# nemo110110/modify-sift-gpu

Hardware: AMD Instinct MI355X
Metric: SIFT images/sec at 1080p (features/sec alongside), 1/2/4/8 MI355X (higher is better)
Workload: dtype f32

## Files before the change

include/sgpu.h:

```cpp
#ifndef SGPU_H
#define SGPU_H
#include <stddef.h>
#include <stdint.h>

#ifdef __cplusplus
extern "C" {
#endif

#define SGPU_OK 0
#define SGPU_EINVAL (-1)
#define SGPU_ENODEV (-2)
#define SGPU_ENOMEM (-3)
#define SGPU_ERANGE (-4)

typedef struct sgpu_options {
    float filter_width_factor;
    float descriptor_window_factor;
    float orientation_window_factor;
    float orientation_gaussian_factor;
    float dog_threshold;
    float edge_threshold;
    int subpixel;
    int max_orientation;
    int fixed_orientation;
    int octave_min;
    int octave_num;
    int dog_level_num;
    int lowe_origin;
    int normalized;
    int descriptors;
    int keep_extremum_sign;
    int circular_window;
    int verbose;
    int max_dimension;
    int preprocess_on_cpu;
    int feature_count_threshold;
    int truncate_method;
} sgpu_options;

void sgpu_default_options(sgpu_options* opt);

int sgpu_parse_args(sgpu_options* opt, int argc, const char* const* argv, int* device);

typedef struct sgpu_ctx sgpu_ctx;

int sgpu_ctx_create(int device, const sgpu_options* opt, sgpu_ctx** out);
int sgpu_ctx_destroy(sgpu_ctx* ctx);
int sgpu_ctx_set_options(sgpu_ctx* ctx, const sgpu_options* opt);
const char* sgpu_last_error(const sgpu_ctx* ctx);
int sgpu_device_count(void);

#define SGPU_INPUT_HOST   0
#define SGPU_INPUT_DEVICE 1
#define SGPU_INPUT_STAGED 2

int sgpu_stage_input(sgpu_ctx* ctx, const uint8_t* images, int n, int w, int h, int stride);

int sgpu_reserve(sgpu_ctx* ctx, int n, int w, int h, int stride);
int sgpu_last_pyramid_launches(const sgpu_ctx* ctx, int* filters);
long long sgpu_debug_alloc_count(void);

int sgpu_extract(sgpu_ctx* ctx, const uint8_t* images, int n, int w, int h, int stride,
                 int flags);

int sgpu_extract_stream(sgpu_ctx* ctx, const uint8_t* const* batches, int nbatches, int batch,
                        int w, int h, int stride, float* keys, float* desc, int64_t cap,
                        int32_t* counts);
void* sgpu_host_alloc(size_t bytes);
void sgpu_host_free(void* p);

int sgpu_extract_f32(sgpu_ctx* ctx, const float* images, int n, int w, int h, int stride,
                     int flags);

#define SGPU_RGB  1
#define SGPU_BGR  2
#define SGPU_RGBA 3
#define SGPU_BGRA 4
int sgpu_extract_color(sgpu_ctx* ctx, const uint8_t* images, int n, int w, int h, int stride,
                       int format, int flags);

int sgpu_feature_count(const sgpu_ctx* ctx, int image);
int64_t sgpu_feature_total(const sgpu_ctx* ctx);

int sgpu_copy_features(sgpu_ctx* ctx, int image, float* keys, float* descriptors);

int sgpu_device_features(sgpu_ctx* ctx, const float** keys, const float** descriptors,
                         const int64_t** image_offsets);

int sgpu_extract_keypoints(sgpu_ctx* ctx, int image, const float* keys, int num,
                           int has_orientation);

int sgpu_match(sgpu_ctx* ctx, const uint8_t* d1, int n1, const uint8_t* d2, int n2,
               float distmax, float ratiomax, int mutual_best_match, int max_match,
               int* out_pairs, int flags);

int sgpu_match_guided(sgpu_ctx* ctx, const uint8_t* d1, int n1, const uint8_t* d2, int n2,
                      const float* loc1, const float* loc2, const float* H, const float* F,
                      float distmax, float ratiomax, float hdistmax, float fdistmax,
                      int mutual_best_match, int max_match, int* out_pairs, int flags);

int sgpu_match_shard_begin(sgpu_ctx* ctx, const uint8_t* d1, int ns, int row_begin,
                           const uint8_t* d2, int n2, float distmax, float ratiomax,
                           int mutual_best_match, int* row_match, int* col_best, int flags);
int sgpu_match_shard_end(const int* col_best_all, int nshards, int n2, const int* row_match,
                         int ns, int row_begin, float distmax, float ratiomax,
                         int mutual_best_match, int max_match, int* out_pairs);
int sgpu_match_sharded(sgpu_ctx* ctx, const uint8_t* d1, int ns, int row_begin,
                       const uint8_t* d2, int n2, float distmax, float ratiomax,
                       int mutual_best_match, int max_match, int* out_pairs, int flags);

void sgpu_quantize_descriptors(const float* d, size_t count, uint8_t* out);
int sgpu_quantize_descriptors_gpu(sgpu_ctx* ctx, const float* d, size_t ndesc, uint8_t* out,
                                  int flags);
int sgpu_feature_descriptors_u8(sgpu_ctx* ctx, const uint8_t** desc_u8);
int sgpu_copy_features_u8(sgpu_ctx* ctx, int image, uint8_t* desc);

int sgpu_match_batch(sgpu_ctx* ctx, const uint8_t* desc, const int64_t* set_offsets, int nsets,
                     const int* set_pairs , int npairs,
                     float distmax, float ratiomax, int mutual_best_match, int max_match,
                     int* out_pairs , int64_t cap, int* out_counts ,
                     int flags);
int sgpu_match_images(sgpu_ctx* ctx, const int* image_pairs, int npairs, float distmax,
                      float ratiomax, int mutual_best_match, int max_match,
                      int* out_pairs, int64_t cap, int* out_counts);

int sgpu_match_batch_guided(sgpu_ctx* ctx, const uint8_t* desc, const float* loc,
                            const int64_t* set_offsets, int nsets,
                            const int* set_pairs , int npairs,
                            const float* H ,
                            const float* F ,
                            float distmax, float ratiomax, float hdistmax, float fdistmax,
                            int mutual_best_match, int max_match,
                            int* out_pairs , int64_t cap,
                            int* out_counts , int flags);
int sgpu_match_images_guided(sgpu_ctx* ctx, const int* image_pairs, int npairs,
                             const float* H, const float* F,
                             float distmax, float ratiomax, float hdistmax, float fdistmax,
                             int mutual_best_match, int max_match,
                             int* out_pairs, int64_t cap, int* out_counts);

#define SGPU_MODEL_HOMOGRAPHY  0
#define SGPU_MODEL_FUNDAMENTAL 1
int sgpu_estimate_batch(sgpu_ctx* ctx, const float* loc ,
                        const int64_t* set_offsets, int nsets,
                        const int* set_pairs , int npairs,
                        const int* matches ,
                        const int* match_counts ,
                        int model, float threshold, int iterations, uint32_t seed,
                        float* out_models , int* out_inliers ,
                        uint8_t* out_mask , int flags);
int sgpu_estimate_images(sgpu_ctx* ctx, const int* image_pairs, int npairs,
                         const int* matches, const int* match_counts,
                         int model, float threshold, int iterations, uint32_t seed,
                         float* out_models, int* out_inliers, uint8_t* out_mask);
int sgpu_estimate_batch_refined(sgpu_ctx* ctx, const float* loc, const int64_t* set_offsets,
                                int nsets, const int* set_pairs, int npairs, const int* matches,
                                const int* match_counts, int model, float threshold,
                                int iterations, uint32_t seed, int refine_rounds,
                                float* out_models, int* out_inliers, uint8_t* out_mask,
                                int* out_rounds , int flags);
int sgpu_estimate_images_refined(sgpu_ctx* ctx, const int* image_pairs, int npairs,
                                 const int* matches, const int* match_counts,
                                 int model, float threshold, int iterations, uint32_t seed,
                                 int refine_rounds, float* out_models, int* out_inliers,
                                 uint8_t* out_mask, int* out_rounds );

int sgpu_last_timing(const sgpu_ctx* ctx, float* times, int n);
int sgpu_set_host_output(sgpu_ctx* ctx, float* keys, float* descriptors, int capacity);
int sgpu_set_stage_timing(sgpu_ctx* ctx, int on);

#define SGPU_COMM_ID_BYTES 128
int sgpu_comm_unique_id(uint8_t* id, int bytes);
int sgpu_comm_init(sgpu_ctx* ctx, int nranks, int rank, const uint8_t* id, int bytes);
int sgpu_comm_allgather_i32(sgpu_ctx* ctx, const int32_t* send, int n, int32_t* recv);
int sgpu_comm_allreduce_f64(sgpu_ctx* ctx, double* v, int n, int op_max);

#define SGPU_DEBUG_PARTS2   1
#define SGPU_DEBUG_PARTS4   2
#define SGPU_DEBUG_TINY_CAP 4
#define SGPU_DEBUG_FUSED_MATCH 8
#define SGPU_DEBUG_EXACT_DESCRIPTOR 16
#define SGPU_DEBUG_GAUSS_BLOCK 32
#define SGPU_DEBUG_BAND_SHIFT 20
#define SGPU_DEBUG_KEYED_MATCH 64
#define SGPU_DEBUG_FULL_COLUMNS 128
#define SGPU_DEBUG_DESC_DUAL 256
#define SGPU_DEBUG_ORIENT_WAVE 512
#define SGPU_DEBUG_GAUSS_TILE_ALWAYS 1024
#define SGPU_DEBUG_MATCH_REGSTAGE 2048
#define SGPU_DEBUG_PYR_SERIAL 4096
#define SGPU_DEBUG_GAUSS_LONG_BANDS 8192
#define SGPU_DEBUG_DUO_ALWAYS 16384
#define SGPU_DEBUG_DUO_OFF 32768
#define SGPU_DEBUG_GAUSS_TILE_OFF 65536
#define SGPU_DEBUG_DESC_WIDE_OFF 131072
#define SGPU_DEBUG_DESC_WIDE_ALWAYS 262144
#define SGPU_DEBUG_EXTREMA_TILE_OFF 524288

int sgpu_debug_set_flags(sgpu_ctx* ctx, int flags);
#define SGPU_FEATURES_QUEUE 0
#define SGPU_FEATURES_STATIC_ORIENTATION 1
#define SGPU_FEATURES_STATIC_DESCRIPTOR 2
#define SGPU_FEATURES_STATIC 3
int sgpu_debug_set_feature_queue(sgpu_ctx* ctx, int mode);
#define SGPU_TRIO_OFF 0
#define SGPU_TRIO_ON 1
#define SGPU_TRIO_ALWAYS 2
#define SGPU_PAIRS_FRONT 0
#define SGPU_PAIRS_END 1
int sgpu_debug_set_schedule(sgpu_ctx* ctx, int trio, int pairs);
#define SGPU_DUO_STRIPS_RULE 0
#define SGPU_DUO_STRIPS_WAVE 1
#define SGPU_DUO_STRIPS_COOP 2
int sgpu_debug_set_duo_strips(sgpu_ctx* ctx, int mode);
int sgpu_debug_set_match_prune(sgpu_ctx* ctx, int on);
int sgpu_debug_match_plan_stats(const sgpu_ctx* ctx, long long out[4]);
#define SGPU_PLAN_ENTRY_INTS 7
#define SGPU_PLAN_LEVEL 0
#define SGPU_PLAN_TILE 1
#define SGPU_PLAN_TWO 2
#define SGPU_PLAN_TILE_TWO 3
#define SGPU_PLAN_TILE_DUO 4
#define SGPU_PLAN_TILE_DUO_ONE 5
#define SGPU_PLAN_DUO 6
#define SGPU_PLAN_TRIO 7
#define SGPU_PLAN_KINDS 8
int sgpu_debug_pyramid_plan(const sgpu_ctx* ctx, int* out, int cap);
int sgpu_debug_geometry(const sgpu_ctx* ctx, int* n_octaves, int* dims , int max);
int sgpu_debug_gaussian(sgpu_ctx* ctx, int image, int octave, int level, float* out);
int sgpu_debug_candidates(sgpu_ctx* ctx, int* ints, float* floats, int cap, int* n);

typedef struct sgpu_verify_params {
    float distmax, ratiomax;
    int   mutual_best_match;
    int   max_match;
    float h_threshold, f_threshold;
    float hdistmax, fdistmax;
    int   iterations;
    uint32_t seed;
    int   refine_rounds;
} sgpu_verify_params;
void sgpu_default_verify_params(sgpu_verify_params* p);
int sgpu_verify_batch(sgpu_ctx* ctx, const uint8_t* desc, const float* loc,
                      const int64_t* set_offsets, int nsets,
                      const int* set_pairs , int npairs,
                      const sgpu_verify_params* params,
                      float* out_H , int* out_inliers_H ,
                      float* out_F , int* out_inliers_F ,
                      int* out_putative ,
                      int* out_pairs , int64_t cap, int* out_counts ,
                      int flags);
int sgpu_verify_images(sgpu_ctx* ctx, const int* image_pairs, int npairs,
                       const sgpu_verify_params* params,
                       float* out_H, int* out_inliers_H, float* out_F, int* out_inliers_F,
                       int* out_putative, int* out_pairs, int64_t cap, int* out_counts);

int sgpu_select_top_scale_batch(sgpu_ctx* ctx, const float* scale, int scale_stride ,
                                const int64_t* set_offsets, int nsets, int top,
                                int* out_index ,
                                int64_t* out_offsets , int flags);
int sgpu_select_top_scale_images(sgpu_ctx* ctx, int top, int* out_index, int64_t* out_offsets);
int sgpu_prematch_batch(sgpu_ctx* ctx, const uint8_t* desc, const float* scale, int scale_stride,
                        const int64_t* set_offsets, int nsets,
                        const int* set_pairs , int npairs, int top,
                        float distmax, float ratiomax, int mutual_best_match,
                        int* out_counts ,
                        int* out_pairs , int64_t cap, int flags);
int sgpu_prematch_images(sgpu_ctx* ctx, const int* image_pairs, int npairs, int top,
                         float distmax, float ratiomax, int mutual_best_match,
                         int* out_counts, int* out_pairs, int64_t cap);

#ifdef __cplusplus
}
#endif
#endif
```

modify-sift-gpu_amd/csrc/sgpu_capi.cpp:

```cpp
#include <dlfcn.h>

#include <cstdio>
#include <cstdlib>
#include <cstring>

#include "sgpu_ctx.h"

using namespace sgh;

std::atomic<long long> sgh::g_allocs{0};

int sgh::part_streams(Part& pt, int which) {
    int prio_lo = 0, prio_hi = 0;
    (void)hipDeviceGetStreamPriorityRange(&prio_lo, &prio_hi);
    if ((which & PS_MAIN) && !pt.stream &&
        hipStreamCreateWithPriority(&pt.stream, hipStreamNonBlocking, prio_hi) != hipSuccess)
        return SGPU_ENODEV;
    if ((which & PS_LO) && !pt.stream_lo &&
        hipStreamCreateWithPriority(&pt.stream_lo, hipStreamNonBlocking, prio_lo) != hipSuccess)
        return SGPU_ENODEV;
    if ((which & PS_OCT) && !pt.stream_oct &&
        hipStreamCreateWithPriority(&pt.stream_oct, hipStreamNonBlocking, prio_hi) != hipSuccess)
        return SGPU_ENODEV;
    if (!pt.ev_ds) {
        for (hipEvent_t& e : pt.ev)
            if (hipEventCreate(&e) != hipSuccess) return SGPU_ENODEV;
        if (hipEventCreateWithFlags(&pt.ev_ds, hipEventDisableTiming) != hipSuccess ||
            hipEventCreateWithFlags(&pt.ev_oct, hipEventDisableTiming) != hipSuccess)
            return SGPU_ENODEV;
    }
    return SGPU_OK;
}

static void apply_env_hooks(sgpu_ctx* ctx) {
    if (const char* ev = getenv("SGPU_EXACT_DESCRIPTOR"))
        if (ev[0] == '1') ctx->debug_flags |= SGPU_DEBUG_EXACT_DESCRIPTOR;
    if (const char* ev = getenv("SGPU_GAUSS")) {
        if (!strcmp(ev, "block")) ctx->debug_flags |= SGPU_DEBUG_GAUSS_BLOCK;
    }
    if (const char* ev = getenv("SGPU_DUO")) {
        if (!strcmp(ev, "off")) ctx->debug_flags |= SGPU_DEBUG_DUO_OFF;
        if (!strcmp(ev, "always")) ctx->debug_flags |= SGPU_DEBUG_DUO_ALWAYS;
        if (!strcmp(ev, "on")) ctx->duo_on = true;
    }
    if (const char* ev = getenv("SGPU_DUO_WIDE")) {
        if (ev[0] == '1') ctx->duo_wide = true;
    }
    if (const char* ev = getenv("SGPU_DUO_U8")) {
        if (ev[0] == '1') ctx->duo_u8 = true;
    }
    if (const char* ev = getenv("SGPU_DUO_PLAN")) {
        if (!strcmp(ev, "end")) ctx->duo_plan = SGPU_PAIRS_END;
        if (!strcmp(ev, "front")) ctx->duo_plan = SGPU_PAIRS_FRONT;
    }
    if (const char* ev = getenv("SGPU_TRIO")) {
        if (!strcmp(ev, "off")) ctx->trio_mode = SGPU_TRIO_OFF;
        if (!strcmp(ev, "always")) ctx->trio_mode = SGPU_TRIO_ALWAYS;
        if (!strcmp(ev, "on")) ctx->trio_mode = SGPU_TRIO_ON;
    }
    if (const char* ev = getenv("SGPU_GAUSS_BANDS"))
        if (!strcmp(ev, "long")) ctx->debug_flags |= SGPU_DEBUG_GAUSS_LONG_BANDS;
    if (const char* ev = getenv("SGPU_PYR")) {
        if (!strcmp(ev, "serial")) ctx->debug_flags |= SGPU_DEBUG_PYR_SERIAL;
    }
    if (const char* ev = getenv("SGPU_STREAMS")) ctx->multi_stream = !strcmp(ev, "multi");
    if (const char* ev = getenv("SGPU_MATCH"))
        if (!strcmp(ev, "reg")) ctx->debug_flags |= SGPU_DEBUG_MATCH_REGSTAGE;
    if (const char* ev = getenv("SGPU_DESC")) {
        if (!strcmp(ev, "dual")) ctx->debug_flags |= SGPU_DEBUG_DESC_DUAL;
        if (!strcmp(ev, "narrow")) ctx->debug_flags |= SGPU_DEBUG_DESC_WIDE_OFF;
        if (!strcmp(ev, "wide")) ctx->debug_flags |= SGPU_DEBUG_DESC_WIDE_ALWAYS;
    }
    if (const char* ev = getenv("SGPU_GAUSS_TILE")) {
        if (!strcmp(ev, "off")) ctx->debug_flags |= SGPU_DEBUG_GAUSS_TILE_OFF;
        if (!strcmp(ev, "always")) ctx->debug_flags |= SGPU_DEBUG_GAUSS_TILE_ALWAYS;
    }
    if (const char* ev = getenv("SGPU_WIDE_DESC_MAX"))
        if (atoll(ev) >= 0) ctx->wide_desc_max = (size_t)atoll(ev);
    if (const char* ev = getenv("SGPU_WAVE_ORIENT_MAX"))
        if (atoll(ev) >= 0) ctx->wave_orient_max = (size_t)atoll(ev);
    if (const char* ev = getenv("SGPU_EXTREMA")) {
        if (!strcmp(ev, "wave")) ctx->debug_flags |= SGPU_DEBUG_EXTREMA_TILE_OFF;
    }
    if (const char* ev = getenv("SGPU_FEATURE_QUEUE")) {
        if (!strcmp(ev, "on") || !strcmp(ev, "ori") || !strcmp(ev, "desc") || !strcmp(ev, "off")) {
            ctx->queue_ori = !strcmp(ev, "on") || !strcmp(ev, "ori");
            ctx->queue_desc = !strcmp(ev, "on") || !strcmp(ev, "desc");
        }
    }
    if (const char* ev = getenv("SGPU_FEATURE_QUEUE_GRID"))
        if (atoi(ev) >= 1) {
            ctx->fq.ori_grid = std::min(ctx->fq.ori_grid, atoi(ev));
            ctx->fq.desc_grid = std::min(ctx->fq.desc_grid, atoi(ev));
        }
    if (const char* ev = getenv("SGPU_TILE_DUO"))
        ctx->tile_duo = !strcmp(ev, "on");
    if (const char* ev = getenv("SGPU_MATCH_PRUNE"))
        ctx->match_prune = strcmp(ev, "off") != 0;
    if (const char* ev = getenv("SGPU_GAUSS_TILE_MB"))
        if (atoi(ev) >= 0) ctx->tile_mb = atoi(ev);
}

extern "C" {

void sgpu_default_options(sgpu_options* o) {
    o->filter_width_factor = 4.0f;
    o->descriptor_window_factor = 3.0f;
    o->orientation_window_factor = 2.0f;
    o->orientation_gaussian_factor = 1.5f;
    o->dog_threshold = 0.0f;
    o->edge_threshold = 0.0f;
    o->subpixel = 1;
    o->max_orientation = 2;
    o->fixed_orientation = 0;
    o->octave_min = 0;
    o->octave_num = -1;
    o->dog_level_num = 3;
    o->lowe_origin = 0;
    o->normalized = 1;
    o->descriptors = 1;
    o->keep_extremum_sign = 0;
    o->circular_window = 0;
    o->verbose = 0;
    o->max_dimension = 13200;
    o->preprocess_on_cpu = 1;
    o->feature_count_threshold = -1;
    o->truncate_method = 0;
}

int sgpu_parse_args(sgpu_options* o, int argc, const char* const* argv, int* device) {
    if (!o) return SGPU_EINVAL;
    auto key = [](const char* s) {
        std::string k;
        for (int i = 0; i < 4 && s[i]; i++) k += (char)((s[i] >= 'A' && s[i] <= 'Z') ? s[i] + 32 : s[i]);
        return k;
    };
    for (int i = 0; i < argc; i++) {
        const char* arg = argv[i];
        if (!arg || arg[0] != '-' || !arg[1]) continue;
        const std::string k = key(arg + 1);
        const char* param = (i + 1 < argc) ? argv[i + 1] : nullptr;
        float fv = 0.f;
        int iv = 0;
        if (k == "cuda") {
            int dev = -1;
            if (param && sscanf(param, "%d", &dev) == 1 && dev >= 0) {
                if (device) *device = dev;
                i++;
            }
        } else if (k == "sd") o->descriptors = 0;
        else if (k == "unn") o->normalized = 0;
        else if (k == "ndes") o->normalized = 1;
        else if (k == "m" || k == "mo") {
            int mo = 2;
            if (param) sscanf(param, "%d", &mo);
            o->max_orientation = std::min(std::max(1, mo), 4);
        } else if (k == "m2p") o->max_orientation = 2;
        else if (k == "s") {
            int sp = 1;
            if (param) sscanf(param, "%d", &sp);
            o->subpixel = std::min(std::max(0, sp), 5);
        } else if (k == "ofix") o->fixed_orientation = (strcmp(arg + 1, "ofix") == 0);
        else if (k == "lowe") o->lowe_origin = 1;
        else if (k == "sign") o->keep_extremum_sign = 1;
        else if (k == "prep") o->preprocess_on_cpu = 1;
        else if (k == "nopr") o->preprocess_on_cpu = 0;
        else if (!param) continue;
        else if (k == "tc" || k == "tc1" || k == "tc2" || k == "tc3") {
            o->truncate_method = k == "tc2" ? 1 : k == "tc3" ? 2 : 0;
            if (sscanf(param, "%d", &iv) == 1 && iv > 0) { o->feature_count_threshold = iv; i++; }
        } else if (k == "maxd") {
            if (sscanf(param, "%d", &iv) == 1 && iv > 0) { o->max_dimension = iv; i++; }
        }
        else if (k == "f") { if (sscanf(param, "%f", &fv) == 1 && fv > 0) { o->filter_width_factor = fv; i++; } }
        else if (k == "w") { if (sscanf(param, "%f", &fv) == 1 && fv > 0) { o->orientation_window_factor = fv; i++; } }
        else if (k == "dw") { if (sscanf(param, "%f", &fv) == 1 && fv > 0) { o->descriptor_window_factor = fv; i++; } }
        else if (k == "fo") { iv = -3; if (sscanf(param, "%d", &iv) == 1 && iv >= -2) { o->octave_min = iv; i++; } }
        else if (k == "no") {
            iv = -1;
            if (sscanf(param, "%d", &iv) == 1) {
                iv = std::max(-1, iv);
                if (iv == -1 || iv >= 1) { o->octave_num = iv; i++; }
            }
        } else if (k == "t") { if (sscanf(param, "%f", &fv) == 1 && fv > 0 && fv < 0.5f) { o->dog_threshold = fv; i++; } }
        else if (k == "e") { if (sscanf(param, "%f", &fv) == 1 && fv > 0) { o->edge_threshold = fv; i++; } }
        else if (k == "d") { if (sscanf(param, "%d", &iv) == 1 && iv >= 1 && iv <= 6) { o->dog_level_num = iv; i++; } }
        else if (k == "v") { if (sscanf(param, "%d", &iv) == 1 && iv >= 0 && iv <= 4) o->verbose = iv; }
    }
    return SGPU_OK;
}

int sgpu_device_count(void) {
    int n = 0;
    if (hipGetDeviceCount(&n) != hipSuccess) return 0;
    return n;
}

int sgpu_ctx_set_options(sgpu_ctx* ctx, const sgpu_options* opt) {
    if (!ctx) return SGPU_EINVAL;
    sgpu_options o;
    if (opt) o = *opt; else sgpu_default_options(&o);
    if (o.octave_min < -3) o.octave_min = -3;
    if (o.dog_level_num < 1 || o.dog_level_num > 6) return ctx->fail(SGPU_EINVAL, "dog_level_num must be 1..6");
    if (o.max_dimension < 8) return ctx->fail(SGPU_EINVAL, "max_dimension must be >= 8");
    ctx->opt = o;
    ctx->f_ready = false;
    sgp::Options po;
    po.filter_width_factor = o.filter_width_factor;
    po.dog_level_num = o.dog_level_num;
    po.dog_threshold = o.dog_threshold;
    po.edge_threshold = o.edge_threshold;
    po.octave_min = o.octave_min;
    ctx->sched = sgp::make_schedule(po);
    return SGPU_OK;
}

int sgpu_ctx_create(int device, const sgpu_options* opt, sgpu_ctx** out) {
    if (!out) return SGPU_EINVAL;
    *out = nullptr;
    int n = 0;
    if (hipGetDeviceCount(&n) != hipSuccess || n <= 0) return SGPU_ENODEV;
    if (device < 0 || device >= n) return SGPU_EINVAL;
    sgpu_ctx* ctx = new sgpu_ctx();
    ctx->device = device;
    if (hipSetDevice(device) != hipSuccess ||
        hipStreamCreateWithFlags(&ctx->stream, hipStreamNonBlocking) != hipSuccess) {
        delete ctx;
        return SGPU_ENODEV;
    }
    for (int i = 0; i <= T_N; i++) (void)hipEventCreate(&ctx->ev[i]);
    {
        Part* p = ctx->part;
        bool ok = part_streams(p[0], PS_MAIN) == SGPU_OK && part_streams(p[0], PS_OCT) == SGPU_OK &&
                  hipStreamCreateWithFlags(&ctx->h2d, hipStreamNonBlocking) == hipSuccess &&
                  hipStreamCreateWithFlags(&ctx->d2h, hipStreamNonBlocking) == hipSuccess &&
                  part_streams(p[0], PS_LO) == SGPU_OK && part_streams(p[1], PS_OCT) == SGPU_OK &&
                  part_streams(p[2], PS_MAIN) == SGPU_OK && part_streams(p[2], PS_LO) == SGPU_OK &&
                  part_streams(p[1], PS_MAIN) == SGPU_OK && part_streams(p[1], PS_LO) == SGPU_OK;
        ok = ok && sgk::feature_queue_grids(&ctx->fq) == hipSuccess;
        for (int i = 0; ok && i < 2; i++)
            ok = hipEventCreateWithFlags(&ctx->up_ev[i], hipEventDisableTiming) == hipSuccess &&
                 hipEventCreateWithFlags(&ctx->down_ev[i], hipEventDisableTiming) == hipSuccess;
        if (!ok) {
            sgpu_ctx_destroy(ctx);
            return SGPU_ENODEV;
        }
    }
    apply_env_hooks(ctx);
    ctx->env_flags = ctx->debug_flags;
    int rc = sgpu_ctx_set_options(ctx, opt);
    if (rc != SGPU_OK) {
        sgpu_ctx_destroy(ctx);
        return rc;
    }
    *out = ctx;
    return SGPU_OK;
}

int sgpu_ctx_destroy(sgpu_ctx* ctx) {
    if (!ctx) return SGPU_EINVAL;
    (void)hipSetDevice(ctx->device);
    if (ctx->stream) (void)hipStreamSynchronize(ctx->stream);
    for (Part& pt : ctx->part) {
        if (pt.stream) (void)hipStreamSynchronize(pt.stream);
        if (pt.stream_lo) (void)hipStreamSynchronize(pt.stream_lo);
        if (pt.stream_oct) (void)hipStreamSynchronize(pt.stream_oct);
        pt.release();
    }
    comm_release(ctx);
    for (hipStream_t st : {ctx->h2d, ctx->d2h})
        if (st) (void)hipStreamSynchronize(st);
    for (int i = 0; i < 2; i++) {
        if (ctx->up_ev[i]) (void)hipEventDestroy(ctx->up_ev[i]);
        if (ctx->down_ev[i]) (void)hipEventDestroy(ctx->down_ev[i]);
    }
    if (ctx->h2d) (void)hipStreamDestroy(ctx->h2d);
    if (ctx->d2h) (void)hipStreamDestroy(ctx->d2h);
    DevBuf* bufs[] = {&ctx->input, &ctx->input2, &ctx->duo_trash, &ctx->all_keys, &ctx->all_desc, &ctx->gray, &ctx->pre, &ctx->m_d1, &ctx->m_d2, &ctx->m_s1, &ctx->m_s2,
                      &ctx->m_part, &ctx->m_terms, &ctx->m_match, &ctx->m_dist, &ctx->m_mask, &ctx->m_loc,
                      &ctx->m_colpart, &ctx->m_cols, &ctx->m_prune, &ctx->m_s1c,
                      &ctx->b_desc, &ctx->b_s8, &ctx->b_sums, &ctx->b_plan, &ctx->b_part, &ctx->b_dec,
                      &ctx->b_cnt, &ctx->b_out, &ctx->b_loc, &ctx->q_in, &ctx->q_out, &ctx->f_u8, &ctx->f_s8,
                      &ctx->f_sums, &ctx->c_buf, &ctx->e_loc, &ctx->e_plan, &ctx->e_pts, &ctx->e_slots,
                      &ctx->e_out, &ctx->e_mask, &ctx->v_buf, &ctx->p_scale, &ctx->p_index, &ctx->p_u8};
    for (DevBuf* b : bufs) b->release();
    for (int i = 0; i <= T_N; i++)
        if (ctx->ev[i]) (void)hipEventDestroy(ctx->ev[i]);
    if (ctx->stream) (void)hipStreamDestroy(ctx->stream);
    delete ctx;
    return SGPU_OK;
}

const char* sgpu_last_error(const sgpu_ctx* ctx) { return ctx ? ctx->err.c_str() : "null context"; }

long long sgpu_debug_alloc_count(void) { return g_allocs.load(); }

int sgpu_set_stage_timing(sgpu_ctx* ctx, int on) {
    if (!ctx) return SGPU_EINVAL;
    ctx->stage_timing = on != 0;
    return SGPU_OK;
}

int sgpu_last_pyramid_launches(const sgpu_ctx* ctx, int* filters) {
    if (!ctx || ctx->batch <= 0) return SGPU_EINVAL;
    if (filters) *filters = ctx->part[0].gauss_filters;
    return ctx->part[0].gauss_launches;
}

int sgpu_last_timing(const sgpu_ctx* ctx, float* times, int n) {
    if (!ctx || !times) return SGPU_EINVAL;
    for (int i = 0; i < n && i < T_N; i++) times[i] = ctx->timing[i];
    return SGPU_OK;
}

int sgpu_debug_set_flags(sgpu_ctx* ctx, int flags) {
    if (!ctx) return SGPU_EINVAL;
    ctx->debug_flags = flags | ctx->env_flags;
    return SGPU_OK;
}

int sgpu_debug_set_match_prune(sgpu_ctx* ctx, int on) {
    if (!ctx) return SGPU_EINVAL;
    ctx->match_prune = on != 0;
    return SGPU_OK;
}

int sgpu_debug_match_plan_stats(const sgpu_ctx* ctx, long long out[4]) {
    if (!ctx || !out || !ctx->b_planned) return SGPU_EINVAL;
    const sgplan::Plan& plan = ctx->b_hplan;
    long long tiles = 0, chunks = 0;
    for (const sgplan::Item& it : plan.items)
        tiles = std::max<long long>(tiles, (it.c_end - it.c_begin + sgplan::kTileCols - 1) / sgplan::kTileCols);
    for (const sgplan::Side& sd : plan.sides) chunks = std::max<long long>(chunks, sd.chunks);
    out[0] = (long long)plan.items.size();
    out[1] = (long long)plan.sides.size();
    out[2] = tiles;
    out[3] = chunks;
    return SGPU_OK;
}

static_assert(SGPU_PLAN_KINDS == sgpyr::kKinds && SGPU_PLAN_TRIO == sgpyr::kTrio &&
              SGPU_PLAN_TILE_DUO_ONE == sgpyr::kTileDuoOne, "sgpu.h and sift_pyramid_plan.h agree");
int sgpu_debug_pyramid_plan(const sgpu_ctx* ctx, int* out, int cap) {
    if (!ctx || ctx->batch <= 0 || cap < 0 || (cap > 0 && !out)) return SGPU_EINVAL;
    const Part& pt = ctx->part[0];
    const int n = (int)pt.plan.launches.size();
    for (int e = 0; e < n && (e + 1) * SGPU_PLAN_ENTRY_INTS <= cap; e++) {
        const sgpyr::Launch& l = pt.plan.launches[e];
        int* p = out + e * SGPU_PLAN_ENTRY_INTS;
        p[0] = l.kind;
        for (int j = 0; j < 3; j++) {
            p[1 + 2 * j] = l.op[j] < 0 ? -1 : pt.levels[l.op[j]].o;
            p[2 + 2 * j] = l.op[j] < 0 ? -1 : pt.levels[l.op[j]].k;
        }
    }
    return n;
}

static_assert(SGPU_DUO_STRIPS_RULE == sgk::kDuoStripsRule && SGPU_DUO_STRIPS_WAVE == sgk::kDuoStripsWave &&
              SGPU_DUO_STRIPS_COOP == sgk::kDuoStripsCoop, "sgpu.h and sift_kernels.h agree");
int sgpu_debug_set_duo_strips(sgpu_ctx* ctx, int mode) {
    if (!ctx || mode < SGPU_DUO_STRIPS_RULE || mode > SGPU_DUO_STRIPS_COOP) return SGPU_EINVAL;
    ctx->duo_strips = mode;
    return SGPU_OK;
}

int sgpu_debug_set_feature_queue(sgpu_ctx* ctx, int mode) {
    if (!ctx || mode < SGPU_FEATURES_QUEUE || mode > SGPU_FEATURES_STATIC) return SGPU_EINVAL;
    ctx->queue_ori = !(mode & SGPU_FEATURES_STATIC_ORIENTATION);
    ctx->queue_desc = !(mode & SGPU_FEATURES_STATIC_DESCRIPTOR);
    return SGPU_OK;
}

int sgpu_debug_set_schedule(sgpu_ctx* ctx, int trio, int pairs) {
    if (!ctx || trio < SGPU_TRIO_OFF || trio > SGPU_TRIO_ALWAYS || pairs < SGPU_PAIRS_FRONT ||
        pairs > SGPU_PAIRS_END)
        return SGPU_EINVAL;
    ctx->trio_mode = trio;
    ctx->duo_plan = pairs;
    return SGPU_OK;
}

int sgpu_debug_geometry(const sgpu_ctx* ctx, int* n_octaves, int* dims, int max) {
    if (!ctx || !n_octaves) return SGPU_EINVAL;
    *n_octaves = (int)ctx->oct.size();
    for (int o = 0; o < (int)ctx->oct.size() && o < max; o++) {
        dims[3 * o] = ctx->oct[o].w;
        dims[3 * o + 1] = ctx->oct[o].h;
        dims[3 * o + 2] = ctx->oct[o].wa;
    }
    return SGPU_OK;
}

int sgpu_debug_gaussian(sgpu_ctx* ctx, int image, int octave, int level, float* out) {
    if (!ctx || image < 0 || image >= ctx->batch || octave < 0 ||
        octave >= (int)ctx->oct.size() || level < 0 || level >= ctx->sched.level_num)
        return SGPU_EINVAL;
    HIPCHK(ctx, hipSetDevice(ctx->device));
    const Part& pt = ctx->part[ctx->part_of(image)];
    const sgk::OctaveDesc& od = pt.fp.oct[octave];
    const long long npx = (long long)od.wa * od.h;
    const float* src = pt.pyr.as<float>() + od.gauss_off + level * od.level_stride +
                       (image - pt.img0) * npx;
    HIPCHK(ctx, hipMemcpy(out, src, npx * sizeof(float), hipMemcpyDeviceToHost));
    return SGPU_OK;
}

static sgk::DebugCandidatesFn debug_candidates_hook() {
    static sgk::DebugCandidatesFn fn = [] {
        Dl_info info{};
        if (!dladdr(reinterpret_cast<void*>(&sgpu_debug_candidates), &info) || !info.dli_fname)
            return (sgk::DebugCandidatesFn) nullptr;
        std::string path(info.dli_fname);
        const size_t slash = path.rfind('/');
        path = (slash == std::string::npos ? std::string(".") : path.substr(0, slash)) +
               "/libsiftgpu_debug.so";
        void* h = dlopen(path.c_str(), RTLD_NOW | RTLD_LOCAL);
        return h ? reinterpret_cast<sgk::DebugCandidatesFn>(dlsym(h, "sgpu_testhook_candidates"))
                 : (sgk::DebugCandidatesFn) nullptr;
    }();
    return fn;
}

int sgpu_debug_candidates(sgpu_ctx* ctx, int* ints, float* floats, int cap, int* n) {
    if (!ctx || !n) return SGPU_EINVAL;
    uint32_t total = 0;
    for (int p = 0; p < ctx->nparts; p++) total += ctx->part[p].n_cand;
    *n = (int)total;
    if (!ints || !floats || cap < (int)total) return total ? SGPU_ERANGE : SGPU_OK;
    if (total == 0) return SGPU_OK;
    const sgk::DebugCandidatesFn hook = debug_candidates_hook();
    if (!hook) return ctx->fail(SGPU_EINVAL, "test-hook library lib/libsiftgpu_debug.so not found");
    HIPCHK(ctx, hipSetDevice(ctx->device));
    DevBuf a, b;
    ALLOCCHK(ctx, a.ensure(total * sizeof(int4)));
    ALLOCCHK(ctx, b.ensure(total * sizeof(float4)));
    uint32_t at = 0;
    for (int p = 0; p < ctx->nparts; p++) {
        const Part& pt = ctx->part[p];
        if (!pt.n_cand) continue;
        HIPCHK(ctx, hook(pt.pyr.as<float>(), pt.mask.as<uint32_t>(), pt.row_base.as<uint32_t>(),
                         pt.total_rows, pt.row_base.as<uint32_t>() + pt.total_rows,
                         (int)pt.n_cand, &pt.fp, a.as<int4>() + at, b.as<float4>() + at,
                         ctx->stream));
        at += pt.n_cand;
    }
    HIPCHK(ctx, hipMemcpyAsync(ints, a.p, total * sizeof(int4), hipMemcpyDeviceToHost, ctx->stream));
    HIPCHK(ctx, hipMemcpyAsync(floats, b.p, total * sizeof(float4), hipMemcpyDeviceToHost, ctx->stream));
    HIPCHK(ctx, hipStreamSynchronize(ctx->stream));
    at = 0;
    for (int p = 0; p < ctx->nparts; p++) {
        const Part& pt = ctx->part[p];
        for (uint32_t i = 0; i < pt.n_cand; i++) ints[4 * (at + i) + 3] += pt.img0;
        at += pt.n_cand;
    }
    a.release();
    b.release();
    return SGPU_OK;
}

}
```

modify-sift-gpu_amd/csrc/sgpu_ctx.h:

```cpp
#pragma once
#include <hip/hip_runtime.h>

#include <algorithm>
#include <atomic>
#include <cstdint>
#include <string>
#include <vector>

#include "../../include/sgpu.h"
#include "sift_geom.h"
#include "sift_kernels.h"
#include "sift_match_plan.h"
#include "sift_params.h"
#include "sift_pyramid_plan.h"
#include "sift_select.h"

typedef struct ncclComm* ncclComm_t;

namespace sgh {

#ifndef SGK_WIDE_DESC_MAX
#define SGK_WIDE_DESC_MAX 8192
#endif

extern std::atomic<long long> g_allocs;

struct DevBuf {
    void* p = nullptr;
    size_t bytes = 0;
    hipError_t ensure(size_t n) {
        if (n <= bytes) return hipSuccess;
        if (p) (void)hipFree(p);
        p = nullptr;
        bytes = 0;
        n = std::max<size_t>(n, 256);
        g_allocs++;
        hipError_t e = hipMalloc(&p, n);
        if (e == hipSuccess) bytes = n;
        return e;
    }
    void release() {
        if (p) (void)hipFree(p);
        p = nullptr;
        bytes = 0;
    }
    template <class T> T* as() const { return reinterpret_cast<T*>(p); }
};

enum { T_UPLOAD, T_PYRAMID, T_DETECT, T_ORIENT, T_EXPAND, T_DESC, T_DOWNLOAD, T_TOTAL, T_MATCH,
       T_LIST, T_COPY_KEYS, T_COPY_DESC, T_ESTIMATE, T_VERIFY, T_PREMATCH, T_N };

struct Part {
    hipStream_t stream = nullptr;
    hipStream_t stream_lo = nullptr;
    bool one_stream = false;
    hipStream_t stream_oct = nullptr;
    hipEvent_t ev_ds = nullptr;
    hipEvent_t ev_oct = nullptr;
    size_t cand_hint = 0, feat_hint = 0;
    int gauss_launches = 0, gauss_filters = 0;
    std::vector<sgk::LevelOp> ops;
    std::vector<sgpyr::LevelDesc> levels;
    sgpyr::Plan plan;
    bool events = true;
    bool copied_out = false;
    hipEvent_t ev[10] = {};
    int img0 = 0, n = 0;
    sgk::FeatureParams fp{};
    int total_rows = 0;
    long long mask_words = 0;
    size_t cand_cap = 0;
    uint32_t n_cand = 0;
    std::vector<int64_t> img_off;
    int64_t* h_read = nullptr;
    size_t h_read_n = 0;
    DevBuf pyr, mask, row_count, row_base, scan_tmp, cand, info, ocount, eoff, feat, feat_info,
        keys, desc, img_off_dev;
    float timing[T_N] = {};

    void release() {
        DevBuf* bufs[] = {&pyr, &mask, &row_count, &row_base, &scan_tmp, &cand, &info, &ocount,
                          &eoff, &feat, &feat_info, &keys, &desc, &img_off_dev};
        for (DevBuf* b : bufs) b->release();
        if (h_read) (void)hipHostFree(h_read);
        h_read = nullptr;
        for (hipEvent_t& e : ev)
            if (e) (void)hipEventDestroy(e);
        if (stream) (void)hipStreamDestroy(stream);
        if (stream_lo) (void)hipStreamDestroy(stream_lo);
        if (ev_ds) (void)hipEventDestroy(ev_ds);
        if (ev_oct) (void)hipEventDestroy(ev_oct);
        ev_ds = ev_oct = nullptr;
        if (stream_oct) (void)hipStreamDestroy(stream_oct);
        stream = stream_lo = stream_oct = nullptr;
    }
};

constexpr int kMaxParts = 4;
#ifndef SGPU_WAVE_ORIENT_MAX
#define SGPU_WAVE_ORIENT_MAX 16384
#endif
constexpr size_t kWaveOrientationMax = SGPU_WAVE_ORIENT_MAX;

}

struct sgpu_ctx {
    int device = 0;
    hipStream_t stream = nullptr;
    sgpu_options opt{};
    sgp::Schedule sched{};
    sgp::InputPlan plan{};
    int debug_flags = 0;
    bool multi_stream = false;
    bool duo_on = false;
    bool duo_wide = false;
    bool duo_u8 = false;
    int trio_mode = SGPU_TRIO_OFF;
    int duo_plan = SGK_DUO_PLAN;
    int duo_strips = SGPU_DUO_STRIPS_RULE;
    size_t wide_desc_max = SGK_WIDE_DESC_MAX;
    size_t wave_orient_max = sgh::kWaveOrientationMax;
    bool unit_input = true;
    bool tile_duo = false;
    int tile_mb = SGK_TILE_MB;
    int env_flags = 0;
    sgk::FeatureQueue fq{};
    bool queue_ori = true, queue_desc = true;
    struct HostOut {
        float* keys = nullptr;
        float* desc = nullptr;
        int cap = 0;
        bool armed = false, active = false, done = false;
    } host_out;
    bool stage_timing = true;
    bool streaming = false;
    std::string err;
    int batch = 0, w = 0, h = 0, nparts = 0;
    std::vector<sgp::Octave> oct;
    size_t staged_bytes = 0;
    std::vector<int64_t> img_off;
    sgh::Part part[sgh::kMaxParts];
    sgh::DevBuf input, all_keys, all_desc, gray, pre;
    sgh::DevBuf input2;
    sgh::DevBuf duo_trash;
    hipStream_t h2d = nullptr, d2h = nullptr;
    hipEvent_t up_ev[2] = {}, down_ev[2] = {};
    bool gathered = false;
    hipEvent_t ev[sgh::T_N + 1] = {};
    float timing[sgh::T_N] = {};
    sgh::DevBuf m_d1, m_d2, m_s1, m_s2, m_part, m_terms, m_match, m_dist, m_mask, m_loc, m_colpart, m_cols;
    sgh::DevBuf m_prune, m_s1c;
    bool match_prune = true;
    std::vector<int> h_match;
    bool dist_ready = false;
    sgh::DevBuf b_desc, b_s8, b_sums, b_plan, b_part, b_dec, b_cnt, b_out;
    sgh::DevBuf b_loc;
    sgplan::Plan b_hplan;
    bool b_planned = false;
    std::vector<unsigned char> b_tables;
    sgh::DevBuf e_loc, e_plan, e_pts, e_slots, e_out, e_mask;
    sgeo::Plan e_hplan;
    std::vector<unsigned char> e_tables, e_result;
    sgh::DevBuf v_buf;
    std::vector<unsigned char> v_result;
    sgh::DevBuf p_scale, p_index, p_u8;
    sgplan::Plan p_hplan;
    std::vector<int64_t> p_sub;
    std::vector<int> p_pairs;
    sgh::DevBuf q_in, q_out, f_u8, f_s8, f_sums;
    bool f_ready = false;
    ncclComm_t comm = nullptr;
    int comm_ranks = 0, comm_rank = 0;
    sgh::DevBuf c_buf;

    int fail(int code, const char* what, hipError_t e = hipSuccess) {
        err = what;
        if (e != hipSuccess) {
            err += ": ";
            err += hipGetErrorString(e);
        }
        return code;
    }
    int part_of(int i) const {
        for (int p = 0; p < nparts; p++)
            if (i < part[p].img0 + part[p].n) return p;
        return nparts - 1;
    }
};

#define HIPCHK(ctx, call)                                                \
    do {                                                                 \
        hipError_t _e = (call);                                          \
        if (_e != hipSuccess) return (ctx)->fail(SGPU_ENODEV, #call, _e); \
    } while (0)
#define ALLOCCHK(ctx, call)                                              \
    do {                                                                 \
        hipError_t _e = (call);                                          \
        if (_e != hipSuccess) return (ctx)->fail(SGPU_ENOMEM, #call, _e); \
    } while (0)

namespace sgh {
enum { PS_MAIN = 1, PS_LO = 2, PS_OCT = 4, PS_ALL = 7 };
int part_streams(Part& pt, int which = PS_ALL);
float match_dist(int v);
int ensure_dist_table(sgpu_ctx* ctx);
int feature_u8(sgpu_ctx* ctx);
void comm_release(sgpu_ctx* ctx);

struct SetSource {
    bool images = false, device = false;
    const uint8_t* desc = nullptr;
    const float* loc = nullptr;
    const float* scale = nullptr;
    int scale_stride = 1;
};
struct DeviceSets {
    const uint8_t* u8 = nullptr;
    const uint8_t* s8 = nullptr;
    const int* sums = nullptr;
    const float* loc = nullptr;
    int loc_stride = 2;
    const float* scale = nullptr;
    int scale_stride = 1;
    bool timing_started = false;
};
enum { SET_DESC = 1, SET_LOC = 2, SET_SCALE = 4 };
int resolve_sets(sgpu_ctx* ctx, const SetSource& src, int64_t rows, int need, DeviceSets& sets);
int check_batch(sgpu_ctx* ctx, const char* what);
int probe_offsets(const int64_t* off, int nsets);
inline size_t round8(size_t n) { return (n + 7) & ~(size_t)7; }
int ensure_pair_buffers(sgpu_ctx* ctx, const sgplan::Plan& plan, size_t table_bytes,
                        int64_t out_rows, int cnt_pairs, int64_t s8_rows);
int derive_s8(sgpu_ctx* ctx, DeviceSets& sets, int64_t rows);
struct MatchPass {
    const uint8_t* s8;
    const int* sums;
    const sgplan::Plan& plan;
    sgplan::TableView tab;
    float distmax, ratiomax;
    int max_match;
    int64_t out_rows;
    int* d_counts;
    long long* d_offs;
    int* d_out;
    const float* loc = nullptr;
    int loc_stride = 2;
    const sgk::GuidedParams* d_geom = nullptr;
};
int queue_match_pass(sgpu_ctx* ctx, const MatchPass& m);
int download_fitting(sgpu_ctx* ctx, const int* counts, int npairs, const int* d_out, int* out_pairs,
                     int64_t cap, bool want_matches = true);
}
```

modify-sift-gpu_amd/csrc/sgpu_debug.hip:

```cpp
#include <cstdint>

#include "sift_kernels.h"
#include "sift_math.h"

using namespace sgm;

#include "sift_keys.h"

namespace sgk {
namespace {

__global__ __launch_bounds__(64) void k_debug_candidates(
    const float* __restrict__ pyr, const uint32_t* __restrict__ mask,
    const uint32_t* __restrict__ row_base, int total_rows, const uint32_t* __restrict__ n_cand_dev,
    const FeatureParams fp, int4* __restrict__ ints, float4* __restrict__ floats) {
    const uint32_t f = blockIdx.x * 64 + threadIdx.x;
    if (f >= *n_cand_dev) return;
    const KeyLoc L = locate(f, row_base, total_rows, mask, fp);
    const KeyOut kv = key_at(pyr, fp, L);
    ints[f] = make_int4(L.col, L.row, L.o * fp.d + L.j, L.b);
    floats[f] = make_float4(kv.dx, kv.dy, kv.ds, kv.result);
}

}
}

extern "C" __attribute__((visibility("default"))) hipError_t sgpu_testhook_candidates(
    const float* pyr, const uint32_t* mask, const uint32_t* row_base, int total_rows,
    const uint32_t* n_cand_dev, int n_cand_cap, const sgk::FeatureParams* fp, int4* ints,
    float4* floats, hipStream_t stream) {
    if (n_cand_cap <= 0) return hipSuccess;
    hipLaunchKernelGGL(sgk::k_debug_candidates, dim3((n_cand_cap + 63) / 64), dim3(64), 0, stream,
                       pyr, mask, row_base, total_rows, n_cand_dev, *fp, ints, floats);
    return hipGetLastError();
}
```

modify-sift-gpu_amd/csrc/sgpu_extract.cpp:

```cpp
#include <cmath>
#include <cstring>

#include "sgpu_ctx.h"

using namespace sgh;

extern "C" {

static int layout_part(sgpu_ctx* ctx, Part& pt) {
    const sgpu_options& O = ctx->opt;
    const sgp::Schedule& S = ctx->sched;
    const int d = S.dog_level_num, nlev = S.level_num;
    const int noct = (int)ctx->oct.size();
    const int n = pt.n;

    sgk::FeatureParams& fp = pt.fp;
    fp = sgk::FeatureParams{};
    fp.batch = n;
    fp.n_octaves = noct;
    fp.d = d;
    long long goff = 0, moff = 0;
    int rows = 0;
    for (int o = 0; o < noct; o++) {
        const sgp::Octave& oc = ctx->oct[o];
        sgk::OctaveDesc& od = fp.oct[o];
        od.w = oc.w;
        od.h = oc.h;
        od.wa = oc.wa;
        od.nwords = (oc.wa + 31) / 32;
        od.gauss_off = goff;
        od.level_stride = (long long)n * oc.wa * oc.h;
        goff += od.level_stride * nlev;
        od.mask_off = moff;
        od.mask_level_stride = (long long)n * oc.h * od.nwords;
        moff += od.mask_level_stride * d;
        fp.row_off[o] = rows;
        rows += d * oc.h;
    }
    fp.rows_per_image = rows;
    pt.total_rows = rows * n;
    pt.mask_words = moff;
    for (int j = 0; j < d; j++) fp.level_sigma[j] = sgp::level_sigma(S, j + S.level_min + 1);
    fp.sigma_step = powf(2.0f, 1.0f / d);
    fp.t0 = (O.subpixel ? 0.8f : 1.0f) * S.dog_threshold;
    fp.t = S.dog_threshold;
    fp.edge = (S.edge_threshold + 1) * (S.edge_threshold + 1) / S.edge_threshold;
    fp.gaussian_factor = O.orientation_gaussian_factor;
    fp.sample_factor = O.orientation_gaussian_factor * O.orientation_window_factor;
    fp.window_factor = O.descriptor_window_factor;
    fp.subpixel = O.subpixel ? 1 : 0;
    fp.num_orientation = O.fixed_orientation ? 0 : std::min(O.max_orientation, 2);
    fp.keep_sign = O.keep_extremum_sign;
    fp.circular = O.circular_window;
    fp.normalize = O.normalized;
    fp.unit_input = ctx->unit_input ? 1 : 0;
    fp.origin_offset = O.lowe_origin ? 0.0f : 0.5f;
    fp.octave_min = ctx->plan.octave_min + ctx->plan.ds;

    const size_t sum_px = (size_t)goff / (size_t)std::max(1, nlev) / (size_t)n;
    pt.cand_cap = (ctx->debug_flags & SGPU_DEBUG_TINY_CAP)
                      ? std::max<size_t>(pt.cand_cap, 64)
                      : std::max(pt.cand_cap, std::max<size_t>(1024, sum_px / 256 * n));
    const size_t nc = pt.cand_cap, ne_cap = 2 * nc;
    ALLOCCHK(ctx, pt.pyr.ensure((size_t)goff * sizeof(float) + 256));
    ALLOCCHK(ctx, pt.mask.ensure((size_t)moff * sizeof(uint32_t)));
    ALLOCCHK(ctx, pt.row_count.ensure((size_t)pt.total_rows * sizeof(uint32_t)));
    ALLOCCHK(ctx, pt.row_base.ensure(((size_t)pt.total_rows + 1) * sizeof(uint32_t)));
    ALLOCCHK(ctx, pt.img_off_dev.ensure((size_t)(n + 2) * sizeof(int64_t)));
    ALLOCCHK(ctx, pt.cand.ensure(nc * sizeof(float4)));
    ALLOCCHK(ctx, pt.info.ensure(nc * sizeof(int2)));
    ALLOCCHK(ctx, pt.ocount.ensure((sgk::feature_queue_base(nc) + sgk::kFeatureQueueWords) * sizeof(uint32_t)));
    ALLOCCHK(ctx, pt.eoff.ensure((nc + 1) * sizeof(uint32_t)));
    ALLOCCHK(ctx, pt.feat.ensure(ne_cap * sizeof(float4)));
    ALLOCCHK(ctx, pt.feat_info.ensure(ne_cap * sizeof(int2)));
    ALLOCCHK(ctx, pt.keys.ensure(ne_cap * sizeof(float4)));
    if (O.descriptors) ALLOCCHK(ctx, pt.desc.ensure(ne_cap * 128 * sizeof(float)));
    ALLOCCHK(ctx, pt.scan_tmp.ensure((sgk::scan_tmp_words(std::max<size_t>(nc, pt.total_rows)) + 16) * 4));
    if (pt.h_read_n < (size_t)n + 2) {
        if (pt.h_read) (void)hipHostFree(pt.h_read);
        pt.h_read = nullptr;
        g_allocs++;
        ALLOCCHK(ctx, hipHostMalloc((void**)&pt.h_read, ((size_t)n + 2) * sizeof(int64_t)));
        pt.h_read_n = (size_t)n + 2;
    }
    return SGPU_OK;
}

static int build_level_ops(sgpu_ctx* ctx, Part& pt, const uint8_t* src8, const float* srcf,
                           int stride, hipStream_t st) {
    const sgpu_options& O = ctx->opt;
    const sgp::Schedule& S = ctx->sched;
    const sgk::FeatureParams& fp = pt.fp;
    const int nlev = S.level_num, noct = (int)ctx->oct.size(), n = pt.n, h = ctx->h;
    const size_t img_elems = (size_t)stride * h;
    float* pyr = pt.pyr.as<float>();
    sgk::Taps ltaps[sgk::kMaxLevels], taps0;
    int lfw[sgk::kMaxLevels] = {0};
    for (int k = 1; k < nlev; k++)
        lfw[k] = sgp::make_filter(S.sigma[k - 1], O.filter_width_factor, ltaps[k].k);
    const int fw0 = sgp::make_filter(S.initial_smooth, O.filter_width_factor, taps0.k);
    const int kds = S.level_ds - S.level_min;
    pt.ops.clear();
    pt.levels.clear();
    pt.ops.reserve((size_t)noct * nlev);
    pt.levels.reserve((size_t)noct * nlev);
    for (int o = 0; o < noct; o++) {
        const sgk::OctaveDesc& od = fp.oct[o];
        const long long npx = (long long)od.wa * od.h;
        float* lvl0 = pyr + od.gauss_off;
        float* ds = nullptr;
        int dsw = 0, dsh = 0;
        long long ds_stride = 0;
        if (o + 1 < noct) {
            const sgk::OctaveDesc& nd = fp.oct[o + 1];
            ds = pyr + nd.gauss_off;
            dsw = nd.wa;
            dsh = nd.h;
            ds_stride = (long long)nd.wa * nd.h;
        }
        const float* in_f = srcf;
        const uint8_t* in_8 = src8;
        int in_stride = stride;
        long long in_img = (long long)img_elems;
        if (o == 0 && ctx->plan.octave_min != 0) {
            float* tmp = lvl0 + od.level_stride;
            HIPCHK(ctx, sgk::launch_first_octave_input(srcf, src8, stride, (long long)img_elems,
                                                       ctx->w & ~3, h, ctx->plan.octave_min, tmp,
                                                       od.wa, od.h, npx, n, st));
            in_f = tmp;
            in_8 = nullptr;
            in_stride = od.wa;
            in_img = npx;
        }
        for (int k = (o == 0 ? 0 : 1); k < nlev; k++) {
            pt.ops.emplace_back();
            sgk::LevelOp& op = pt.ops.back();
            op.fw = k == 0 ? fw0 : lfw[k];
            const float* tk = k == 0 ? taps0.k : ltaps[k].k;
            for (int i = 0; i < op.fw; i++) op.taps.k[i] = tk[i];
            const bool dk = ds && kds == k;
            op.src = k == 0 ? in_f : lvl0 + (k - 1) * od.level_stride;
            op.src_u8 = k == 0 ? in_8 : nullptr;
            op.src_stride = k == 0 ? in_stride : od.wa;
            op.src_img_stride = k == 0 ? in_img : npx;
            op.dst = lvl0 + k * od.level_stride;
            op.dst_img_stride = npx;
            op.w = od.wa;
            op.h = od.h;
            op.batch = n;
            op.ds_dst = dk ? ds : nullptr;
            op.ds_w = dk ? dsw : 0;
            op.ds_h = dk ? dsh : 0;
            op.ds_img_stride = dk ? ds_stride : 0;
            if (o == 0 && k == 0 && pt.one_stream) {
                op.zero.p[0] = pt.row_count.as<uint32_t>();
                op.zero.n[0] = (size_t)pt.total_rows;
                op.zero.p[1] = pt.mask.as<uint32_t>();
                op.zero.n[1] = (size_t)pt.mask_words;
                op.zero.p[2] = pt.ocount.as<uint32_t>();
                op.zero.n[2] = sgk::feature_queue_base(pt.cand_cap) + sgk::kFeatureQueueWords;
            }
            pt.levels.push_back(sgpyr::LevelDesc{o, k, op.fw, op.w, op.h, op.batch, dk,
                                                 op.src_u8 != nullptr,
                                                 (op.zero.n[0] | op.zero.n[1] | op.zero.n[2]) != 0});
        }
    }
    pt.gauss_filters = (int)pt.ops.size();
    return SGPU_OK;
}

struct OpSupport {
    const sgk::LevelOp* op;
    bool tile(int i) const { return sgk::gauss_tile_supported(op[i]); }
    bool tile_duo(int i, int j) const { return sgk::gauss_tile_duo_supported(op[i], op[j]); }
    bool duo(int i, int j) const { return sgk::gauss_duo_supported(op[i], op[j]); }
    bool trio(int i, int j, int l) const { return sgk::gauss_trio_supported(op[i], op[j], op[l]); }
};

static sgpyr::Rules pyramid_rules(const sgpu_ctx* ctx, const Part& pt) {
    const int f = ctx->debug_flags;
    sgpyr::Rules R;
    R.kds = ctx->sched.level_ds - ctx->sched.level_min;
    R.side_stream = !pt.one_stream;
    R.serial = (f & SGPU_DEBUG_PYR_SERIAL) != 0;
    R.wave_rows = (f & SGPU_DEBUG_GAUSS_BLOCK) ? -1 : ((f >> SGPU_DEBUG_BAND_SHIFT) & 0x7ff);
    R.long_bands = (f & SGPU_DEBUG_GAUSS_LONG_BANDS) != 0;
    R.tiles_off = (f & SGPU_DEBUG_GAUSS_TILE_OFF) != 0;
    R.tiles_always = (f & SGPU_DEBUG_GAUSS_TILE_ALWAYS) != 0;
    R.tile_mb = ctx->tile_mb;
    R.tile_duo = ctx->tile_duo;
    R.duo_off = (f & SGPU_DEBUG_DUO_OFF) != 0;
    R.duo_always = (f & SGPU_DEBUG_DUO_ALWAYS) != 0;
    R.duo_on = ctx->duo_on;
    R.duo_wide = ctx->duo_wide;
    R.duo_u8 = ctx->duo_u8;
    R.trio_mode = ctx->trio_mode;
    R.duo_plan = ctx->duo_plan;
    return R;
}
static_assert(SGPU_TRIO_OFF == sgpyr::kTrioOff && SGPU_TRIO_ON == sgpyr::kTrioOn &&
              SGPU_TRIO_ALWAYS == sgpyr::kTrioAlways && SGPU_PAIRS_FRONT == sgpyr::kPairsFront &&
              SGPU_PAIRS_END == sgpyr::kPairsEnd, "sgpu.h and sift_pyramid_plan.h agree");

static int ensure_gauss_trash(sgpu_ctx* ctx) {
    ALLOCCHK(ctx, ctx->duo_trash.ensure(std::max(sgk::kGaussDuoTrashBytes, sgk::kGaussTrioTrashBytes)));
    return SGPU_OK;
}

static int enqueue_part(sgpu_ctx* ctx, Part& pt, const void* src_in, bool is_f32, int stride,
                        hipEvent_t wait, hipEvent_t wait_lo = nullptr) {
    hipStream_t st = pt.stream;
    const sgpu_options& O = ctx->opt;
    const int n = pt.n, h = ctx->h;
    const int rc_layout = layout_part(ctx, pt);
    if (rc_layout != SGPU_OK) return rc_layout;
    const sgk::FeatureParams& fp = pt.fp;
    const long long moff = pt.mask_words;
    const size_t nc = pt.cand_cap, ne_cap = 2 * nc;

    if (wait) HIPCHK(ctx, hipStreamWaitEvent(st, wait, 0));
    pt.events = ctx->stage_timing || !pt.one_stream || ctx->nparts > 1 || ctx->streaming;
    auto rec = [&](int i, hipStream_t s_) -> hipError_t {
        return pt.events ? hipEventRecord(pt.ev[i], s_) : hipSuccess;
    };
    HIPCHK(ctx, rec(0, st));
    const size_t img_elems = (size_t)stride * h;
    const uint8_t* src8 = is_f32 ? nullptr : (const uint8_t*)src_in + (size_t)pt.img0 * img_elems;
    const float* srcf = is_f32 ? (const float*)src_in + (size_t)pt.img0 * img_elems : nullptr;

    float* pyr = pt.pyr.as<float>();
    const int rc_ops = build_level_ops(ctx, pt, src8, srcf, stride, st);
    if (rc_ops != SGPU_OK) return rc_ops;
    const sgpyr::Rules R = pyramid_rules(ctx, pt);
    sgpyr::plan_pyramid(pt.levels.data(), (int)pt.levels.size(), R, OpSupport{pt.ops.data()}, pt.plan);
    const int rc_trash = pt.plan.trash ? ensure_gauss_trash(ctx) : SGPU_OK;
    if (rc_trash != SGPU_OK) return rc_trash;
    const bool side = pt.plan.side;
    float* const trash = ctx->duo_trash.as<float>();
    pt.gauss_launches = 0;
    for (const sgpyr::Launch& l : pt.plan.launches) {
        const hipStream_t s_ = l.side ? pt.stream_oct : st;
        const sgk::LevelOp& a = pt.ops[l.op[0]];
        const sgk::LevelOp& b = pt.ops[std::max(l.op[1], 0)];
        const sgk::LevelOp& c = pt.ops[std::max(l.op[2], 0)];
        int nl = 1;
        if (l.wait_ds) HIPCHK(ctx, hipStreamWaitEvent(s_, pt.ev_ds, 0));
        switch (l.kind) {
            case sgpyr::kLevel: HIPCHK(ctx, sgk::launch_gauss_op(a, s_, R.wave_rows, R.long_bands)); break;
            case sgpyr::kTile: HIPCHK(ctx, sgk::launch_gauss_tile(a, s_)); break;
            case sgpyr::kTwo: HIPCHK(ctx, sgk::launch_gauss_two(a, b, s_, R.wave_rows, R.long_bands, &nl)); break;
            case sgpyr::kTileTwo: HIPCHK(ctx, sgk::launch_gauss_tile_two(a, b, s_, &nl)); break;
            case sgpyr::kTileDuo: HIPCHK(ctx, sgk::launch_gauss_tile_duo(a, b, s_)); break;
            case sgpyr::kTileDuoOne: HIPCHK(ctx, sgk::launch_gauss_tile_duo_one(a, b, c, s_, &nl)); break;
            case sgpyr::kDuo:
                HIPCHK(ctx, sgk::launch_gauss_duo(a, b, s_, R.wave_rows, trash, ctx->duo_strips));
                break;
            case sgpyr::kTrio: HIPCHK(ctx, sgk::launch_gauss_trio(a, b, c, s_, R.wave_rows, trash)); break;
            default: return ctx->fail(SGPU_EINVAL, "unknown pyramid launch kind");
        }
        pt.gauss_launches += nl;
        if (l.rec_ds) HIPCHK(ctx, hipEventRecord(pt.ev_ds, st));
    }
    if (side) {
        HIPCHK(ctx, hipEventRecord(pt.ev_oct, pt.stream_oct));
        HIPCHK(ctx, hipStreamWaitEvent(st, pt.ev_oct, 0));
    }
    HIPCHK(ctx, rec(1, st));

    if (!pt.one_stream)
        HIPCHK(ctx, sgk::launch_zero(pt.row_count.as<uint32_t>(), (size_t)pt.total_rows,
                                     pt.mask.as<uint32_t>(), (size_t)moff, nullptr, 0, st));
    const bool ext_tiles = !(ctx->debug_flags & SGPU_DEBUG_EXTREMA_TILE_OFF) &&
                           ((ctx->debug_flags & SGPU_DEBUG_GAUSS_TILE_ALWAYS) ||
                            4ll * fp.oct[0].wa * fp.oct[0].h * n <= ((long long)ctx->tile_mb << 20));
    HIPCHK(ctx, sgk::launch_extrema(pyr, pt.mask.as<uint32_t>(), pt.row_count.as<uint32_t>(),
                                    fp, st, ext_tiles));
    if (O.feature_count_threshold > 0)
        HIPCHK(ctx, sgk::launch_limit_rows(pt.row_count.as<uint32_t>(), fp,
                                           O.feature_count_threshold, O.truncate_method, st));
    HIPCHK(ctx, rec(7, st));
    HIPCHK(ctx, sgk::launch_scan(pt.row_count.as<uint32_t>(), pt.row_base.as<uint32_t>(),
                                 pt.total_rows, pt.scan_tmp.as<uint32_t>(), st));
    HIPCHK(ctx, rec(2, st));

    if (!pt.one_stream) {
        st = pt.stream_lo;
        HIPCHK(ctx, hipStreamWaitEvent(st, pt.ev[2], 0));
    }
    if (wait_lo) HIPCHK(ctx, hipStreamWaitEvent(st, wait_lo, 0));
    const uint32_t* n_cand_dev = pt.row_base.as<uint32_t>() + pt.total_rows;
    if (!pt.one_stream)
        HIPCHK(ctx, sgk::launch_zero(pt.ocount.as<uint32_t>(), sgk::feature_queue_base(nc) + sgk::kFeatureQueueWords,
                                     nullptr, 0, nullptr, 0, st));
    sgk::FeatureQueue fq = ctx->fq;
    fq.next = pt.ocount.as<uint32_t>() + sgk::feature_queue_base(nc);
    const int cand_grid = (int)std::min(nc, pt.cand_hint ? pt.cand_hint : nc);
    const bool ori_wave = (ctx->debug_flags & SGPU_DEBUG_ORIENT_WAVE) ||
                          (pt.cand_hint > 0 && pt.cand_hint <= ctx->wave_orient_max);
    const int feat_grid = (int)std::min(ne_cap, pt.feat_hint ? pt.feat_hint : ne_cap);
    const bool desc_wide = !(ctx->debug_flags & SGPU_DEBUG_DESC_WIDE_OFF) &&
                           ((ctx->debug_flags & SGPU_DEBUG_DESC_WIDE_ALWAYS) ||
                            (pt.feat_hint > 0 && pt.feat_hint <= ctx->wide_desc_max));
    HIPCHK(ctx, sgk::launch_orientation(pyr, pt.mask.as<uint32_t>(), pt.row_base.as<uint32_t>(),
                                        pt.total_rows, n_cand_dev, (int)nc, cand_grid, fp,
                                        pt.cand.as<float4>(), pt.info.as<int2>(),
                                        pt.ocount.as<uint32_t>(), st, ori_wave,
                                        ctx->queue_ori ? &fq : nullptr));
    if (O.feature_count_threshold > 0 && fp.num_orientation >= 2)
        HIPCHK(ctx, sgk::launch_limit_oriented(pt.ocount.as<uint32_t>(), pt.row_base.as<uint32_t>(),
                                               fp, O.feature_count_threshold, O.truncate_method,
                                               (uint32_t)nc, st));
    HIPCHK(ctx, rec(3, st));
    const uint32_t* n_feat_dev = pt.eoff.as<uint32_t>() + nc;
    sgk::ImageOffsetsArgs io;
    io.row_base = pt.row_base.as<uint32_t>();
    io.batch = n;
    io.rows_per_image = fp.rows_per_image;
    io.total_rows = pt.total_rows;
    io.off = pt.img_off_dev.as<int64_t>();
    HIPCHK(ctx, sgk::launch_scan(pt.ocount.as<uint32_t>(), pt.eoff.as<uint32_t>(), nc,
                                 pt.scan_tmp.as<uint32_t>(), st));
    HIPCHK(ctx, sgk::launch_expand(pt.cand.as<float4>(), pt.info.as<int2>(),
                                   pt.eoff.as<uint32_t>(), n_cand_dev, (int)nc, fp,
                                   pt.feat.as<float4>(), pt.feat_info.as<int2>(),
                                   pt.keys.as<float4>(), st, &io));
    HIPCHK(ctx, rec(4, st));
    pt.copied_out = ctx->host_out.active && pt.one_stream && n == 1 && ctx->nparts == 1;
    const bool exact_desc = ctx->debug_flags & SGPU_DEBUG_EXACT_DESCRIPTOR;
    const bool dual_desc = ctx->debug_flags & SGPU_DEBUG_DESC_DUAL;
    const bool host_in_desc = pt.copied_out && O.descriptors && desc_wide && !exact_desc && !dual_desc;
    sgk::HostCopy hcopy;
    if (host_in_desc) {
        hcopy.keys = pt.keys.as<float4>();
        hcopy.rec = pt.img_off_dev.as<int64_t>();
        hcopy.rec_n = n + 2;
        hcopy.cap = (uint32_t)ctx->host_out.cap;
        hcopy.hkeys = reinterpret_cast<float4*>(ctx->host_out.keys);
        hcopy.hdesc = ctx->host_out.desc;
        hcopy.hrec = pt.h_read;
    }
    if (O.descriptors) {
        sgk::DescriptorForm form;
        form.exact = exact_desc;
        form.dual = dual_desc;
        form.wide = desc_wide;
        form.host = host_in_desc ? &hcopy : nullptr;
        form.queue = ctx->queue_desc ? &fq : nullptr;
        HIPCHK(ctx, sgk::launch_descriptor(pyr, pt.feat.as<float4>(), pt.feat_info.as<int2>(),
                                           n_feat_dev, feat_grid, fp, pt.desc.as<float>(), form, st));
    }
    HIPCHK(ctx, rec(5, st));
    if (pt.copied_out && !host_in_desc)
        HIPCHK(ctx, sgk::launch_copy_out(pt.keys.as<float4>(), O.descriptors ? pt.desc.as<float>() : nullptr,
                                         n_feat_dev, ctx->host_out.cap, pt.img_off_dev.as<int64_t>(),
                                         n + 2, ctx->host_out.keys,
                                         O.descriptors ? ctx->host_out.desc : nullptr, pt.h_read, st));
    return SGPU_OK;
}

static int enqueue_readback(sgpu_ctx* ctx, Part& pt) {
    hipStream_t st = pt.one_stream ? pt.stream : pt.stream_lo;
    if (!pt.copied_out)
        HIPCHK(ctx, hipMemcpyAsync(pt.h_read, pt.img_off_dev.p, (size_t)(pt.n + 2) * sizeof(int64_t),
                                   hipMemcpyDeviceToHost, st));
    if (pt.events) HIPCHK(ctx, hipEventRecord(pt.ev[6], st));
    return SGPU_OK;
}

static int plan_batch(sgpu_ctx* ctx, int n, int w, int h) {
    const sgpu_options& O = ctx->opt;
    const sgp::InputPlan plan = sgp::plan_input(w, h, O.octave_min, O.max_dimension, O.preprocess_on_cpu);
    if (plan.w < 8 || plan.h < 8) return ctx->fail(SGPU_EINVAL, "image too small for the first octave");
    {
        sgp::Options po;
        po.filter_width_factor = O.filter_width_factor;
        po.dog_level_num = O.dog_level_num;
        po.dog_threshold = O.dog_threshold;
        po.edge_threshold = O.edge_threshold;
        po.octave_min = plan.octave_min + plan.ds;
        ctx->sched = sgp::make_schedule(po);
    }
    ctx->plan = plan;
    ctx->oct = sgp::make_octaves(plan.w, plan.h, O.octave_num, plan.octave_min);
    const int noct = (int)ctx->oct.size();
    if (noct > sgk::kMaxOctaves) return ctx->fail(SGPU_EINVAL, "too many octaves");
    for (const auto& oc : ctx->oct)
        if (oc.w < 4 || oc.h < 4) return ctx->fail(SGPU_EINVAL, "image too small for the octave count");
    ctx->batch = n;
    ctx->w = plan.ds ? plan.w : w;
    ctx->h = plan.h;
    ctx->gathered = false;
    ctx->f_ready = false;
    return SGPU_OK;
}

static int abandon_batch(sgpu_ctx* ctx, int rc) {
    ctx->host_out.done = false;
    for (hipStream_t st : {ctx->stream, ctx->h2d, ctx->d2h})
        if (st) (void)hipStreamSynchronize(st);
    for (Part& pt : ctx->part) {
        if (pt.stream) (void)hipStreamSynchronize(pt.stream);
        if (pt.stream_lo) (void)hipStreamSynchronize(pt.stream_lo);
        if (pt.stream_oct) (void)hipStreamSynchronize(pt.stream_oct);
        pt.img_off.clear();
    }
    ctx->batch = 0;
    ctx->img_off.clear();
    ctx->gathered = false;
    ctx->f_ready = false;
    return rc;
}

static int check_extract_args(sgpu_ctx* ctx, const void* images, bool is_f32, int n, int w, int h,
                              int stride, int flags, int color) {
    const bool staged = (flags & SGPU_INPUT_STAGED) != 0;
    const int channels = color == SGPU_RGB || color == SGPU_BGR ? 3 : color ? 4 : 1;
    if ((!images && !staged) || n <= 0 || w < 8 || h < 8 || stride < w * channels)
        return ctx->fail(SGPU_EINVAL, "bad image arguments");
    if (color && (staged || is_f32 || color > SGPU_BGRA))
        return ctx->fail(SGPU_EINVAL, "bad color input");
    if (staged && (is_f32 || ctx->staged_bytes < (size_t)n * h * stride))
        return ctx->fail(SGPU_EINVAL, "staged input does not match the batch");
    return SGPU_OK;
}

static int extract_body(sgpu_ctx* ctx, const void* images, bool is_f32, int n, int w, int h,
                        int stride, int flags, int color) {
    ctx->unit_input = !is_f32;
    const bool staged = (flags & SGPU_INPUT_STAGED) != 0;
    const int channels = color == SGPU_RGB || color == SGPU_BGR ? 3 : color ? 4 : 1;
    HIPCHK(ctx, hipSetDevice(ctx->device));
    int rc0 = plan_batch(ctx, n, w, h);
    if (rc0 != SGPU_OK) return rc0;
    const sgp::InputPlan plan = ctx->plan;

    int np = 1;
    if ((ctx->debug_flags & SGPU_DEBUG_PARTS2) && n >= 2) np = 2;
    if ((ctx->debug_flags & SGPU_DEBUG_PARTS4) && n >= 4) np = 4;
    ctx->nparts = np;
    for (int p = 0; p < np; p++)
        if (part_streams(ctx->part[p]) != SGPU_OK)
            return ctx->fail(SGPU_ENODEV, "stream creation failed");
    for (int p = 0, i0 = 0; p < np; p++) {
        const int cnt = n / np + (p < n % np ? 1 : 0);
        ctx->part[p].img0 = i0;
        ctx->part[p].n = cnt;
        ctx->part[p].one_stream = false;
        i0 += cnt;
    }
    const bool one = np == 1 && !ctx->multi_stream;
    ctx->part[0].one_stream = one;
    const hipStream_t up = one ? ctx->part[0].stream : ctx->stream;

    const size_t in_bytes = (size_t)n * h * stride * (is_f32 ? sizeof(float) : 1);
    const bool up_events = !one || ((color || plan.ds > 0 ||
                                     !(flags & (SGPU_INPUT_DEVICE | SGPU_INPUT_STAGED))) &&
                                    ctx->stage_timing);
    if (up_events) HIPCHK(ctx, hipEventRecord(ctx->ev[0], up));
    const void* src_in = staged ? ctx->input.p : images;
    if (!(flags & (SGPU_INPUT_DEVICE | SGPU_INPUT_STAGED))) {
        ctx->staged_bytes = 0;
        ALLOCCHK(ctx, ctx->input.ensure(in_bytes));
        HIPCHK(ctx, hipMemcpyAsync(ctx->input.p, images, in_bytes, hipMemcpyHostToDevice, up));
        src_in = ctx->input.p;
    }
    if (color) {
        const int tw = w & ~3;
        ALLOCCHK(ctx, ctx->gray.ensure((size_t)n * h * tw * sizeof(float)));
        HIPCHK(ctx, sgk::launch_color_to_gray((const uint8_t*)src_in, n, w, h, stride, channels,
                                              color == SGPU_BGR || color == SGPU_BGRA,
                                              ctx->gray.as<float>(), up));
        src_in = ctx->gray.p;
        is_f32 = true;
        stride = tw;
    }
    if (plan.ds > 0) {
        const size_t px = (size_t)plan.w * plan.h;
        ALLOCCHK(ctx, ctx->pre.ensure((size_t)n * px * sizeof(float)));
        HIPCHK(ctx, sgk::launch_first_octave_input(is_f32 ? (const float*)src_in : nullptr,
                                                   is_f32 ? nullptr : (const uint8_t*)src_in,
                                                   stride, (long long)stride * h, w & ~3, h, plan.ds,
                                                   ctx->pre.as<float>(), plan.w, plan.h,
                                                   (long long)px, n, up));
        src_in = ctx->pre.p;
        is_f32 = true;
        stride = plan.w;
    }
    if (up_events) HIPCHK(ctx, hipEventRecord(ctx->ev[1], up));

    for (int p = 0; p < np; p++) {
        hipEvent_t wait = p == 0 ? (one ? nullptr : ctx->ev[1]) : ctx->part[p - 1].ev[2];
        int rc = enqueue_part(ctx, ctx->part[p], src_in, is_f32, stride, wait);
        if (rc != SGPU_OK) return rc;
    }
    for (int p = 0; p < np; p++) {
        int rc = enqueue_readback(ctx, ctx->part[p]);
        if (rc != SGPU_OK) return rc;
    }
    for (int p = 0; p < np; p++) {
        HIPCHK(ctx, hipStreamSynchronize(ctx->part[p].stream));
        HIPCHK(ctx, hipStreamSynchronize(ctx->part[p].stream_lo));
    }

    for (int p = 0; p < np; p++) {
        Part& pt = ctx->part[p];
        uint32_t nc = (uint32_t)pt.h_read[0];
        if (nc > pt.cand_cap) {
            pt.cand_cap = (size_t)nc + nc / 4 + 1024;
            int rc = enqueue_part(ctx, pt, src_in, is_f32, stride, nullptr);
            if (rc == SGPU_OK) rc = enqueue_readback(ctx, pt);
            if (rc != SGPU_OK) return rc;
            HIPCHK(ctx, hipStreamSynchronize(pt.one_stream ? pt.stream : pt.stream_lo));
            nc = (uint32_t)pt.h_read[0];
            if (nc > pt.cand_cap) return ctx->fail(SGPU_ERANGE, "keypoint capacity overflow");
        }
        pt.n_cand = nc;
        pt.img_off.assign(pt.h_read + 1, pt.h_read + 2 + pt.n);
        pt.cand_hint = (size_t)nc + nc / 16 + 64;
        pt.feat_hint = (size_t)pt.img_off[pt.n] + pt.img_off[pt.n] / 16 + 64;
    }
    ctx->img_off.assign(n + 1, 0);
    int64_t base = 0;
    for (int p = 0; p < np; p++) {
        const Part& pt = ctx->part[p];
        for (int i = 0; i <= pt.n; i++) ctx->img_off[pt.img0 + i] = base + pt.img_off[i];
        base += pt.img_off[pt.n];
    }

    Part& p0 = ctx->part[0];
    ctx->timing[T_UPLOAD] = 0.0f;
    if (!p0.events) {
        for (int i = T_UPLOAD; i <= T_DOWNLOAD; i++) ctx->timing[i] = 0.0f;
        ctx->timing[T_TOTAL] = ctx->timing[T_LIST] = 0.0f;
        return SGPU_OK;
    }
    if (up_events) (void)hipEventElapsedTime(&ctx->timing[T_UPLOAD], ctx->ev[0], ctx->ev[1]);
    (void)hipEventElapsedTime(&ctx->timing[T_PYRAMID], p0.ev[0], p0.ev[1]);
    (void)hipEventElapsedTime(&ctx->timing[T_DETECT], p0.ev[1], p0.ev[2]);
    (void)hipEventElapsedTime(&ctx->timing[T_LIST], p0.ev[7], p0.ev[2]);
    (void)hipEventElapsedTime(&ctx->timing[T_ORIENT], p0.ev[2], p0.ev[3]);
    (void)hipEventElapsedTime(&ctx->timing[T_EXPAND], p0.ev[3], p0.ev[4]);
    (void)hipEventElapsedTime(&ctx->timing[T_DESC], p0.ev[4], p0.ev[5]);
    (void)hipEventElapsedTime(&ctx->timing[T_DOWNLOAD], p0.ev[5], p0.ev[6]);
    (void)hipEventElapsedTime(&ctx->timing[T_TOTAL], up_events ? ctx->ev[0] : p0.ev[0], ctx->part[np - 1].ev[6]);
    return SGPU_OK;
}

static int extract_impl(sgpu_ctx* ctx, const void* images, bool is_f32, int n, int w, int h,
                        int stride, int flags, int color = 0) {
    if (!ctx) return SGPU_EINVAL;
    const bool armed = ctx->host_out.armed;
    ctx->host_out.armed = false;
    ctx->host_out.done = false;
    const int rc_args = check_extract_args(ctx, images, is_f32, n, w, h, stride, flags, color);
    if (rc_args != SGPU_OK) return rc_args;
    ctx->host_out.active = armed && n == 1;
    const int rc = extract_body(ctx, images, is_f32, n, w, h, stride, flags, color);
    ctx->host_out.done = rc == SGPU_OK && ctx->host_out.active && ctx->nparts == 1 &&
                         ctx->part[0].copied_out;
    ctx->host_out.active = false;
    ctx->part[0].copied_out = ctx->part[1].copied_out = false;
    return rc == SGPU_OK ? rc : abandon_batch(ctx, rc);
}

static int extract_stream_body(sgpu_ctx* ctx, const uint8_t* const* batches, int nbatches,
                               int batch, int w, int h, int stride, float* keys, float* desc,
                               int64_t cap, int32_t* counts) {
    if (!batches || nbatches <= 0 || batch <= 0 || w < 8 || h < 8 || stride < w || !counts ||
        cap < 0)
        return ctx->fail(SGPU_EINVAL, "bad stream arguments");
    for (int k = 0; k < nbatches; k++)
        if (!batches[k]) return ctx->fail(SGPU_EINVAL, "null batch pointer");
    if (desc && !ctx->opt.descriptors) return ctx->fail(SGPU_EINVAL, "descriptors disabled (-sd)");
    HIPCHK(ctx, hipSetDevice(ctx->device));
    int rc = plan_batch(ctx, batch, w, h);
    if (rc != SGPU_OK) return rc;
    int64_t out_base = 0;
    int result = SGPU_OK;
    auto emit_counts = [&](int k, const std::vector<int64_t>& off, int n) {
// ... 426 lines not shown
```

modify-sift-gpu_amd/csrc/sift_detect.hip:

```cpp
#include <algorithm>

#include "sift_device.h"
#include "sift_keys.h"

#ifndef SGK_EXT2_WAVES
#define SGK_EXT2_WAVES 1
#endif
#ifndef SGK_EXT_XCD
#define SGK_EXT_XCD 2
#endif
#ifndef SGK_EXT_XCDG
#define SGK_EXT_XCDG 4
#endif
#ifndef SGK_EXT_CPL
#define SGK_EXT_CPL 2
#endif
#ifndef SGK_EXT_WAVES
#define SGK_EXT_WAVES 32768
#endif
#ifndef SGK_EXT_MINROWS
#define SGK_EXT_MINROWS 16
#endif
#ifndef SGK_EXT_SEG_MIN
#define SGK_EXT_SEG_MIN 32
#endif

namespace sgk {
namespace {


struct ExtremaWaveGrid {
    int wave0[kMaxOctaves + 1];
    int seg_rows[kMaxOctaves];
    int nseg[kMaxOctaves];
};

template <int ND, int CPL>
__global__ __launch_bounds__(256, SGK_EXT2_WAVES) void k_extrema_wave2(const float* __restrict__ pyr,
                                                       uint32_t* __restrict__ mask,
                                                       uint32_t* __restrict__ row_count,
                                                       const FeatureParams fp,
                                                       const ExtremaWaveGrid eg) {
    static_assert(CPL == 1 || CPL == 2, "one or two columns per lane");
    constexpr int TW = 64 * CPL - 2;
    constexpr int RW = 64 * CPL + 2 * CPL + 2;
    constexpr int NJ = ND - 2;
    __shared__ __attribute__((aligned(8))) float s_ring[4][ND][4][RW];
    __shared__ uint16_t s_list[4][NJ * 64 * CPL];
    const int lane = threadIdx.x & 63, wave = threadIdx.x >> 6;
    const int gw = (SGK_EXT_XCD == 1 ? xcd_block(blockIdx.x, gridDim.x)
                    : SGK_EXT_XCD == 2 ? xcd_group<SGK_EXT_XCDG>(blockIdx.x, gridDim.x)
                                       : (int)blockIdx.x) * 4 + wave;
    if (gw >= eg.wave0[fp.n_octaves]) return;
    int o = 0;
    while (o + 1 < fp.n_octaves && gw >= eg.wave0[o + 1]) o++;
    o = __builtin_amdgcn_readfirstlane(o);
    const OctaveDesc& od = fp.oct[o];
    const long long mask_off = od.mask_off, mask_lstride = od.mask_level_stride;
    const int nwords = od.nwords;
    const long long rc_base = fp.row_off[o];
    const int W = od.wa, H = od.h;
    const int strips_x = (W + TW - 1) / TW;
    const int id = gw - eg.wave0[o];
    const int sx = id % strips_x, rest = id / strips_x;
    const int sg = rest % eg.nseg[o], b = rest / eg.nseg[o];
    const int x0 = sx * TW + (CPL - 1);
    const int ys = sg * eg.seg_rows[o], ye = min(H, ys + eg.seg_rows[o]);
    const long long lstride = od.level_stride;
    const float* g0 = pyr + od.gauss_off + (long long)b * W * H;
    float(*ring)[4][RW] = s_ring[wave];
    uint16_t* list = s_list[wave];

    const int xl = x0 - 1 + CPL * lane;
    const int gx = CPL == 1 ? clampi(xl, 0, W - 1) : min(xl, W - 2);
    bool out_col[CPL];
#pragma unroll
    for (int k = 0; k < CPL; k++) {
        const int i = CPL * lane + k, x = xl + k;
        out_col[k] = i >= 1 && i <= TW && x > 0 && x < W - 1;
    }
    struct Row { float m[ND + 1][CPL]; };
    Row rA, rB;
    auto fetch = [&](Row& r, int y) {
        const float* q = g0 + (long long)clampi(y, 0, H - 1) * W + gx;
#pragma unroll
        for (int m = 0; m <= ND; m++) {
            if constexpr (CPL == 1) {
                r.m[m][0] = q[m * lstride];
            } else {
                const float2 v = *reinterpret_cast<const float2*>(q + m * lstride);
                r.m[m][0] = v.x;
                r.m[m][1] = v.y;
            }
        }
    };
    float dog[ND][CPL];
    auto put = [&](const Row& r, int y) {
        float* rr = &ring[0][y & 3][CPL * lane + CPL];
#pragma unroll
        for (int m = 0; m < ND; m++) {
#pragma unroll
            for (int k = 0; k < CPL; k++) dog[m][k] = r.m[m + 1][k] - r.m[m][k];
            if constexpr (CPL == 1)
                rr[m * 4 * RW] = dog[m][0];
            else
                *reinterpret_cast<float2*>(&rr[m * 4 * RW]) = make_float2(dog[m][0], dog[m][1]);
        }
        asm volatile("" ::: "memory");
    };
    float hx0[ND][CPL], hn0[ND][CPL], hx1[ND][CPL], hn1[ND][CPL], cvx[ND][CPL];
    auto rowmm = [&](float (*mx)[CPL], float (*mn)[CPL], float (*cv)[CPL]) {
#pragma unroll
        for (int m = 0; m < ND; m++) {
            float v[CPL + 2];
#pragma unroll
            for (int k = 0; k < CPL; k++) v[k + 1] = dog[m][k];
            v[0] = __int_as_float(__builtin_amdgcn_update_dpp(
                0, __float_as_int(dog[m][CPL - 1]), 0x138, 0xf, 0xf, false));
            v[CPL + 1] = __int_as_float(__builtin_amdgcn_update_dpp(
                0, __float_as_int(dog[m][0]), 0x130, 0xf, 0xf, false));
#pragma unroll
            for (int k = 0; k < CPL; k++) {
                mx[m][k] = fmax_(fmax_(v[k], v[k + 1]), v[k + 2]);
                mn[m][k] = fmin_(fmin_(v[k], v[k + 1]), v[k + 2]);
                if (cv) cv[m][k] = v[k + 1];
            }
        }
    };
    auto body = [&](int y) {
        float hx2[ND][CPL], hn2[ND][CPL], cnx[ND][CPL];
        rowmm(hx2, hn2, cnx);
        const bool row_ok = y < ye && y > 0 && y < H - 1;
        int ncand = 0;
#pragma unroll
        for (int j = 0; j < NJ; j++) {
#pragma unroll
            for (int k = 0; k < CPL; k++) {
                const float v = cvx[j + 1][k];
                float mx = hx0[j][k], mn = hn0[j][k];
#pragma unroll
                for (int m = j; m < j + 3; m++) {
                    mx = fmax_(mx, fmax_(fmax_(hx0[m][k], hx1[m][k]), hx2[m][k]));
                    mn = fmin_(mn, fmin_(fmin_(hn0[m][k], hn1[m][k]), hn2[m][k]));
                }
                const bool cand = row_ok && out_col[k] && !(fabs_(v) <= fp.t0) && !(v < mx && v > mn);
                const unsigned long long bal = __ballot(cand);
                if (cand) {
                    const int pos = ncand + __builtin_amdgcn_mbcnt_hi(
                                                (uint32_t)(bal >> 32),
                                                __builtin_amdgcn_mbcnt_lo((uint32_t)bal, 0u));
                    list[pos] = (uint16_t)((j << 7) | (CPL * lane + k));
                }
                ncand += __popcll(bal);
            }
        }
        asm volatile("" ::: "memory");
        for (int c0 = 0; c0 < ncand; c0 += 64) {
            if (c0 + lane < ncand) {
                const int code = list[c0 + lane];
                const int j = code >> 7, cl = code & 127;
                auto get = [&](int m, int r, int c) {
                    return ring[j + m][(y + r - 1) & 3][cl + c - 1 + CPL];
                };
                if (key_test(get, fp.t0, fp.t, fp.edge, fp.subpixel).result != 0.f) {
                    const int xx = x0 - 1 + cl;
                    uint32_t* mrow = mask + mask_off + j * mask_lstride +
                                     ((long long)b * H + y) * nwords;
                    atomicOr(&mrow[xx >> 5], 1u << (xx & 31));
                    atomicAdd(&row_count[(long long)b * fp.rows_per_image + rc_base + j * H + y],
                              1u);
                }
            }
        }
#pragma unroll
        for (int m = 0; m < ND; m++)
#pragma unroll
            for (int k = 0; k < CPL; k++) {
                hx0[m][k] = hx1[m][k]; hn0[m][k] = hn1[m][k];
                hx1[m][k] = hx2[m][k]; hn1[m][k] = hn2[m][k];
                cvx[m][k] = cnx[m][k];
            }
        asm volatile("" ::: "memory");
    };
    fetch(rA, ys - 1);
    put(rA, ys - 1);
    rowmm(hx0, hn0, nullptr);
    fetch(rA, ys);
    put(rA, ys);
    rowmm(hx1, hn1, cvx);
    fetch(rA, min(ys + 1, ye));
    fetch(rB, min(ys + 2, ye));
    for (int y = ys; y < ye; y += 2) {
        put(rA, y + 1);
        body(y);
        fetch(rA, min(y + 3, ye));
        put(rB, y + 2);
        body(y + 1);
        fetch(rB, min(y + 4, ye));
    }
}

struct ExtremaTileGrid {
    int tile0[kMaxOctaves + 1];
    int tx[kMaxOctaves];
    int ty[kMaxOctaves];
};
constexpr int kEtW = 64, kEtH = 16, kEtLW = 72;

template <int ND>
__global__ __launch_bounds__(256) void k_extrema_tile(const float* __restrict__ pyr,
                                                      uint32_t* __restrict__ mask,
                                                      uint32_t* __restrict__ row_count,
                                                      const FeatureParams fp,
                                                      const ExtremaTileGrid eg) {
    constexpr int NJ = ND - 2, R = kEtH + 2, NQ = kEtLW / 4, NIT = R * NQ;
    constexpr int LITEMS = (NIT + 255) / 256;
    __shared__ __attribute__((aligned(16))) float s_d[ND][R][kEtLW];
    const int tid = threadIdx.x, lane = tid & 63;
    const int wave = __builtin_amdgcn_readfirstlane(tid >> 6);
    const int bid = blockIdx.x;
    int o = 0;
    while (o + 1 < fp.n_octaves && bid >= eg.tile0[o + 1]) o++;
    o = __builtin_amdgcn_readfirstlane(o);
    const OctaveDesc& od = fp.oct[o];
    const int W = od.wa, H = od.h;
    const int id = bid - eg.tile0[o];
    const int sx = id % eg.tx[o], rest = id / eg.tx[o];
    const int sy = rest % eg.ty[o], b = rest / eg.ty[o];
    const int x0 = sx * kEtW, y0 = sy * kEtH;
    const long long lstride = od.level_stride;
    const float* g0 = pyr + od.gauss_off + (long long)b * W * H;
    float4 gq[LITEMS][ND + 1];
#pragma unroll
    for (int i = 0; i < LITEMS; i++) {
        const int it = min(tid + 256 * i, NIT - 1);
        const int rr = it / NQ, q = it - rr * NQ;
        const int y = clampi(y0 - 1 + rr, 0, H - 1);
        const int xq = clampi(x0 - 4 + 4 * q, 0, W - 4);
        const float* p = g0 + (long long)y * W + xq;
#pragma unroll
        for (int m = 0; m <= ND; m++) gq[i][m] = *reinterpret_cast<const float4*>(p + m * lstride);
    }
#pragma unroll
    for (int i = 0; i < LITEMS; i++) {
        const int it = tid + 256 * i;
        if (NIT % 256 != 0 && it >= NIT) break;
        const int rr = it / NQ, q = it - rr * NQ;
#pragma unroll
        for (int m = 0; m < ND; m++) {
            const float4 a = gq[i][m], c = gq[i][m + 1];
            *reinterpret_cast<float4*>(&s_d[m][rr][4 * q]) =
                make_float4(c.x - a.x, c.y - a.y, c.z - a.z, c.w - a.w);
        }
    }
    __syncthreads();
    const int x = x0 + lane;
    const bool col_ok = x > 0 && x < W - 1;
    const int lc = lane + 4;
    float hx[ND][6], hn[ND][6];
#pragma unroll
    for (int m = 0; m < ND; m++)
#pragma unroll
        for (int r = 0; r < 6; r++) {
            const float* row = &s_d[m][4 * wave + r][lc];
            const float a = row[-1], c = row[0], e = row[1];
            hx[m][r] = fmax_(fmax_(a, c), e);
            hn[m][r] = fmin_(fmin_(a, c), e);
        }
    uint32_t pend = 0;
#pragma unroll
    for (int i = 0; i < 4; i++) {
        const int y = y0 + 4 * wave + i;
        const bool row_ok = y > 0 && y < H - 1;
#pragma unroll
        for (int j = 0; j < NJ; j++) {
            const float v = s_d[j + 1][4 * wave + 1 + i][lc];
            float mx = hx[j][i], mn = hn[j][i];
#pragma unroll
            for (int m = j; m < j + 3; m++) {
                mx = fmax_(mx, fmax_(fmax_(hx[m][i], hx[m][i + 1]), hx[m][i + 2]));
                mn = fmin_(mn, fmin_(fmin_(hn[m][i], hn[m][i + 1]), hn[m][i + 2]));
            }
            if (row_ok && col_ok && !(fabs_(v) <= fp.t0) && !(v < mx && v > mn)) pend |= 1u << (i * NJ + j);
        }
    }
    while (__ballot(pend != 0)) {
        if (pend) {
            const int bit = __ffs(pend) - 1;
            pend &= pend - 1;
            const int i = bit / NJ, j = bit - i * NJ;
            const int lr = 4 * wave + 1 + i;
            auto get = [&](int m, int r, int c) { return s_d[j + m][lr + r - 1][lc + c - 1]; };
            if (key_test(get, fp.t0, fp.t, fp.edge, fp.subpixel).result != 0.f) {
                const int y = y0 + 4 * wave + i;
                uint32_t* mrow = mask + od.mask_off + j * od.mask_level_stride +
                                 ((long long)b * H + y) * od.nwords;
                atomicOr(&mrow[x >> 5], 1u << (x & 31));
                atomicAdd(&row_count[(long long)b * fp.rows_per_image + fp.row_off[o] + j * H + y], 1u);
            }
        }
    }
}

__device__ __forceinline__ uint32_t wave_incl_scan(uint32_t v) {
    const int lane = threadIdx.x & 63;
#pragma unroll
    for (int d = 1; d < 64; d <<= 1) {
        uint32_t t = __shfl_up(v, d, 64);
        if (lane >= d) v += t;
    }
    return v;
}

__global__ __launch_bounds__(256) void k_scan_block(const uint32_t* __restrict__ in,
                                                    uint32_t* __restrict__ out, size_t n,
                                                    uint32_t* __restrict__ block_sums) {
    __shared__ uint32_t s_w[4];
    const size_t base = (size_t)blockIdx.x * 1024 + threadIdx.x * 4;
    uint32_t v[4];
#pragma unroll
    for (int i = 0; i < 4; i++) v[i] = (base + i < n) ? in[base + i] : 0u;
    uint32_t tsum = v[0] + v[1] + v[2] + v[3];
    uint32_t incl = wave_incl_scan(tsum);
    const int lane = threadIdx.x & 63, wave = threadIdx.x >> 6;
    if (lane == 63) s_w[wave] = incl;
    __syncthreads();
    uint32_t wofs = 0, total = 0;
    for (int w = 0; w < 4; w++) {
        if (w < wave) wofs += s_w[w];
        total += s_w[w];
    }
    uint32_t run = wofs + incl - tsum;
#pragma unroll
    for (int i = 0; i < 4; i++) {
        if (base + i < n) out[base + i] = run;
        run += v[i];
    }
    if (threadIdx.x == 0) {
        if (block_sums) block_sums[blockIdx.x] = total;
        else out[n] = total;
    }
}

__global__ __launch_bounds__(1024) void k_scan_single(const uint32_t* __restrict__ in,
                                                      uint32_t* __restrict__ out, size_t n) {
    __shared__ uint32_t s_w[16];
    const int lane = threadIdx.x & 63, wave = threadIdx.x >> 6;
    const size_t c = (n + 1023) / 1024;
    const size_t base = (size_t)threadIdx.x * c;
    uint32_t v[32];
    uint32_t tsum = 0;
#pragma unroll
    for (int i = 0; i < 32; i++) {
        v[i] = ((size_t)i < c && base + i < n) ? in[base + i] : 0u;
        tsum += v[i];
    }
    const uint32_t incl = wave_incl_scan(tsum);
    if (lane == 63) s_w[wave] = incl;
    __syncthreads();
    uint32_t wofs = 0, total = 0;
#pragma unroll
    for (int w = 0; w < 16; w++) {
        const uint32_t sw = s_w[w];
        wofs += w < wave ? sw : 0u;
        total += sw;
    }
    uint32_t run = wofs + incl - tsum;
#pragma unroll
    for (int i = 0; i < 32; i++) {
        if ((size_t)i < c && base + i < n) out[base + i] = run;
        run += v[i];
    }
    if (threadIdx.x == 0) out[n] = total;
}

__global__ __launch_bounds__(256) void k_scan_add(uint32_t* __restrict__ out, size_t n,
                                                  const uint32_t* __restrict__ block_ofs) {
    const size_t base = (size_t)blockIdx.x * 1024 + threadIdx.x * 4;
    const uint32_t add = block_ofs[blockIdx.x];
#pragma unroll
    for (int i = 0; i < 4; i++)
        if (base + i < n) out[base + i] += add;
    if (blockIdx.x == 0 && threadIdx.x == 0) out[n] = block_ofs[gridDim.x];
}

constexpr int kMaxLimitLevels = kMaxOctaves * 8;

__device__ void limit_levels(int* cnt, int nl, int T, int method, bool list_stage) {
    if (list_stage && method != 0) {
        int total = 0;
        for (int q = 0; q < nl; q++) {
            const int l = method == 1 ? nl - 1 - q : q;
            if (total > T) cnt[l] = 0;
            else total += cnt[l];
        }
    }
    int num = 0;
    for (int l = 0; l < nl; l++) num += cnt[l];
    if (method == 2) {
        int i = 0, kept = 0;
        for (; kept < T && i < nl; ++i) kept += cnt[i];
        for (; i < nl; ++i) cnt[i] = 0;
    } else {
        for (int i = 0; i < nl && num - cnt[i] > T; ++i) {
            num -= cnt[i];
            cnt[i] = 0;
        }
    }
}

__device__ __forceinline__ int level_of_row(const FeatureParams& fp, int r) {
    int o = 0;
    while (o + 1 < fp.n_octaves && fp.row_off[o + 1] <= r) o++;
    return o * fp.d + (r - fp.row_off[o]) / fp.oct[o].h;
}

__global__ __launch_bounds__(256) void k_limit_rows(uint32_t* __restrict__ row_count,
                                                    const FeatureParams fp, int T, int method) {
    __shared__ int s_cnt[kMaxLimitLevels];
    const int nl = fp.n_octaves * fp.d;
    uint32_t* rc = row_count + (size_t)blockIdx.x * fp.rows_per_image;
    for (int l = threadIdx.x; l < nl; l += 256) s_cnt[l] = 0;
    __syncthreads();
    for (int r = threadIdx.x; r < fp.rows_per_image; r += 256) {
        const uint32_t v = rc[r];
        if (v) atomicAdd(&s_cnt[level_of_row(fp, r)], (int)v);
    }
    __syncthreads();
    if (threadIdx.x == 0) limit_levels(s_cnt, nl, T, method, true);
    __syncthreads();
    for (int r = threadIdx.x; r < fp.rows_per_image; r += 256)
        if (s_cnt[level_of_row(fp, r)] == 0) rc[r] = 0;
}

__global__ __launch_bounds__(256) void k_limit_oriented(uint32_t* __restrict__ ocount,
                                                        const uint32_t* __restrict__ row_base,
                                                        const FeatureParams fp, int T, int method,
                                                        uint32_t cap) {
    __shared__ int s_cnt[kMaxLimitLevels];
    const int nl = fp.n_octaves * fp.d;
    const size_t r0 = (size_t)blockIdx.x * fp.rows_per_image;
    auto range = [&](int l, uint32_t& lo, uint32_t& hi) {
        const int o = l / fp.d, j = l - o * fp.d;
        const size_t first = r0 + fp.row_off[o] + (size_t)j * fp.oct[o].h;
        lo = min(row_base[first], cap);
        hi = min(row_base[first + fp.oct[o].h], cap);
    };
    for (int l = threadIdx.x; l < nl; l += 256) s_cnt[l] = 0;
    __syncthreads();
    for (int l = 0; l < nl; l++) {
        uint32_t lo, hi;
        range(l, lo, hi);
        int sum = 0;
        for (uint32_t f = lo + threadIdx.x; f < hi; f += 256) sum += (int)ocount[f];
        if (sum) atomicAdd(&s_cnt[l], sum);
    }
    __syncthreads();
    if (threadIdx.x == 0) limit_levels(s_cnt, nl, T, method, false);
    __syncthreads();
    for (int l = 0; l < nl; l++) {
        if (s_cnt[l] != 0) continue;
        uint32_t lo, hi;
        range(l, lo, hi);
        for (uint32_t f = lo + threadIdx.x; f < hi; f += 256) ocount[f] = 0;
    }
}

}

hipError_t launch_extrema(const float* pyr, uint32_t* mask, uint32_t* row_count,
                          const FeatureParams& fp, hipStream_t stream, bool tiles) {
    bool tile_ok = tiles && ((uintptr_t)pyr % 16) == 0;
    for (int o = 0; o < fp.n_octaves; o++)
        tile_ok = tile_ok && fp.oct[o].wa % 4 == 0 && fp.oct[o].wa >= 4 && fp.oct[o].gauss_off % 4 == 0 &&
                  fp.oct[o].level_stride % 4 == 0;
    if (tile_ok) {
        ExtremaTileGrid tg{};
        long long nb = 0;
        for (int o = 0; o < fp.n_octaves; o++) {
            tg.tile0[o] = (int)nb;
            tg.tx[o] = (fp.oct[o].wa + kEtW - 1) / kEtW;
            tg.ty[o] = (fp.oct[o].h + kEtH - 1) / kEtH;
            nb += (long long)tg.tx[o] * tg.ty[o] * fp.batch;
        }
        tg.tile0[fp.n_octaves] = (int)nb;
        if (nb <= 0 || nb >= (1ll << 31)) return hipErrorInvalidValue;
        switch (fp.d + 2) {
#define SGK_EXTT(ND) \
    case ND: hipLaunchKernelGGL((k_extrema_tile<ND>), dim3((unsigned)nb), dim3(256), 0, stream, pyr, mask, \
                                row_count, fp, tg); return hipGetLastError();
            SGK_EXTT(3) SGK_EXTT(4) SGK_EXTT(5) SGK_EXTT(6) SGK_EXTT(7) SGK_EXTT(8)
#undef SGK_EXTT
            default: return hipErrorInvalidValue;
        }
    }
    bool pairs = SGK_EXT_CPL == 2 && ((uintptr_t)pyr % 8) == 0;
    for (int o = 0; o < fp.n_octaves; o++)
        pairs = pairs && fp.oct[o].wa % 2 == 0 && fp.oct[o].gauss_off % 2 == 0 &&
                fp.oct[o].level_stride % 2 == 0 && ((long long)fp.oct[o].wa * fp.oct[o].h) % 2 == 0;
    const int sw = pairs ? 126 : 62;
    ExtremaWaveGrid eg{};
    int nw = 0;
    for (int o = 0; o < fp.n_octaves; o++) {
        const OctaveDesc& od = fp.oct[o];
        const int strips_x = (od.wa + sw - 1) / sw;
        const long long per_col = (long long)strips_x * fp.batch;
        const int minrows = fp.batch == 1 ? 8 : SGK_EXT_MINROWS;
        int nseg = (int)std::min<long long>(std::max<long long>(1, (SGK_EXT_WAVES + per_col - 1) / per_col),
                                            std::max(1, od.h / minrows));
        if (o > 0 && per_col * (od.h / SGK_EXT_SEG_MIN) >= 8192)
            nseg = std::min(nseg, std::max(1, od.h / SGK_EXT_SEG_MIN));
        const int rows = (od.h + nseg - 1) / nseg;
        nseg = (od.h + rows - 1) / rows;
        eg.wave0[o] = nw;
        eg.seg_rows[o] = rows;
        eg.nseg[o] = nseg;
        nw += strips_x * nseg * fp.batch;
    }
    eg.wave0[fp.n_octaves] = nw;
    const unsigned nb = (unsigned)((nw + 3) / 4);
    switch ((fp.d + 2) * 2 + (pairs ? 1 : 0)) {
#define SGK_EXTW(ND)                                                                             \
    case 2 * ND: hipLaunchKernelGGL((k_extrema_wave2<ND, 1>), dim3(nb), dim3(256), 0, stream, pyr, \
                                    mask, row_count, fp, eg); break;                             \
    case 2 * ND + 1: hipLaunchKernelGGL((k_extrema_wave2<ND, 2>), dim3(nb), dim3(256), 0, stream,  \
                                        pyr, mask, row_count, fp, eg); break;
        SGK_EXTW(3) SGK_EXTW(4) SGK_EXTW(5) SGK_EXTW(6) SGK_EXTW(7) SGK_EXTW(8)
        default: return hipErrorInvalidValue;
#undef SGK_EXTW
    }
    return hipGetLastError();
}

static size_t scan_blocks(size_t n) { return (n + 1023) / 1024; }

size_t scan_tmp_words(size_t n) {
    size_t words = 0;
    while (n > 1024) {
        size_t nb = scan_blocks(n);
        words += nb + nb + 1;
        n = nb;
    }
    return words + 16;
}

__global__ __launch_bounds__(256) void k_zero(uint32_t* __restrict__ a, size_t na,
                                              uint32_t* __restrict__ b, size_t nb,
                                              uint32_t* __restrict__ c, size_t nc) {
    const size_t step = (size_t)gridDim.x * 256;
    for (size_t q = (size_t)blockIdx.x * 256 + threadIdx.x; q * 4 < na; q += step) zero_words(a, na, q);
    for (size_t q = (size_t)blockIdx.x * 256 + threadIdx.x; q * 4 < nb; q += step) zero_words(b, nb, q);
    for (size_t q = (size_t)blockIdx.x * 256 + threadIdx.x; q * 4 < nc; q += step) zero_words(c, nc, q);
}

hipError_t launch_zero(uint32_t* a, size_t na, uint32_t* b, size_t nb, uint32_t* c, size_t nc,
                       hipStream_t stream) {
    for (const uint32_t* p : {(const uint32_t*)a, (const uint32_t*)b, (const uint32_t*)c})
        if ((uintptr_t)p % 16) return hipErrorInvalidValue;
    if (!a) na = 0;
    if (!b) nb = 0;
    if (!c) nc = 0;
    const size_t quads = (std::max(na, std::max(nb, nc)) + 3) / 4;
    if (quads == 0) return hipSuccess;
    const unsigned grid = (unsigned)std::min<size_t>((quads + 255) / 256, 4096);
    hipLaunchKernelGGL(k_zero, dim3(grid), dim3(256), 0, stream, a, na, b, nb, c, nc);
    return hipGetLastError();
}

hipError_t launch_scan(const uint32_t* in, uint32_t* out, size_t n, uint32_t* tmp,
                       hipStream_t stream) {
    if (n <= 1024) {
        hipLaunchKernelGGL(k_scan_block, dim3(1), dim3(256), 0, stream, in, out, n,
                           (uint32_t*)nullptr);
        return hipGetLastError();
    }
    if (n <= 32768) {
        hipLaunchKernelGGL(k_scan_single, dim3(1), dim3(1024), 0, stream, in, out, n);
        return hipGetLastError();
    }
    const size_t nb = scan_blocks(n);
    uint32_t* sums = tmp;
    uint32_t* sums_scan = tmp + nb;
    hipLaunchKernelGGL(k_scan_block, dim3((unsigned)nb), dim3(256), 0, stream, in, out, n, sums);
    hipError_t e = launch_scan(sums, sums_scan, nb, tmp + nb + nb + 1, stream);
    if (e != hipSuccess) return e;
    hipLaunchKernelGGL(k_scan_add, dim3((unsigned)nb), dim3(256), 0, stream, out, n, sums_scan);
    return hipGetLastError();
}

hipError_t launch_limit_rows(uint32_t* row_count, const FeatureParams& fp, int threshold,
                             int method, hipStream_t stream) {
    if (fp.n_octaves * fp.d > kMaxLimitLevels) return hipErrorInvalidValue;
    hipLaunchKernelGGL(k_limit_rows, dim3(fp.batch), dim3(256), 0, stream, row_count, fp,
                       threshold, method);
    return hipGetLastError();
}

hipError_t launch_limit_oriented(uint32_t* ocount, const uint32_t* row_base,
                                 const FeatureParams& fp, int threshold, int method,
                                 uint32_t cand_cap, hipStream_t stream) {
    if (fp.n_octaves * fp.d > kMaxLimitLevels) return hipErrorInvalidValue;
    hipLaunchKernelGGL(k_limit_oriented, dim3(fp.batch), dim3(256), 0, stream, ocount, row_base,
                       fp, threshold, method, cand_cap);
    return hipGetLastError();
}

}
```

modify-sift-gpu_amd/csrc/sift_kernels.h:

```cpp
#pragma once
#include <hip/hip_runtime.h>
#include <stdint.h>

namespace sgk {

constexpr int kMaxLevels = 16;
constexpr int kMaxOctaves = 16;

struct Taps { float k[33]; };

struct OctaveDesc {
    int w, h, wa;
    int nwords;
    long long gauss_off;
    long long level_stride;
    long long mask_off;
    long long mask_level_stride;
};

struct FeatureParams {
    int batch, n_octaves, d;
    int rows_per_image;
    int row_off[kMaxOctaves];
    float level_sigma[kMaxLevels];
    float sigma_step;
    float t0, t, edge;
    float gaussian_factor, sample_factor;
    float window_factor;
    int subpixel, num_orientation, keep_sign, circular, normalize;
    float origin_offset;
    int octave_min;
    int unit_input;
    OctaveDesc oct[kMaxOctaves];
};

struct ZeroJob {
    uint32_t* p[3] = {nullptr, nullptr, nullptr};
    size_t n[3] = {0, 0, 0};
};

hipError_t launch_gauss(const float* src, const uint8_t* src_u8, int src_stride,
                        long long src_img_stride, float* dst, long long dst_img_stride,
                        int w, int h, int fw, const Taps& taps, int batch,
                        float* ds_dst, int ds_w, int ds_h, long long ds_img_stride,
                        hipStream_t stream, int wave_rows = -1, bool long_bands = false,
                        const ZeroJob& zero = ZeroJob{});

struct LevelOp {
    const float* src;
    const uint8_t* src_u8;
    int src_stride;
    long long src_img_stride;
    float* dst;
    long long dst_img_stride;
    int w, h, fw;
    Taps taps;
    int batch;
    float* ds_dst;
    int ds_w, ds_h;
    long long ds_img_stride;
    ZeroJob zero;
};
hipError_t launch_gauss_op(const LevelOp& op, hipStream_t stream, int wave_rows,
                           bool long_bands = false);
hipError_t launch_gauss_two(const LevelOp& a, const LevelOp& b, hipStream_t stream, int wave_rows,
                            bool long_bands = false, int* launches = nullptr);

constexpr size_t kGaussDuoTrashBytes = 1024 * 3072;
constexpr int kDuoStripsRule = 0, kDuoStripsWave = 1, kDuoStripsCoop = 2;
bool gauss_duo_supported(const LevelOp& a, const LevelOp& b);
hipError_t launch_gauss_duo(const LevelOp& a, const LevelOp& b, hipStream_t stream, int rows_hint,
                            float* trash, int strips = kDuoStripsRule);

constexpr size_t kGaussTrioTrashBytes = 1024 * 4096;
bool gauss_trio_supported(const LevelOp& a, const LevelOp& b, const LevelOp& c);
hipError_t launch_gauss_trio(const LevelOp& a, const LevelOp& b, const LevelOp& c,
                             hipStream_t stream, int rows_hint, float* trash);

bool gauss_tile_supported(const LevelOp& op);
hipError_t launch_gauss_tile(const LevelOp& op, hipStream_t stream);
hipError_t launch_gauss_tile_two(const LevelOp& a, const LevelOp& b, hipStream_t stream,
                                 int* launches = nullptr);
bool gauss_tile_duo_supported(const LevelOp& a, const LevelOp& b);
hipError_t launch_gauss_tile_duo(const LevelOp& a, const LevelOp& b, hipStream_t stream);
hipError_t launch_gauss_tile_duo_one(const LevelOp& a, const LevelOp& b, const LevelOp& c,
                                     hipStream_t stream, int* launches = nullptr);

hipError_t launch_first_octave_input(const float* src, const uint8_t* src_u8, int stride,
                                     long long src_img_stride, int tw, int h, int fo, float* dst,
                                     int dw, int dh, long long dst_img_stride, int batch,
                                     hipStream_t stream);

hipError_t launch_color_to_gray(const uint8_t* src, int n, int w, int h, int stride,
                                int channels, bool bgr, float* dst, hipStream_t stream);

hipError_t launch_extrema(const float* pyr, uint32_t* mask, uint32_t* row_count,
                          const FeatureParams& fp, hipStream_t stream, bool tiles = false);

size_t scan_tmp_words(size_t n);
hipError_t launch_zero(uint32_t* a, size_t na, uint32_t* b, size_t nb, uint32_t* c, size_t nc,
                       hipStream_t stream);
hipError_t launch_scan(const uint32_t* in, uint32_t* out, size_t n, uint32_t* tmp,
                       hipStream_t stream);

constexpr int kQueueCounters = 8;
constexpr int kQueueStride = 32;
constexpr size_t kFeatureQueueWords = 2 * kQueueCounters * kQueueStride;
constexpr size_t feature_queue_base(size_t n_cand_cap) {
    return (n_cand_cap + kQueueStride - 1) / kQueueStride * kQueueStride;
}
struct FeatureQueue {
    uint32_t* next = nullptr;
    int ori_grid = 0;
    int desc_grid = 0;
    int desc_waves = 1;
};
hipError_t feature_queue_grids(FeatureQueue* q);

hipError_t launch_orientation(const float* pyr, const uint32_t* mask, const uint32_t* row_base,
                              int total_rows, const uint32_t* n_cand_dev, int n_cand_cap,
                              int grid_hint, const FeatureParams& fp, float4* out4, int2* info,
                              uint32_t* ocount, hipStream_t stream,
                              bool wave_per_candidate = false,
                              const FeatureQueue* queue = nullptr);

struct ImageOffsetsArgs {
    const uint32_t* row_base = nullptr;
    int batch = 0, rows_per_image = 0, total_rows = 0;
    int64_t* off = nullptr;
};
hipError_t launch_expand(const float4* cand, const int2* info, const uint32_t* eoff,
                         const uint32_t* n_cand_dev, int n_cand_cap, const FeatureParams& fp,
                         float4* feat, int2* feat_info, float4* keys, hipStream_t stream,
                         const ImageOffsetsArgs* io = nullptr);

hipError_t launch_copy_out(const float4* keys, const float* desc, const uint32_t* n_dev, int cap,
                           const int64_t* rec, int rec_n, float* hkeys, float* hdesc,
                           int64_t* hrec, hipStream_t stream);

struct HostCopy {
    const float4* keys = nullptr;
    const int64_t* rec = nullptr;
    int rec_n = 0;
    uint32_t cap = 0;
    float4* hkeys = nullptr;
    float* hdesc = nullptr;
    int64_t* hrec = nullptr;
};
struct DescriptorForm {
    const int* out_index = nullptr;
    bool rect = false;
    bool exact = false;
    bool dual = false;
    bool wide = false;
    const HostCopy* host = nullptr;
    const FeatureQueue* queue = nullptr;
};
hipError_t launch_descriptor(const float* pyr, const float4* feat, const int2* feat_info,
                             const uint32_t* n_feat_dev, int n_feat_cap, const FeatureParams& fp,
                             float* desc, const DescriptorForm& form, hipStream_t stream);

hipError_t launch_orient_keys(const float* pyr, float4* feat, const int2* feat_info,
                              const int* index, int n, const FeatureParams& fp, float4* keys_out,
                              hipStream_t stream);

hipError_t launch_limit_rows(uint32_t* row_count, const FeatureParams& fp, int threshold,
                             int method, hipStream_t stream);
hipError_t launch_limit_oriented(uint32_t* ocount, const uint32_t* row_base,
                                 const FeatureParams& fp, int threshold, int method,
                                 uint32_t cand_cap, hipStream_t stream);


typedef hipError_t (*DebugCandidatesFn)(const float* pyr, const uint32_t* mask,
                                        const uint32_t* row_base, int total_rows,
                                        const uint32_t* n_cand_dev, int n_cand_cap,
                                        const FeatureParams* fp, int4* ints, float4* floats,
                                        hipStream_t stream);

constexpr int kDistTable = 262145;
struct Top2 { int max, idx, second; };
hipError_t launch_to_s8(const uint8_t* src, int n, uint8_t* dst, hipStream_t stream);
struct PrepSet {
    const uint8_t* src;
    int n;
    uint8_t* dst;
    int* sums = nullptr;
    int scale = 128;
    int bias = 0;
    int* zero = nullptr;
    int nzero = 0;
    int* ctp = nullptr;
    int* ctfill = nullptr;
};
hipError_t launch_prep_set(const PrepSet& p, hipStream_t stream);
int match_ct_pad();
int match_chunks(int nA, int nB, bool dma = false);
struct MatchRows {
    const uint8_t* A;
    int nA;
    const uint8_t* B;
    int nB;
    int chunks;
    Top2* part;
    bool row_side = true;
    const uint8_t* mask = nullptr;
    const int* row_term = nullptr;
    Top2* colpart = nullptr;
    bool raw = false;
    const int* amap = nullptr;
    const int* an = nullptr;
    const int* ctp = nullptr;
    const int* bn = nullptr;
};
hipError_t launch_match_rows(const MatchRows& r, hipStream_t stream);
size_t match_part_bound(int nA, int nB, bool dma = false);
int match_panels(int nA);
hipError_t launch_match_cols(const Top2* colpart, int n, int panels, const int* col_term,
                             const float* dist, float distmax, float ratiomax, int* out,
                             Top2* best, hipStream_t stream);
struct GuidedParams { float H[9]; float F[9]; float hdistmax, fdistmax; };
size_t guided_mask_bytes(int nA, int nB);
hipError_t launch_guided_mask(const float* loc1, int n1, const float* loc2, int n2,
                              const GuidedParams& gp, uint8_t* rec1, uint8_t* rec2,
                              hipStream_t stream);
struct ColumnList {
    int* flag = nullptr;
    int* list = nullptr;
    int* count = nullptr;
    const int* map = nullptr;
    int dma = 0;
    int* rmax = nullptr;
    int* ntau = nullptr;
    const int* bmap = nullptr;
    const int* bn = nullptr;
};
hipError_t launch_prune_set(const int* rmax, const int* ntau, int n, const uint8_t* s8,
                            const int* ct, uint8_t* s8c, int* ctc, int* mapc, int* countc,
                            hipStream_t stream);
struct MatchFinish {
    const Top2* part;
    int n;
    int chunks;
    const int* row_term;
    const float* dist;
    float distmax;
    float ratiomax;
    int* out;
    bool row_side = true;
    Top2* best = nullptr;
    const uint8_t* raw_A = nullptr;
    const uint8_t* raw_B = nullptr;
    int nB = 0;
    ColumnList cl{};
};
hipError_t launch_match_finish(const MatchFinish& f, hipStream_t stream);

}

namespace sgplan {
struct Item;
struct Side;
struct FinishPanel;
struct PairRec;
}
namespace sgeo {
struct PairRec;
struct Item;
}

namespace sgk {
hipError_t launch_quantize_desc(const float* d, size_t n, uint8_t* u8, uint8_t* s8, int* sums,
                                hipStream_t stream);
hipError_t launch_match_pairs(const uint8_t* s8, const sgplan::Item* items, int nitems, Top2* part,
                              hipStream_t stream);
hipError_t launch_match_pairs_guided(const uint8_t* s8, const sgplan::Item* items, int nitems,
                                     Top2* part, const float* loc, int loc_stride,
                                     const GuidedParams* geom, hipStream_t stream);
hipError_t launch_match_pairs_finish(const Top2* part, const sgplan::Side* sides,
                                     const sgplan::FinishPanel* fpanels, int nfpanels,
                                     const int* sums, const float* dist, float distmax,
                                     float ratiomax, int* dec, hipStream_t stream);
hipError_t launch_match_pairs_compact(const int* dec, const sgplan::PairRec* pairs, int npairs,
                                      int max_match, long long cap, int* counts, long long* offs,
                                      int* out, hipStream_t stream);

hipError_t launch_estimate_gather(const float* loc, int loc_stride, const sgeo::PairRec* pairs,
                                  int npairs, const int* matches, long long total, float4* pts,
                                  hipStream_t stream);
hipError_t launch_estimate_pairs(const float4* pts, const sgeo::PairRec* pairs,
                                 const sgeo::Item* items, int nitems, int model, float threshold,
                                 int iterations, uint32_t seed, unsigned long long* slots,
                                 hipStream_t stream);
hipError_t launch_estimate_finish(const float4* pts, const sgeo::PairRec* pairs, int npairs,
                                  int model, float threshold, uint32_t seed,
                                  const unsigned long long* slots, float* models, int* inliers,
                                  uint8_t* mask, int* err, hipStream_t stream);
hipError_t launch_estimate_refine(const float4* pts, const sgeo::PairRec* pairs, int npairs,
                                  int model, float threshold, int rounds, float* models,
                                  int* inliers, uint8_t* mask, int* rounds_done, hipStream_t stream);

hipError_t launch_verify_pair_recs(const long long* offs, const int* counts, int npairs,
                                   sgeo::PairRec* recs, hipStream_t stream);
hipError_t launch_verify_gather(const float* loc, int loc_stride, const sgeo::PairRec* pairs,
                                int npairs, const int* matches, const long long* total,
                                long long bound, float4* pts, hipStream_t stream);
hipError_t launch_verify_estimate_pairs(const float4* pts, const sgeo::PairRec* pairs,
                                        const sgeo::Item* items, int nitems, int model,
                                        float threshold, int iterations, uint32_t seed,
                                        unsigned long long* slots, hipStream_t stream);
hipError_t launch_verify_guided_params(const float* H, const float* F, float hdistmax,
                                       float fdistmax, int npairs, GuidedParams* geom,
                                       hipStream_t stream);

hipError_t launch_select_top_scale(const float* scale, int stride, const long long* set_off,
                                   const int* sub_off, int nsets, int top, int* index,
                                   hipStream_t stream);
hipError_t launch_gather_rows(const uint8_t* src, const int* src_terms, const long long* set_off,
                              const int* sub_off, const int* index, int nsets, uint8_t* dst,
                              int* dst_terms, hipStream_t stream);
hipError_t launch_remap_matches(const int* counts, const long long* offs, const int* pair_sub,
                                const int* index, int npairs, long long cap, int* out,
                                hipStream_t stream);
}
```

modify-sift-gpu_amd/csrc/sift_keys.h:

```cpp
#pragma once

namespace sgk {
namespace {

struct KeyOut { float result, dx, dy, ds; };

template <class Get>
__device__ __forceinline__ KeyOut key_test(Get get, float t0, float t, float edge, int subpixel) {
    KeyOut o{0.f, 0.f, 0.f, 0.f};
    const float v = get(1, 1, 1);
    if (fabs_(v) <= t0) return o;
    const float l = get(1, 1, 0), r = get(1, 1, 2);
    float nmax = fmax_(l, r), nmin = fmin_(l, r);
    if (v <= nmax && v >= nmin) return o;
    const int seq_m[8] = {1, 1, 0, 0, 0, 2, 2, 2};
    const int seq_r[8] = {0, 2, 0, 1, 2, 0, 1, 2};
#pragma unroll
    for (int s = 0; s < 8; s++) {
        if (s == 2) {
            const float vx2 = v * 2.0f;
            const float fxx = l + r - vx2;
            const float fyy = get(1, 0, 1) + get(1, 2, 1) - vx2;
            const float fxy = 0.25f * (get(1, 2, 2) + get(1, 0, 0) - get(1, 2, 0) - get(1, 0, 2));
            const float temp1 = fma_(fxx, fyy, -(fxy * fxy));
            const float temp2 = (fxx + fyy) * (fxx + fyy);
            if (temp1 <= 0 || temp2 > edge * temp1) return o;
        }
        const float a = get(seq_m[s], seq_r[s], 0), bb = get(seq_m[s], seq_r[s], 1),
                    cc = get(seq_m[s], seq_r[s], 2);
        if (v > nmax) {
            nmax = fmax_(fmax_(fmax_(nmax, a), bb), cc);
            if (v < nmax) return o;
        } else {
            nmin = fmin_(fmin_(fmin_(nmin, a), bb), cc);
            if (v > nmin) return o;
        }
    }
    bool ok = true;
    float dx = 0.f, dy = 0.f, ds = 0.f;
    if (subpixel) {
        const float vx2 = v * 2.0f;
        const float fxx = l + r - vx2;
        const float fyy = get(1, 0, 1) + get(1, 2, 1) - vx2;
        const float fxy = 0.25f * (get(1, 2, 2) + get(1, 0, 0) - get(1, 2, 0) - get(1, 0, 2));
        const float fx = 0.5f * (r - l);
        const float fy = 0.5f * (get(1, 2, 1) - get(1, 0, 1));
        const float pc = get(0, 1, 1), nc = get(2, 1, 1);
        const float fs = 0.5f * (nc - pc);
        const float fss = (nc + pc - vx2);
        const float fxs = 0.25f * (get(2, 1, 2) + get(0, 1, 0) - get(2, 1, 0) - get(0, 1, 2));
        const float fys = 0.25f * (get(2, 2, 1) + get(0, 0, 1) - get(2, 0, 1) - get(0, 2, 1));
        float4 A0 = fxx > 0 ? make_float4(fxx, fxy, fxs, -fx) : make_float4(-fxx, -fxy, -fxs, fx);
        float4 A1 = fxy > 0 ? make_float4(fxy, fyy, fys, -fy) : make_float4(-fxy, -fyy, -fys, fy);
        float4 A2 = fxs > 0 ? make_float4(fxs, fys, fss, -fs) : make_float4(-fxs, -fys, -fss, fs);
        const float maxa = fmax_(fmax_(A0.x, A1.x), A2.x);
        if ((double)maxa >= 1e-10) {
            if (maxa == A1.x) { float4 T = A1; A1 = A0; A0 = T; }
            else if (maxa == A2.x) { float4 T = A2; A2 = A0; A0 = T; }
            A0.y /= A0.x; A0.z /= A0.x; A0.w /= A0.x;
            A1.y = fma_(-A1.x, A0.y, A1.y); A1.z = fma_(-A1.x, A0.z, A1.z); A1.w = fma_(-A1.x, A0.w, A1.w);
            A2.y = fma_(-A2.x, A0.y, A2.y); A2.z = fma_(-A2.x, A0.z, A2.z); A2.w = fma_(-A2.x, A0.w, A2.w);
            if (fabs_(A2.y) > fabs_(A1.y)) { float4 T = A2; A2 = A1; A1 = T; }
            if ((double)fabs_(A1.y) >= 1e-10) {
                A1.z /= A1.y; A1.w /= A1.y;
                A2.z = fma_(-A2.y, A1.z, A2.z); A2.w = fma_(-A2.y, A1.w, A2.w);
                if ((double)fabs_(A2.z) >= 1e-10) {
                    ds = A2.w / A2.z;
                    dy = fma_(-ds, A1.z, A1.w);
                    dx = fma_(-dy, A0.y, fma_(-ds, A0.z, A0.w));
                    const float dot = fma_(ds, fs, fma_(dx, fx, dy * fy));
                    ok = fabs_(fma_(0.5f, dot, v)) > t && fabs_(ds) < 1.0f &&
                         fabs_(dx) < 1.0f && fabs_(dy) < 1.0f;
                }
            }
        }
    }
    if (ok) o.result = v > nmax ? 1.0f : -1.0f;
    o.dx = dx; o.dy = dy; o.ds = ds;
    return o;
}

struct KeyLoc { int b, o, j, row, col; };

__device__ __forceinline__ KeyLoc row_loc(int lo, const FeatureParams& fp) {
    KeyLoc L;
    L.b = lo / fp.rows_per_image;
    int rem = lo - L.b * fp.rows_per_image;
    int o = 0;
    while (o + 1 < fp.n_octaves && fp.row_off[o + 1] <= rem) o++;
    L.o = o;
    rem -= fp.row_off[o];
    const OctaveDesc& od = fp.oct[o];
    L.j = rem / od.h;
    L.row = rem - L.j * od.h;
    L.col = 0;
    return L;
}

__device__ __forceinline__ KeyLoc locate(uint32_t f, const uint32_t* __restrict__ row_base,
                                         int total_rows, const uint32_t* __restrict__ mask,
                                         const FeatureParams& fp) {
    int lo = 0, hi = total_rows;
    while (hi - lo > 1) {
        int mid = (lo + hi) >> 1;
        if (row_base[mid] <= f) lo = mid; else hi = mid;
    }
    KeyLoc L = row_loc(lo, fp);
    uint32_t k = f - row_base[lo];
    const OctaveDesc& od = fp.oct[L.o];
    const uint32_t* mrow = mask + od.mask_off + L.j * od.mask_level_stride +
                           ((long long)L.b * od.h + L.row) * od.nwords;
    int col = 0;
    for (int w = 0; w < od.nwords; w++) {
        uint32_t m = mrow[w];
        uint32_t c = __popc(m);
        if (k < c) {
            for (uint32_t q = 0; q < k; q++) m &= m - 1;
            col = w * 32 + (__ffs(m) - 1);
            break;
        }
        k -= c;
    }
    L.col = col;
    return L;
}

__device__ __forceinline__ KeyOut key_at(const float* __restrict__ pyr, const FeatureParams& fp,
                                         const KeyLoc& L) {
    const OctaveDesc& od = fp.oct[L.o];
    const long long npx = (long long)od.wa * od.h;
    const float* g = pyr + od.gauss_off + (long long)L.b * npx + (long long)L.row * od.wa + L.col;
    auto get = [&](int m, int r, int c) {
        const long long p = (long long)(r - 1) * od.wa + (c - 1);
        const float* gm = g + (long long)(L.j + m) * od.level_stride;
        return gm[od.level_stride + p] - gm[p];
    };
    return key_test(get, fp.t0, fp.t, fp.edge, fp.subpixel);
}

}
}
```

modify-sift-gpu_amd/python/sgpu.py:

```python
from __future__ import annotations

import contextlib
import ctypes
import os
import subprocess

import numpy as np

from sgpu_types import SgpuOptions, SgpuVerifyParams, default_options

PKG = os.path.dirname(os.path.dirname(os.path.abspath(__file__)))
LIB_PATH = os.environ.get("SGPU_LIB_PATH") or os.path.join(PKG, "lib", "libsiftgpu.so")

SGPU_OK, SGPU_EINVAL, SGPU_ENODEV, SGPU_ENOMEM, SGPU_ERANGE = 0, -1, -2, -3, -4
SGPU_INPUT_HOST, SGPU_INPUT_DEVICE, SGPU_INPUT_STAGED = 0, 1, 2

C_API = [
    "sgpu_default_options", "sgpu_parse_args", "sgpu_ctx_create", "sgpu_ctx_destroy",
    "sgpu_ctx_set_options", "sgpu_last_error", "sgpu_device_count", "sgpu_extract",
    "sgpu_extract_f32", "sgpu_stage_input", "sgpu_feature_count", "sgpu_feature_total", "sgpu_copy_features",
    "sgpu_device_features", "sgpu_match", "sgpu_quantize_descriptors", "sgpu_last_timing",
    "sgpu_debug_geometry", "sgpu_debug_gaussian", "sgpu_debug_candidates",
    "sgpu_debug_set_flags", "sgpu_comm_unique_id", "sgpu_comm_init", "sgpu_comm_allgather_i32",
    "sgpu_comm_allreduce_f64", "sgpu_extract_keypoints", "sgpu_match_guided", "sgpu_extract_color",
    "sgpu_match_shard_begin", "sgpu_match_shard_end", "sgpu_match_sharded",
    "sgpu_extract_stream", "sgpu_host_alloc", "sgpu_host_free", "sgpu_reserve",
    "sgpu_debug_alloc_count", "sgpu_last_pyramid_launches", "sgpu_set_stage_timing",
    "sgpu_set_host_output", "sgpu_debug_set_schedule", "sgpu_debug_set_match_prune",
    "sgpu_quantize_descriptors_gpu", "sgpu_feature_descriptors_u8", "sgpu_copy_features_u8",
    "sgpu_match_batch", "sgpu_match_images", "sgpu_debug_match_plan_stats",
    "sgpu_debug_set_duo_strips", "sgpu_debug_pyramid_plan", "sgpu_debug_set_feature_queue",
    "sgpu_match_batch_guided", "sgpu_match_images_guided",
    "sgpu_estimate_batch", "sgpu_estimate_images",
    "sgpu_estimate_batch_refined", "sgpu_estimate_images_refined",
    "sgpu_default_verify_params", "sgpu_verify_batch", "sgpu_verify_images",
    "sgpu_select_top_scale_batch", "sgpu_select_top_scale_images",
    "sgpu_prematch_batch", "sgpu_prematch_images",
]

PLAN_KINDS = ("level", "tile", "two", "tile_two", "tile_duo", "tile_duo_one", "duo", "trio")

_LIB = None


def build():
    subprocess.check_call(["make", "-C", PKG, "-j8"])


def lib():
    global _LIB
    if _LIB is None:
        if not os.path.exists(LIB_PATH):
            raise RuntimeError(f"{LIB_PATH} missing: build it with `make -C {PKG}`")
        L = ctypes.CDLL(LIB_PATH)
        P, c = ctypes.POINTER, ctypes
        vp = c.c_void_p
        L.sgpu_default_options.argtypes = [P(SgpuOptions)]
        L.sgpu_parse_args.argtypes = [P(SgpuOptions), c.c_int, P(c.c_char_p), P(c.c_int)]
        L.sgpu_ctx_create.argtypes = [c.c_int, P(SgpuOptions), P(vp)]
        L.sgpu_ctx_destroy.argtypes = [vp]
        L.sgpu_ctx_set_options.argtypes = [vp, P(SgpuOptions)]
        L.sgpu_last_error.argtypes = [vp]
        L.sgpu_last_error.restype = c.c_char_p
        L.sgpu_extract.argtypes = [vp, vp, c.c_int, c.c_int, c.c_int, c.c_int, c.c_int]
        L.sgpu_stage_input.argtypes = [vp, vp, c.c_int, c.c_int, c.c_int, c.c_int]
        L.sgpu_reserve.argtypes = [vp, c.c_int, c.c_int, c.c_int, c.c_int]
        L.sgpu_debug_alloc_count.argtypes = []
        L.sgpu_debug_alloc_count.restype = c.c_longlong
        L.sgpu_last_pyramid_launches.argtypes = [vp, P(c.c_int)]
        L.sgpu_set_stage_timing.argtypes = [vp, c.c_int]
        L.sgpu_set_host_output.argtypes = [vp, vp, vp, c.c_int]
        L.sgpu_extract_f32.argtypes = [vp, vp, c.c_int, c.c_int, c.c_int, c.c_int, c.c_int]
        L.sgpu_feature_count.argtypes = [vp, c.c_int]
        L.sgpu_feature_total.argtypes = [vp]
        L.sgpu_feature_total.restype = c.c_int64
        L.sgpu_copy_features.argtypes = [vp, c.c_int, vp, vp]
        L.sgpu_device_features.argtypes = [vp, P(vp), P(vp), P(vp)]
        L.sgpu_match.argtypes = [vp, vp, c.c_int, vp, c.c_int, c.c_float, c.c_float, c.c_int,
                                 c.c_int, vp, c.c_int]
        L.sgpu_match_guided.argtypes = [vp, vp, c.c_int, vp, c.c_int, vp, vp, vp, vp, c.c_float,
                                        c.c_float, c.c_float, c.c_float, c.c_int, c.c_int, vp,
                                        c.c_int]
        L.sgpu_extract_color.argtypes = [vp, vp, c.c_int, c.c_int, c.c_int, c.c_int, c.c_int, c.c_int]
        L.sgpu_quantize_descriptors.argtypes = [vp, c.c_size_t, vp]
        L.sgpu_last_timing.argtypes = [vp, vp, c.c_int]
        L.sgpu_debug_set_flags.argtypes = [vp, c.c_int]
        L.sgpu_debug_set_schedule.argtypes = [vp, c.c_int, c.c_int]
        L.sgpu_debug_set_match_prune.argtypes = [vp, c.c_int]
        L.sgpu_debug_set_duo_strips.argtypes = [vp, c.c_int]
        L.sgpu_debug_set_feature_queue.argtypes = [vp, c.c_int]
        L.sgpu_debug_geometry.argtypes = [vp, P(c.c_int), vp, c.c_int]
        L.sgpu_debug_gaussian.argtypes = [vp, c.c_int, c.c_int, c.c_int, vp]
        L.sgpu_debug_candidates.argtypes = [vp, vp, vp, c.c_int, P(c.c_int)]
        L.sgpu_extract_keypoints.argtypes = [vp, c.c_int, vp, c.c_int, c.c_int]
        L.sgpu_comm_unique_id.argtypes = [vp, c.c_int]
        L.sgpu_comm_init.argtypes = [vp, c.c_int, c.c_int, vp, c.c_int]
        L.sgpu_comm_allgather_i32.argtypes = [vp, vp, c.c_int, vp]
        L.sgpu_comm_allreduce_f64.argtypes = [vp, vp, c.c_int, c.c_int]
        L.sgpu_match_shard_begin.argtypes = [vp, vp, c.c_int, c.c_int, vp, c.c_int, c.c_float,
                                             c.c_float, c.c_int, vp, vp, c.c_int]
        L.sgpu_match_shard_end.argtypes = [vp, c.c_int, c.c_int, vp, c.c_int, c.c_int, c.c_float,
                                           c.c_float, c.c_int, c.c_int, vp]
        L.sgpu_match_sharded.argtypes = [vp, vp, c.c_int, c.c_int, vp, c.c_int, c.c_float,
                                         c.c_float, c.c_int, c.c_int, vp, c.c_int]
        L.sgpu_extract_stream.argtypes = [vp, P(vp), c.c_int, c.c_int, c.c_int, c.c_int, c.c_int,
                                          vp, vp, c.c_int64, vp]
        L.sgpu_host_alloc.argtypes = [c.c_size_t]
        L.sgpu_host_alloc.restype = vp
        L.sgpu_host_free.argtypes = [vp]
        L.sgpu_quantize_descriptors_gpu.argtypes = [vp, vp, c.c_size_t, vp, c.c_int]
        L.sgpu_feature_descriptors_u8.argtypes = [vp, P(vp)]
        L.sgpu_copy_features_u8.argtypes = [vp, c.c_int, vp]
        L.sgpu_match_batch.argtypes = [vp, vp, vp, c.c_int, vp, c.c_int, c.c_float, c.c_float,
                                       c.c_int, c.c_int, vp, c.c_int64, vp, c.c_int]
        L.sgpu_match_images.argtypes = [vp, vp, c.c_int, c.c_float, c.c_float, c.c_int, c.c_int,
                                        vp, c.c_int64, vp]
        L.sgpu_match_batch_guided.argtypes = [vp, vp, vp, vp, c.c_int, vp, c.c_int, vp, vp,
                                              c.c_float, c.c_float, c.c_float, c.c_float,
                                              c.c_int, c.c_int, vp, c.c_int64, vp, c.c_int]
        L.sgpu_match_images_guided.argtypes = [vp, vp, c.c_int, vp, vp, c.c_float, c.c_float,
                                               c.c_float, c.c_float, c.c_int, c.c_int, vp,
                                               c.c_int64, vp]
        L.sgpu_estimate_batch.argtypes = [vp, vp, vp, c.c_int, vp, c.c_int, vp, vp, c.c_int,
                                          c.c_float, c.c_int, c.c_uint32, vp, vp, vp, c.c_int]
        L.sgpu_estimate_images.argtypes = [vp, vp, c.c_int, vp, vp, c.c_int, c.c_float, c.c_int,
                                           c.c_uint32, vp, vp, vp]
        L.sgpu_estimate_batch_refined.argtypes = [vp, vp, vp, c.c_int, vp, c.c_int, vp, vp,
                                                  c.c_int, c.c_float, c.c_int, c.c_uint32,
                                                  c.c_int, vp, vp, vp, vp, c.c_int]
        L.sgpu_estimate_images_refined.argtypes = [vp, vp, c.c_int, vp, vp, c.c_int, c.c_float,
                                                   c.c_int, c.c_uint32, c.c_int, vp, vp, vp, vp]
        L.sgpu_default_verify_params.argtypes = [P(SgpuVerifyParams)]
        L.sgpu_default_verify_params.restype = None
        L.sgpu_verify_batch.argtypes = [vp, vp, vp, vp, c.c_int, vp, c.c_int, P(SgpuVerifyParams),
                                        vp, vp, vp, vp, vp, vp, c.c_int64, vp, c.c_int]
        L.sgpu_verify_images.argtypes = [vp, vp, c.c_int, P(SgpuVerifyParams), vp, vp, vp, vp, vp,
                                         vp, c.c_int64, vp]
        L.sgpu_select_top_scale_batch.argtypes = [vp, vp, c.c_int, vp, c.c_int, c.c_int, vp, vp,
                                                  c.c_int]
        L.sgpu_select_top_scale_images.argtypes = [vp, c.c_int, vp, vp]
        L.sgpu_prematch_batch.argtypes = [vp, vp, vp, c.c_int, vp, c.c_int, vp, c.c_int, c.c_int,
                                          c.c_float, c.c_float, c.c_int, vp, vp, c.c_int64, c.c_int]
        L.sgpu_prematch_images.argtypes = [vp, vp, c.c_int, c.c_int, c.c_float, c.c_float, c.c_int,
                                           vp, vp, c.c_int64]
        L.sgpu_debug_match_plan_stats.argtypes = [vp, vp]
        L.sgpu_debug_pyramid_plan.argtypes = [vp, vp, c.c_int]
        _LIB = L
    return _LIB


class PinnedArray:

    def __init__(self, shape, dtype):
        dt = np.dtype(dtype)
        n = int(np.prod(shape)) * dt.itemsize
        self._p = lib().sgpu_host_alloc(max(n, 1))
        if not self._p:
            raise MemoryError(f"sgpu_host_alloc({n}) failed")
        buf = (ctypes.c_uint8 * max(n, 1)).from_address(self._p)
        self.array = np.frombuffer(buf, dtype=dt, count=int(np.prod(shape))).reshape(shape)

    def free(self):
        if self._p:
            self.array = None
            lib().sgpu_host_free(self._p)
            self._p = None

    def __del__(self):
        self.free()


def match_shard_end(col_best_all: np.ndarray, row_match: np.ndarray, row_begin: int,
                    distmax=0.7, ratiomax=0.8, mbm=1, max_match=None) -> np.ndarray:
    cb = np.ascontiguousarray(col_best_all, np.int32)
    if cb.ndim == 2:
        cb = cb[None]
    rm = np.ascontiguousarray(row_match, np.int32)
    ns, n2 = len(rm), cb.shape[1]
    max_match = ns if max_match is None else max_match
    out = np.zeros((max(max_match, 1), 2), np.int32)
    m = lib().sgpu_match_shard_end(cb.ctypes.data, cb.shape[0], n2, rm.ctypes.data, ns,
                                   row_begin, distmax, ratiomax, mbm, max_match, out.ctypes.data)
    if m < 0:
        raise RuntimeError(f"sgpu_match_shard_end failed ({m})")
    return out[:m].copy()


def comm_unique_id() -> bytes:
    buf = (ctypes.c_uint8 * 128)()
    rc = lib().sgpu_comm_unique_id(buf, 128)
    if rc != SGPU_OK:
        raise RuntimeError(f"sgpu_comm_unique_id failed ({rc})")
    return bytes(buf)


def device_count() -> int:
    return lib().sgpu_device_count()


def quantize(desc: np.ndarray) -> np.ndarray:
    d = np.ascontiguousarray(desc, np.float32)
    out = np.empty(d.shape, np.uint8)
    lib().sgpu_quantize_descriptors(d.ctypes.data, d.size, out.ctypes.data)
    return out


def quantize_gpu(desc: np.ndarray, ctx: "SiftContext | None" = None) -> np.ndarray:
    own = ctx is None
    if own:
        ctx = SiftContext(0)
    try:
        return ctx.quantize_gpu(desc)
    finally:
        if own:
            ctx.close()


class MatchOverflow(RuntimeError):

    def __init__(self, counts, matches):
        super().__init__(f"{int(counts.sum())} matches exceed cap")
        self.counts = counts
        self.matches = matches


class SiftContext:

    def __init__(self, device: int = 0, opts: SgpuOptions | None = None):
        self.opts = opts or default_options()
        self.device = device
        self._ctx = ctypes.c_void_p()
        rc = lib().sgpu_ctx_create(device, ctypes.byref(self.opts), ctypes.byref(self._ctx))
        if rc != SGPU_OK:
            raise RuntimeError(f"sgpu_ctx_create(device={device}) failed with {rc}: "
                               "no usable gfx950 device")
        self.batch = 0

    def close(self):
        if self._ctx:
            lib().sgpu_ctx_destroy(self._ctx)
            self._ctx = ctypes.c_void_p()

    def __del__(self):
        try:
            self.close()
        except Exception:
            pass

    def _check(self, rc, what):
        if rc != SGPU_OK:
            raise RuntimeError(f"{what} failed ({rc}): {lib().sgpu_last_error(self._ctx).decode()}")

    def set_options(self, opts: SgpuOptions):
        self.opts = opts
        self._check(lib().sgpu_ctx_set_options(self._ctx, ctypes.byref(opts)), "set_options")

    def reserve(self, n: int, w: int, h: int):
        self._check(lib().sgpu_reserve(self._ctx, n, w, h, w), "sgpu_reserve")
        self._staged = None
        self.batch = 0
        return self

    def pyramid_launches(self):
        f = ctypes.c_int(0)
        n = lib().sgpu_last_pyramid_launches(self._ctx, ctypes.byref(f))
        if n < 0:
            raise RuntimeError("sgpu_last_pyramid_launches: no extract")
        return int(n), int(f.value)

    def pyramid_plan(self):
        n = lib().sgpu_debug_pyramid_plan(self._ctx, None, 0)
        if n < 0:
            raise RuntimeError("sgpu_debug_pyramid_plan: no extract")
        out = np.zeros((n, 7), np.int32)
        self._check(min(0, lib().sgpu_debug_pyramid_plan(self._ctx, out.ctypes.data, out.size)),
                    "sgpu_debug_pyramid_plan")
        return [(PLAN_KINDS[int(e[0])], [(int(e[1 + 2 * j]), int(e[2 + 2 * j]))
                                         for j in range(3) if e[1 + 2 * j] >= 0]) for e in out]

    def set_stage_timing(self, on: bool):
        self._check(lib().sgpu_set_stage_timing(self._ctx, int(bool(on))), "sgpu_set_stage_timing")

    @staticmethod
    def alloc_count() -> int:
        return int(lib().sgpu_debug_alloc_count())

    @staticmethod
    def _padded(images, stride, shape, dtype, channels=1):
        if stride is None:
            a = np.ascontiguousarray(images, dtype)
            if a.ndim == (2 if channels == 1 else 3):
                a = a[None]
            if a.ndim != (3 if channels == 1 else 4):
                raise ValueError(f"images must be [n, h, w{'' if channels == 1 else ', c'}], got {a.shape}")
            n, h, w = a.shape[:3]
            if channels != 1 and a.shape[3] != channels:
                raise ValueError("channel count does not match the format")
            return a, n, h, w, w * channels
        if shape is None:
            raise ValueError("a row stride needs shape=(n, h, w)")
        n, h, w = (int(v) for v in shape)
        a = np.ascontiguousarray(images, dtype).reshape(-1)
        stride = int(stride)
        if stride < w * channels or a.size < n * h * stride:
            raise ValueError(f"{a.size} elements do not hold {n} x {h} rows {stride} apart "
                             f"of {w * channels}")
        return a, n, h, w, stride

    def stage(self, images: np.ndarray, stride=None, shape=None):
        a, n, h, w, stride = self._padded(images, stride, shape, np.uint8)
        self._check(lib().sgpu_stage_input(self._ctx, a.ctypes.data, n, w, h, stride), "stage")
        self._staged = (n, h, w, stride)
        return self

    def extract_staged(self):
        n, h, w, stride = self._staged
        self._check(lib().sgpu_extract(self._ctx, None, n, w, h, stride, SGPU_INPUT_STAGED),
                    "sgpu_extract(staged)")
        self.batch = n
        return self

    def extract(self, images: np.ndarray | int, shape=None, device_ptr=False, stride=None,
                dtype=None):
        if device_ptr:
            n, h, w, stride = shape
            dt = np.dtype(np.uint8 if dtype is None else dtype)
        else:
            dt = np.dtype(np.asarray(images).dtype if dtype is None else dtype)
        if dt not in (np.dtype(np.uint8), np.dtype(np.float32)):
            raise TypeError(dt)
        fn = lib().sgpu_extract if dt == np.uint8 else lib().sgpu_extract_f32
        if device_ptr:
            rc = fn(self._ctx, ctypes.c_void_p(images), n, w, h, stride, SGPU_INPUT_DEVICE)
        else:
            a, n, h, w, stride = self._padded(images, stride, shape, dt)
            rc = fn(self._ctx, a.ctypes.data, n, w, h, stride, SGPU_INPUT_HOST)
        self._check(rc, "sgpu_extract")
        self.batch = n
        return self

    COLOR_FORMATS = {"rgb": 1, "bgr": 2, "rgba": 3, "bgra": 4}

    def extract_color(self, images: np.ndarray | int, fmt: str = "rgb", stride=None, shape=None,
                      device_ptr=False):
        c = 3 if fmt in ("rgb", "bgr") else 4
        if device_ptr:
            n, h, w, stride = shape
            rc = lib().sgpu_extract_color(self._ctx, ctypes.c_void_p(images), n, w, h, stride,
                                          self.COLOR_FORMATS[fmt], SGPU_INPUT_DEVICE)
        else:
            a, n, h, w, stride = self._padded(images, stride, shape, np.uint8, c)
            rc = lib().sgpu_extract_color(self._ctx, a.ctypes.data, n, w, h, stride,
                                          self.COLOR_FORMATS[fmt], SGPU_INPUT_HOST)
        self._check(rc, "extract_color")
        self.batch = n

    def extract_stream(self, batches, keys=None, desc=None, cap=None, stride=None, shape=None):
        if not len(batches):
            raise ValueError("no batches")
        if stride is None:
            bl = [np.ascontiguousarray(b) for b in batches]
            n, h, w = bl[0].shape
            if any(b.shape != (n, h, w) or b.dtype != np.uint8 for b in bl):
                raise ValueError("batches must be u8 arrays of one shape")
            stride = w
        else:
            if any(np.asarray(b).dtype != np.uint8 for b in batches):
                raise ValueError("batches must be u8 buffers")
            bl = [self._padded(b, stride, shape, np.uint8)[0] for b in batches]
            n, h, w = (int(v) for v in shape)
            stride = int(stride)
        want_desc = bool(self.opts.descriptors)

        def check_out(a, width, name):
            if (not isinstance(a, np.ndarray) or a.dtype != np.float32 or a.ndim != 2 or
                    a.shape[1] != width or not a.flags.c_contiguous or not a.flags.writeable):
                raise ValueError(f"{name} must be a writable C-contiguous float32 [cap, {width}]")
        if keys is not None:
            check_out(keys, 4, "keys")
        if desc is not None:
            if not want_desc:
                raise ValueError("descriptors are disabled (-sd): pass desc=None")
            check_out(desc, 128, "desc")
        given = [len(a) for a in (keys, desc) if a is not None]
        if cap is None:
            cap = min(given) if given else 4096 * n * len(bl)
        cap = int(cap)
        if cap < 0 or any(cap > g for g in given):
            raise ValueError(f"cap {cap} exceeds an output array ({given})")
        if keys is None:
            keys = np.zeros((cap, 4), np.float32)
        if desc is None and want_desc:
            desc = np.zeros((cap, 128), np.float32)
# ... 244 lines not shown
        return out if rounds is None else out + (done[:npairs].copy(),)

    def estimate_batch(self, loc: np.ndarray, offsets, pairs, matches, model="H", threshold=2.0,
                       iterations=512, seed=0, device_ptr=None):
        off, nsets, lc, ptr, flags = self._estimate_sets(loc, offsets, device_ptr)

        def call(pr, npairs, cat, counts, mdl, thr, it, sd, models, inliers, mask):
            return lib().sgpu_estimate_batch(self._ctx, ptr, off.ctypes.data, nsets, pr, npairs, cat,
                                             counts, mdl, thr, it, sd, models, inliers, mask, flags)
        return self._estimate(call, pairs, matches, model, threshold, iterations, seed)

    @staticmethod
    def _estimate_sets(loc, offsets, device_ptr):
        off = np.ascontiguousarray(offsets, np.int64)
        nsets = len(off) - 1
        if device_ptr is not None:
            return off, nsets, None, ctypes.c_void_p(device_ptr), SGPU_INPUT_DEVICE
        lc = np.ascontiguousarray(loc, np.float32)
        if lc.ndim != 2 or lc.shape[1] != 2 or nsets < 0 or (len(off) and off[-1] > len(lc)):
            raise ValueError(f"locations must be [rows][2] covering the offsets, got {lc.shape}")
        return off, nsets, lc, (lc.ctypes.data if len(lc) else None), SGPU_INPUT_HOST

    def estimate_batch_refined(self, loc: np.ndarray, offsets, pairs, matches, model="H",
                               threshold=2.0, iterations=512, seed=0, rounds=3, device_ptr=None):
        off, nsets, lc, ptr, flags = self._estimate_sets(loc, offsets, device_ptr)

        def call(pr, npairs, cat, counts, mdl, thr, it, sd, models, inliers, mask, budget, done):
            return lib().sgpu_estimate_batch_refined(self._ctx, ptr, off.ctypes.data, nsets, pr,
                                                     npairs, cat, counts, mdl, thr, it, sd, budget,
                                                     models, inliers, mask, done, flags)
        return self._estimate(call, pairs, matches, model, threshold, iterations, seed, rounds)

    def estimate_images_refined(self, pairs, matches, model="H", threshold=2.0, iterations=512,
                                seed=0, rounds=3):
        def call(pr, npairs, cat, counts, mdl, thr, it, sd, models, inliers, mask, budget, done):
            return lib().sgpu_estimate_images_refined(self._ctx, pr, npairs, cat, counts, mdl, thr,
                                                      it, sd, budget, models, inliers, mask, done)
        return self._estimate(call, pairs, matches, model, threshold, iterations, seed, rounds)

    def estimate_images(self, pairs, matches, model="H", threshold=2.0, iterations=512, seed=0):
        def call(pr, npairs, cat, counts, mdl, thr, it, sd, models, inliers, mask):
            return lib().sgpu_estimate_images(self._ctx, pr, npairs, cat, counts, mdl, thr, it, sd,
                                              models, inliers, mask)
        return self._estimate(call, pairs, matches, model, threshold, iterations, seed)

    @staticmethod
    def verify_params(**params) -> SgpuVerifyParams:
        vp = SgpuVerifyParams()
        lib().sgpu_default_verify_params(ctypes.byref(vp))
        names = {f[0] for f in SgpuVerifyParams._fields_}
        for k, v in params.items():
            if k not in names:
                raise TypeError(f"unknown verify parameter {k!r}")
            setattr(vp, k, int(v) & 0xFFFFFFFF if k == "seed" else v)
        return vp

    def _verify(self, call, pairs, sizes, H, F, cap, params):
        if not H and not F:
            raise ValueError("verify needs a model: H, F or both (match_batch matches without one)")
        vp = self.verify_params(**params)
        pr = np.ascontiguousarray(pairs, np.int32).reshape(-1, 2)
        npairs = len(pr)
        cap = self._default_cap(pr[:, 0], sizes, vp.max_match) if cap is None else int(cap)
        out = np.zeros((max(cap, 1), 2), np.int32)
        counts = np.zeros(max(npairs, 1), np.int32)
        putative = np.zeros(max(npairs, 1), np.int32)
        models = [np.zeros((max(npairs, 1), 9), np.float32) if want else None for want in (H, F)]
        inliers = [np.zeros(max(npairs, 1), np.int32) if want else None for want in (H, F)]
        ptr = lambda a: None if a is None else a.ctypes.data
        rc = call(pr.ctypes.data if npairs else None, npairs, ctypes.byref(vp), ptr(models[0]),
                  ptr(inliers[0]), ptr(models[1]), ptr(inliers[1]), putative.ctypes.data,
                  out.ctypes.data, cap, counts.ctypes.data)
        ms = [None if m is None else m[:npairs].reshape(npairs, 3, 3).copy() for m in models]
        ins = [None if i is None else i[:npairs].copy() for i in inliers]
        rest = (ms[0], ins[0], ms[1], ins[1], putative[:npairs].copy())
        return (self._fitting(rc, "verify", out, counts[:npairs], cap, rest),) + rest

    def verify_batch(self, desc_u8, loc, offsets, pairs, H=True, F=False, cap=None,
                     device_ptrs=None, **params):
        off = np.ascontiguousarray(offsets, np.int64)
        nsets = len(off) - 1
        if device_ptrs is not None:
            dp, lp = (ctypes.c_void_p(a) for a in device_ptrs)
            flags = SGPU_INPUT_DEVICE
            if nsets < 0:
                raise ValueError("offsets must hold at least one entry")
        else:
            d = np.ascontiguousarray(desc_u8, np.uint8).reshape(-1, 128)
            lc = np.ascontiguousarray(loc, np.float32)
            if lc.ndim != 2 or lc.shape != (len(d), 2):
                raise ValueError(f"locations must be [rows][2] for {len(d)} rows, got {lc.shape}")
            if nsets < 0 or (len(off) and off[-1] > len(d)):
                raise ValueError("offsets do not fit the descriptor buffer")
            dp, lp = (d.ctypes.data if len(d) else None), (lc.ctypes.data if len(lc) else None)
            flags = SGPU_INPUT_HOST

        def call(pr, npairs, vp, *outs):
            return lib().sgpu_verify_batch(self._ctx, dp, lp, off.ctypes.data, nsets, pr, npairs, vp,
                                           *outs, flags)
        return self._verify(call, pairs, np.diff(off), H, F, cap, params)

    def verify_images(self, pairs, H=True, F=False, cap=None, **params):
        if not H and not F:
            raise ValueError("verify needs a model: H, F or both (match_images matches without one)")
        sizes = np.array([self.count(i) for i in range(self.batch)], np.int64)

        def call(pr, npairs, vp, *outs):
            return lib().sgpu_verify_images(self._ctx, pr, npairs, vp, *outs)
        return self._verify(call, pairs, sizes, H, F, cap, params)

    def verify_time(self) -> float:
        t = np.zeros(14, np.float32)
        lib().sgpu_last_timing(self._ctx, t.ctypes.data, 14)
        return float(t[13])

    @staticmethod
    def _set_offsets(offsets):
        off = np.ascontiguousarray(offsets, np.int64).reshape(-1)
        if len(off) < 1:
            raise ValueError("offsets must hold at least one entry")
        return off, len(off) - 1

    @staticmethod
    def _scales(scale, off, stride):
        sc = np.ascontiguousarray(scale, np.float32).reshape(-1)
        stride = int(stride)
        rows = int(off[-1])
        if stride < 1 or (rows > 0 and len(sc) < (rows - 1) * stride + 1):
            raise ValueError(f"{len(sc)} floats do not hold {rows} scales {stride} apart")
        return sc, stride

    @staticmethod
    def _split(flat, offs):
        return [flat[offs[s]:offs[s + 1]].copy() for s in range(len(offs) - 1)]

    def select_top_scale(self, scale, offsets, top, stride=1, device_ptr=None):
        off, nsets = self._set_offsets(offsets)
        if device_ptr is not None:
            ptr, flags, stride = ctypes.c_void_p(device_ptr), SGPU_INPUT_DEVICE, int(stride)
        else:
            sc, stride = self._scales(scale, off, stride)
            ptr, flags = (sc.ctypes.data if len(sc) else None), SGPU_INPUT_HOST
        sizes = np.diff(off)
        cap = int(np.minimum(sizes, max(int(top), 0)).clip(0).sum()) if (sizes >= 0).all() else 0
        index = np.zeros(max(cap, 1), np.int32)
        sub = np.zeros(nsets + 1, np.int64)
        self._check(lib().sgpu_select_top_scale_batch(self._ctx, ptr, stride, off.ctypes.data, nsets,
                                                      int(top), index.ctypes.data, sub.ctypes.data,
                                                      flags), "sgpu_select_top_scale_batch")
        return self._split(index, sub)

    def select_top_scale_images(self, top):
        cap = sum(min(self.count(i), max(int(top), 0)) for i in range(self.batch))
        index = np.zeros(max(cap, 1), np.int32)
        sub = np.zeros(self.batch + 1, np.int64)
        self._check(lib().sgpu_select_top_scale_images(self._ctx, int(top), index.ctypes.data,
                                                       sub.ctypes.data), "sgpu_select_top_scale_images")
        return self._split(index, sub)

    def _prematch(self, call, pairs, sizes, top, matches, cap):
        nsets, top = len(sizes), int(top)
        if pairs is None:
            a, b = np.triu_indices(nsets, 1)
            first, npairs, ptr = a, len(a), None
        else:
            pr = np.ascontiguousarray(pairs, np.int32).reshape(-1, 2)
            npairs = len(pr)
            first = pr[:, 0]
            keep = pr if npairs else np.zeros((1, 2), np.int32)
            ptr = keep.ctypes.data
        counts = np.zeros(max(npairs, 1), np.int32)
        out = None
        if matches:
            cap = self._default_cap(first, sizes, top) if cap is None else int(cap)
            out = np.zeros((max(cap, 1), 2), np.int32)
        rc = call(ptr, npairs, counts.ctypes.data, None if out is None else out.ctypes.data,
                  cap if matches else 0)
        counts = counts[:npairs]
        if not matches:
            if rc < 0 and rc != SGPU_ERANGE:
                self._check(rc, "prematch")
            return counts.copy(), None
        return counts.copy(), self._fitting(rc, "prematch", out, counts, cap)

    def prematch_batch(self, desc_u8, scale, offsets, pairs=None, top=100, distmax=0.7, ratiomax=0.8,
                       mbm=1, matches=True, cap=None, stride=1, device_ptrs=None):
        off, nsets = self._set_offsets(offsets)
        if device_ptrs is not None:
            dp, sp = (ctypes.c_void_p(a) for a in device_ptrs)
            flags, stride = SGPU_INPUT_DEVICE, int(stride)
        else:
            d = np.ascontiguousarray(desc_u8, np.uint8).reshape(-1, 128)
            if off[-1] > len(d):
                raise ValueError("offsets do not fit the descriptor buffer")
            sc, stride = self._scales(scale, off, stride)
            dp, sp = (d.ctypes.data if len(d) else None), (sc.ctypes.data if len(sc) else None)
            flags = SGPU_INPUT_HOST

        def call(pr, npairs, counts, out, cp):
            return lib().sgpu_prematch_batch(self._ctx, dp, sp, stride, off.ctypes.data, nsets, pr,
                                             npairs, int(top), distmax, ratiomax, mbm, counts, out,
                                             cp, flags)
        return self._prematch(call, pairs, np.diff(off), top, matches, cap)

    def prematch_images(self, pairs=None, top=100, distmax=0.7, ratiomax=0.8, mbm=1, matches=True,
                        cap=None):
        sizes = np.array([self.count(i) for i in range(self.batch)], np.int64)

        def call(pr, npairs, counts, out, cp):
            return lib().sgpu_prematch_images(self._ctx, pr, npairs, int(top), distmax, ratiomax, mbm,
                                              counts, out, cp)
        return self._prematch(call, pairs, sizes, top, matches, cap)

    def candidate_pairs(self, top=100, min_matches=4, distmax=0.7, ratiomax=0.8, mbm=1):
        counts, _ = self.prematch_images(None, top, distmax, ratiomax, mbm, matches=False)
        a, b = np.triu_indices(self.batch, 1)
        keep = counts >= int(min_matches)
        return np.stack([a[keep], b[keep]], axis=1).astype(np.int32).reshape(-1, 2), counts[keep]

    def prematch_time(self) -> float:
        t = np.zeros(15, np.float32)
        lib().sgpu_last_timing(self._ctx, t.ctypes.data, 15)
        return float(t[14])

    def match_guided(self, d1: np.ndarray, d2: np.ndarray, loc1: np.ndarray, loc2: np.ndarray,
                     H=None, F=None, distmax=0.7, ratiomax=0.8, hdistmax=32.0, fdistmax=16.0,
                     mbm=1, max_match=None, device_ptrs=None):
        if device_ptrs is not None:
            p1, n1, p2, n2, q1, q2 = device_ptrs
            flags = SGPU_INPUT_DEVICE
        else:
            d1 = np.ascontiguousarray(d1, np.uint8)
            d2 = np.ascontiguousarray(d2, np.uint8)
            l1 = np.ascontiguousarray(loc1, np.float32)
            l2 = np.ascontiguousarray(loc2, np.float32)
            n1, n2 = d1.shape[0], d2.shape[0]
            if l1.shape != (n1, 2) or l2.shape != (n2, 2):
                raise ValueError("locations must be [n][2] per descriptor set")
            p1, p2, q1, q2 = d1.ctypes.data, d2.ctypes.data, l1.ctypes.data, l2.ctypes.data
            flags = SGPU_INPUT_HOST
        hm = None if H is None else np.ascontiguousarray(H, np.float32).reshape(9)
        fm = None if F is None else np.ascontiguousarray(F, np.float32).reshape(9)
        max_match = n1 if max_match is None else max_match
        out = np.zeros((max(max_match, 1), 2), np.int32)
        m = lib().sgpu_match_guided(
            self._ctx, ctypes.c_void_p(p1), n1, ctypes.c_void_p(p2), n2, ctypes.c_void_p(q1),
            ctypes.c_void_p(q2),
            None if hm is None else hm.ctypes.data, None if fm is None else fm.ctypes.data,
            distmax, ratiomax, hdistmax, fdistmax, mbm, max_match, out.ctypes.data, flags)
        if m < 0:
            self._check(m, "sgpu_match_guided")
        return out[:m]

    def comm_init(self, nranks: int, rank: int, uid: bytes):
        buf = (ctypes.c_uint8 * len(uid)).from_buffer_copy(uid)
        self._check(lib().sgpu_comm_init(self._ctx, nranks, rank, buf, len(uid)), "sgpu_comm_init")

    def allgather_i32(self, send: np.ndarray, nranks: int) -> np.ndarray:
        a = np.ascontiguousarray(send, np.int32)
        out = np.zeros(a.size * nranks, np.int32)
        self._check(lib().sgpu_comm_allgather_i32(self._ctx, a.ctypes.data, a.size, out.ctypes.data),
                    "sgpu_comm_allgather_i32")
        return out

    def allreduce_f64(self, v, op_max: bool) -> np.ndarray:
        a = np.ascontiguousarray(np.atleast_1d(v), np.float64).copy()
        self._check(lib().sgpu_comm_allreduce_f64(self._ctx, a.ctypes.data, a.size, 1 if op_max else 0),
                    "sgpu_comm_allreduce_f64")
        return a

    DEBUG_PARTS2, DEBUG_PARTS4, DEBUG_TINY_CAP, DEBUG_FUSED_MATCH = 1, 2, 4, 8
    DEBUG_EXACT_DESCRIPTOR = 16
    DEBUG_GAUSS_BLOCK = 32
    DEBUG_BAND_SHIFT = 20
    DEBUG_KEYED_MATCH = 64
    DEBUG_FULL_COLUMNS = 128
    DEBUG_DESC_DUAL = 256
    DEBUG_ORIENT_WAVE = 512
    DEBUG_GAUSS_TILE_ALWAYS = 1024
    DEBUG_MATCH_REGSTAGE = 2048
    DEBUG_PYR_SERIAL = 4096
    DEBUG_GAUSS_LONG_BANDS = 8192
    DEBUG_DUO_ALWAYS = 16384
    DEBUG_DUO_OFF = 32768
    DEBUG_GAUSS_TILE_OFF = 65536
    DEBUG_DESC_WIDE_OFF = 131072
    DEBUG_DESC_WIDE_ALWAYS = 262144
    DEBUG_EXTREMA_TILE_OFF = 524288

    def set_debug_flags(self, flags: int):
        self._check(lib().sgpu_debug_set_flags(self._ctx, flags), "sgpu_debug_set_flags")

    TRIO_OFF, TRIO_ON, TRIO_ALWAYS = 0, 1, 2
    PAIRS_FRONT, PAIRS_END = 0, 1

    def set_schedule(self, trio: int = 0, pairs: int = 1):
        self._check(lib().sgpu_debug_set_schedule(self._ctx, trio, pairs), "sgpu_debug_set_schedule")

    STRIPS_RULE, STRIPS_WAVE, STRIPS_COOP = 0, 1, 2

    def set_duo_strips(self, mode: int = 0):
        self._check(lib().sgpu_debug_set_duo_strips(self._ctx, mode), "sgpu_debug_set_duo_strips")

    FEATURES_QUEUE, FEATURES_STATIC_ORIENTATION, FEATURES_STATIC_DESCRIPTOR, FEATURES_STATIC = 0, 1, 2, 3

    def set_feature_queue(self, mode: int = 0):
        self._check(lib().sgpu_debug_set_feature_queue(self._ctx, mode), "sgpu_debug_set_feature_queue")

    def set_match_prune(self, on: bool = True):
        self._check(lib().sgpu_debug_set_match_prune(self._ctx, int(bool(on))),
                    "sgpu_debug_set_match_prune")

    def match_plan_stats(self):
        out = np.zeros(4, np.int64)
        self._check(lib().sgpu_debug_match_plan_stats(self._ctx, out.ctypes.data),
                    "sgpu_debug_match_plan_stats")
        return dict(zip(["items", "sides", "max_tiles", "max_chunks"], out.tolist()))

    @contextlib.contextmanager
    def exact_descriptors(self):
        self.set_debug_flags(self.DEBUG_EXACT_DESCRIPTOR)
        try:
            yield self
        finally:
            self.set_debug_flags(0)

    def geometry(self):
        n = ctypes.c_int(0)
        dims = np.zeros(48, np.int32)
        lib().sgpu_debug_geometry(self._ctx, ctypes.byref(n), dims.ctypes.data, 16)
        return [tuple(dims[3 * i:3 * i + 3]) for i in range(n.value)]

    def gaussian(self, image, octave, level):
        w, h, wa = self.geometry()[octave]
        out = np.zeros(wa * h, np.float32)
        self._check(lib().sgpu_debug_gaussian(self._ctx, image, octave, level, out.ctypes.data),
                    "sgpu_debug_gaussian")
        return out

    def candidates(self):
        n = ctypes.c_int(0)
        lib().sgpu_debug_candidates(self._ctx, None, None, 0, ctypes.byref(n))
        ints = np.zeros((max(n.value, 1), 4), np.int32)
        fl = np.zeros((max(n.value, 1), 4), np.float32)
        self._check(lib().sgpu_debug_candidates(self._ctx, ints.ctypes.data, fl.ctypes.data,
                                                n.value, ctypes.byref(n)), "sgpu_debug_candidates")
        return ints[:n.value], fl[:n.value]
```

Measured before the change: 18990.

## Compute the top Gaussian level lazily, only at surviving top-scale extrema candidates

```diff
diff --git a/include/sgpu.h b/include/sgpu.h
--- a/include/sgpu.h
+++ b/include/sgpu.h
@@ -213,6 +213,10 @@
 #define SGPU_DUO_STRIPS_WAVE 1
 #define SGPU_DUO_STRIPS_COOP 2
 int sgpu_debug_set_duo_strips(sgpu_ctx* ctx, int mode);
+#define SGPU_TOP_LEVEL_RULE 0
+#define SGPU_TOP_LEVEL_DENSE 1
+#define SGPU_TOP_LEVEL_LAZY 2
+int sgpu_debug_set_top_level(sgpu_ctx* ctx, int mode);
 int sgpu_debug_set_match_prune(sgpu_ctx* ctx, int on);
 int sgpu_debug_match_plan_stats(const sgpu_ctx* ctx, long long out[4]);
 #define SGPU_PLAN_ENTRY_INTS 7
@@ -229,6 +233,7 @@
 int sgpu_debug_geometry(const sgpu_ctx* ctx, int* n_octaves, int* dims , int max);
 int sgpu_debug_gaussian(sgpu_ctx* ctx, int image, int octave, int level, float* out);
 int sgpu_debug_candidates(sgpu_ctx* ctx, int* ints, float* floats, int cap, int* n);
+int sgpu_debug_top_level_at(sgpu_ctx* ctx, int image, int octave, int x, int y, float out[9]);
 
 typedef struct sgpu_verify_params {
     float distmax, ratiomax;
diff --git a/modify-sift-gpu_amd/csrc/sgpu_capi.cpp b/modify-sift-gpu_amd/csrc/sgpu_capi.cpp
--- a/modify-sift-gpu_amd/csrc/sgpu_capi.cpp
+++ b/modify-sift-gpu_amd/csrc/sgpu_capi.cpp
@@ -52,6 +52,10 @@
     if (const char* ev = getenv("SGPU_DUO_PLAN")) {
         if (!strcmp(ev, "end")) ctx->duo_plan = SGPU_PAIRS_END;
         if (!strcmp(ev, "front")) ctx->duo_plan = SGPU_PAIRS_FRONT;
+    }
+    if (const char* ev = getenv("SGPU_TOP_LEVEL")) {
+        if (!strcmp(ev, "dense")) ctx->top_level = SGPU_TOP_LEVEL_DENSE;
+        if (!strcmp(ev, "lazy")) ctx->top_level = SGPU_TOP_LEVEL_LAZY;
     }
     if (const char* ev = getenv("SGPU_TRIO")) {
         if (!strcmp(ev, "off")) ctx->trio_mode = SGPU_TRIO_OFF;
@@ -381,6 +385,12 @@
     return SGPU_OK;
 }
 
+int sgpu_debug_set_top_level(sgpu_ctx* ctx, int mode) {
+    if (!ctx || mode < SGPU_TOP_LEVEL_RULE || mode > SGPU_TOP_LEVEL_LAZY) return SGPU_EINVAL;
+    ctx->top_level = mode;
+    return SGPU_OK;
+}
+
 int sgpu_debug_geometry(const sgpu_ctx* ctx, int* n_octaves, int* dims, int max) {
     if (!ctx || !n_octaves) return SGPU_EINVAL;
     *n_octaves = (int)ctx->oct.size();
@@ -397,29 +407,68 @@
         octave >= (int)ctx->oct.size() || level < 0 || level >= ctx->sched.level_num)
         return SGPU_EINVAL;
     HIPCHK(ctx, hipSetDevice(ctx->device));
-    const Part& pt = ctx->part[ctx->part_of(image)];
+    Part& pt = ctx->part[ctx->part_of(image)];
     const sgk::OctaveDesc& od = pt.fp.oct[octave];
     const long long npx = (long long)od.wa * od.h;
+    if (level == ctx->sched.level_num - 1 && (size_t)octave < pt.top_dense.size() &&
+        !pt.top_dense[octave]) {
+        HIPCHK(ctx, sgk::launch_gauss_op(pt.top_ops[octave], ctx->stream, 0));
+        HIPCHK(ctx, hipStreamSynchronize(ctx->stream));
+        pt.top_dense[octave] = 1;
+    }
     const float* src = pt.pyr.as<float>() + od.gauss_off + level * od.level_stride +
                        (image - pt.img0) * npx;
     HIPCHK(ctx, hipMemcpy(out, src, npx * sizeof(float), hipMemcpyDeviceToHost));
     return SGPU_OK;
 }
 
-static sgk::DebugCandidatesFn debug_candidates_hook() {
-    static sgk::DebugCandidatesFn fn = [] {
+static void* debug_library() {
+    static void* lib = []() -> void* {
         Dl_info info{};
         if (!dladdr(reinterpret_cast<void*>(&sgpu_debug_candidates), &info) || !info.dli_fname)
-            return (sgk::DebugCandidatesFn) nullptr;
+            return nullptr;
         std::string path(info.dli_fname);
         const size_t slash = path.rfind('/');
         path = (slash == std::string::npos ? std::string(".") : path.substr(0, slash)) +
                "/libsiftgpu_debug.so";
-        void* h = dlopen(path.c_str(), RTLD_NOW | RTLD_LOCAL);
-        return h ? reinterpret_cast<sgk::DebugCandidatesFn>(dlsym(h, "sgpu_testhook_candidates"))
-                 : (sgk::DebugCandidatesFn) nullptr;
+        return dlopen(path.c_str(), RTLD_NOW | RTLD_LOCAL);
     }();
+    return lib;
+}
+static void* debug_symbol(const char* name) {
+    void* h = debug_library();
+    return h ? dlsym(h, name) : nullptr;
+}
+static sgk::DebugCandidatesFn debug_candidates_hook() {
+    static sgk::DebugCandidatesFn fn =
+        reinterpret_cast<sgk::DebugCandidatesFn>(debug_symbol("sgpu_testhook_candidates"));
     return fn;
+}
+
+int sgpu_debug_top_level_at(sgpu_ctx* ctx, int image, int octave, int x, int y, float out[9]) {
+    if (!ctx || !out || image < 0 || image >= ctx->batch || ctx->img_off.empty() || octave < 0 ||
+        octave >= (int)ctx->oct.size())
+        return SGPU_EINVAL;
+    const Part& pt = ctx->part[ctx->part_of(image)];
+    const sgk::OctaveDesc& od = pt.fp.oct[octave];
+    if (x < 1 || x > od.wa - 2 || y < 1 || y > od.h - 2 || (size_t)octave >= pt.top_ops.size())
+        return ctx->fail(SGPU_EINVAL, "point outside the octave's interior");
+    const sgk::DebugTopLevelFn hook = reinterpret_cast<sgk::DebugTopLevelFn>(debug_symbol("sgpu_testhook_top_level"));
+    if (!hook) return ctx->fail(SGPU_EINVAL, "test-hook library lib/libsiftgpu_debug.so not found");
+    HIPCHK(ctx, hipSetDevice(ctx->device));
+    DevBuf d;
+    ALLOCCHK(ctx, d.ensure(9 * sizeof(float)));
+    sgk::TopLevelFilter tf;
+    tf.fw = pt.top_ops[octave].fw;
+    tf.taps = pt.top_ops[octave].taps;
+    hipError_t e = hook(pt.pyr.as<float>(), &pt.fp, &tf, image - pt.img0, octave, x, y,
+                        d.as<float>(), ctx->stream);
+    if (e == hipSuccess)
+        e = hipMemcpyAsync(out, d.p, 9 * sizeof(float), hipMemcpyDeviceToHost, ctx->stream);
+    if (e == hipSuccess) e = hipStreamSynchronize(ctx->stream);
+    d.release();
+    HIPCHK(ctx, e);
+    return SGPU_OK;
 }
 
 int sgpu_debug_candidates(sgpu_ctx* ctx, int* ints, float* floats, int cap, int* n) {
diff --git a/modify-sift-gpu_amd/csrc/sgpu_ctx.h b/modify-sift-gpu_amd/csrc/sgpu_ctx.h
--- a/modify-sift-gpu_amd/csrc/sgpu_ctx.h
+++ b/modify-sift-gpu_amd/csrc/sgpu_ctx.h
@@ -62,6 +62,9 @@
     std::vector<sgk::LevelOp> ops;
     std::vector<sgpyr::LevelDesc> levels;
     sgpyr::Plan plan;
+    std::vector<sgk::LevelOp> top_ops;
+    std::vector<char> top_dense;
+    bool lazy = false;
     bool events = true;
     bool copied_out = false;
     hipEvent_t ev[10] = {};
@@ -117,6 +120,7 @@
     bool duo_u8 = false;
     int trio_mode = SGPU_TRIO_OFF;
     int duo_plan = SGK_DUO_PLAN;
+    int top_level = SGPU_TOP_LEVEL_RULE;
     int duo_strips = SGPU_DUO_STRIPS_RULE;
     size_t wide_desc_max = SGK_WIDE_DESC_MAX;
     size_t wave_orient_max = sgh::kWaveOrientationMax;
diff --git a/modify-sift-gpu_amd/csrc/sgpu_debug.hip b/modify-sift-gpu_amd/csrc/sgpu_debug.hip
--- a/modify-sift-gpu_amd/csrc/sgpu_debug.hip
+++ b/modify-sift-gpu_amd/csrc/sgpu_debug.hip
@@ -6,6 +6,7 @@
 using namespace sgm;
 
 #include "sift_keys.h"
+#include "sift_top_level.h"
 
 namespace sgk {
 namespace {
@@ -22,7 +23,34 @@
     floats[f] = make_float4(kv.dx, kv.dy, kv.ds, kv.result);
 }
 
+template <int FW>
+__global__ __launch_bounds__(64) void k_debug_top_level(const float* __restrict__ pyr,
+                                                        const FeatureParams fp,
+                                                        const TopLevelFilter tf, int image,
+                                                        int octave, int x, int y,
+                                                        float* __restrict__ out9) {
+    __shared__ TopLds s;
+    const int lane = threadIdx.x;
+    const OctaveDesc& od = fp.oct[octave];
+    const float* src = pyr + od.gauss_off + (long long)(fp.d + 1) * od.level_stride +
+                       (long long)image * od.wa * od.h;
+    float v[TopGeom<FW>::NLD];
+    top_window_load<FW>(src, od.wa, od.h, x, y, lane, v);
+    top_level_eval<FW>(v, tf.taps, s, lane);
+    if (lane < 9) out9[lane] = s.top[lane];
 }
+
+}
+}
+
+extern "C" __attribute__((visibility("default"))) hipError_t sgpu_testhook_top_level(
+    const float* pyr, const sgk::FeatureParams* fp, const sgk::TopLevelFilter* tf, int image,
+    int octave, int x, int y, float* out9, hipStream_t stream) {
+    const bool known = sgk::top_level_dispatch(tf->fw, [&](auto FWC) {
+        hipLaunchKernelGGL((sgk::k_debug_top_level<decltype(FWC)::value>), dim3(1), dim3(64), 0, stream,
+                           pyr, *fp, *tf, image, octave, x, y, out9);
+    });
+    return known ? hipGetLastError() : hipErrorInvalidValue;
 }
 
 extern "C" __attribute__((visibility("default"))) hipError_t sgpu_testhook_candidates(
diff --git a/modify-sift-gpu_amd/csrc/sgpu_extract.cpp b/modify-sift-gpu_amd/csrc/sgpu_extract.cpp
--- a/modify-sift-gpu_amd/csrc/sgpu_extract.cpp
+++ b/modify-sift-gpu_amd/csrc/sgpu_extract.cpp
@@ -87,7 +87,7 @@
 }
 
 static int build_level_ops(sgpu_ctx* ctx, Part& pt, const uint8_t* src8, const float* srcf,
-                           int stride, hipStream_t st) {
+                           int stride, hipStream_t st, bool lazy) {
     const sgpu_options& O = ctx->opt;
     const sgp::Schedule& S = ctx->sched;
     const sgk::FeatureParams& fp = pt.fp;
@@ -104,6 +104,7 @@
     pt.levels.clear();
     pt.ops.reserve((size_t)noct * nlev);
     pt.levels.reserve((size_t)noct * nlev);
+    pt.top_ops.resize((size_t)noct);
     for (int o = 0; o < noct; o++) {
         const sgk::OctaveDesc& od = fp.oct[o];
         const long long npx = (long long)od.wa * od.h;
@@ -160,6 +161,13 @@
                 op.zero.p[2] = pt.ocount.as<uint32_t>();
                 op.zero.n[2] = sgk::feature_queue_base(pt.cand_cap) + sgk::kFeatureQueueWords;
             }
+            if (k == nlev - 1) {
+                pt.top_ops[o] = op;
+                if (lazy) {
+                    pt.ops.pop_back();
+                    continue;
+                }
+            }
             pt.levels.push_back(sgpyr::LevelDesc{o, k, op.fw, op.w, op.h, op.batch, dk,
                                                  op.src_u8 != nullptr,
                                                  (op.zero.n[0] | op.zero.n[1] | op.zero.n[2]) != 0});
@@ -229,7 +237,13 @@
     const float* srcf = is_f32 ? (const float*)src_in + (size_t)pt.img0 * img_elems : nullptr;
 
     float* pyr = pt.pyr.as<float>();
-    const int rc_ops = build_level_ops(ctx, pt, src8, srcf, stride, st);
+    const bool ext_small = 4ll * fp.oct[0].wa * fp.oct[0].h * n <= ((long long)ctx->tile_mb << 20);
+    const bool ext_tiles = !(ctx->debug_flags & SGPU_DEBUG_EXTREMA_TILE_OFF) &&
+                           ((ctx->debug_flags & SGPU_DEBUG_GAUSS_TILE_ALWAYS) || ext_small);
+    pt.lazy = !ext_tiles && ctx->top_level != SGPU_TOP_LEVEL_DENSE &&
+              (ctx->top_level == SGPU_TOP_LEVEL_LAZY || !ext_small);
+    pt.top_dense.assign(ctx->oct.size(), pt.lazy ? 0 : 1);
+    const int rc_ops = build_level_ops(ctx, pt, src8, srcf, stride, st, pt.lazy);
     if (rc_ops != SGPU_OK) return rc_ops;
     const sgpyr::Rules R = pyramid_rules(ctx, pt);
     sgpyr::plan_pyramid(pt.levels.data(), (int)pt.levels.size(), R, OpSupport{pt.ops.data()}, pt.plan);
@@ -270,11 +284,15 @@
     if (!pt.one_stream)
         HIPCHK(ctx, sgk::launch_zero(pt.row_count.as<uint32_t>(), (size_t)pt.total_rows,
                                      pt.mask.as<uint32_t>(), (size_t)moff, nullptr, 0, st));
-    const bool ext_tiles = !(ctx->debug_flags & SGPU_DEBUG_EXTREMA_TILE_OFF) &&
-                           ((ctx->debug_flags & SGPU_DEBUG_GAUSS_TILE_ALWAYS) ||
-                            4ll * fp.oct[0].wa * fp.oct[0].h * n <= ((long long)ctx->tile_mb << 20));
     HIPCHK(ctx, sgk::launch_extrema(pyr, pt.mask.as<uint32_t>(), pt.row_count.as<uint32_t>(),
-                                    fp, st, ext_tiles));
+                                    fp, st, ext_tiles, pt.lazy));
+    if (pt.lazy) {
+        sgk::TopLevelFilter tf;
+        tf.fw = pt.top_ops[0].fw;
+        tf.taps = pt.top_ops[0].taps;
+        HIPCHK(ctx, sgk::launch_extrema_top(pyr, pt.mask.as<uint32_t>(), pt.row_count.as<uint32_t>(),
+                                            fp, tf, st));
+    }
     if (O.feature_count_threshold > 0)
         HIPCHK(ctx, sgk::launch_limit_rows(pt.row_count.as<uint32_t>(), fp,
                                            O.feature_count_threshold, O.truncate_method, st));
diff --git a/modify-sift-gpu_amd/csrc/sift_detect.hip b/modify-sift-gpu_amd/csrc/sift_detect.hip
--- a/modify-sift-gpu_amd/csrc/sift_detect.hip
+++ b/modify-sift-gpu_amd/csrc/sift_detect.hip
@@ -2,6 +2,7 @@
 
 #include "sift_device.h"
 #include "sift_keys.h"
+#include "sift_top_level.h"
 
 #ifndef SGK_EXT2_WAVES
 #define SGK_EXT2_WAVES 1
@@ -35,7 +36,7 @@
     int nseg[kMaxOctaves];
 };
 
-template <int ND, int CPL>
+template <int ND, int CPL, bool LAZY = false>
 __global__ __launch_bounds__(256, SGK_EXT2_WAVES) void k_extrema_wave2(const float* __restrict__ pyr,
                                                        uint32_t* __restrict__ mask,
                                                        uint32_t* __restrict__ row_count,
@@ -45,7 +46,8 @@
     constexpr int TW = 64 * CPL - 2;
     constexpr int RW = 64 * CPL + 2 * CPL + 2;
     constexpr int NJ = ND - 2;
-    __shared__ __attribute__((aligned(8))) float s_ring[4][ND][4][RW];
+    constexpr int NR = LAZY ? ND - 1 : ND;
+    __shared__ __attribute__((aligned(8))) float s_ring[4][NR][4][RW];
     __shared__ uint16_t s_list[4][NJ * 64 * CPL];
     const int lane = threadIdx.x & 63, wave = threadIdx.x >> 6;
     const int gw = (SGK_EXT_XCD == 1 ? xcd_block(blockIdx.x, gridDim.x)
@@ -79,12 +81,12 @@
         const int i = CPL * lane + k, x = xl + k;
         out_col[k] = i >= 1 && i <= TW && x > 0 && x < W - 1;
     }
-    struct Row { float m[ND + 1][CPL]; };
+    struct Row { float m[NR + 1][CPL]; };
     Row rA, rB;
     auto fetch = [&](Row& r, int y) {
         const float* q = g0 + (long long)clampi(y, 0, H - 1) * W + gx;
 #pragma unroll
-        for (int m = 0; m <= ND; m++) {
+        for (int m = 0; m <= NR; m++) {
             if constexpr (CPL == 1) {
                 r.m[m][0] = q[m * lstride];
             } else {
@@ -94,11 +96,11 @@
             }
         }
     };
-    float dog[ND][CPL];
+    float dog[NR][CPL];
     auto put = [&](const Row& r, int y) {
         float* rr = &ring[0][y & 3][CPL * lane + CPL];
 #pragma unroll
-        for (int m = 0; m < ND; m++) {
+        for (int m = 0; m < NR; m++) {
 #pragma unroll
             for (int k = 0; k < CPL; k++) dog[m][k] = r.m[m + 1][k] - r.m[m][k];
             if constexpr (CPL == 1)
@@ -108,10 +110,10 @@
         }
         asm volatile("" ::: "memory");
     };
-    float hx0[ND][CPL], hn0[ND][CPL], hx1[ND][CPL], hn1[ND][CPL], cvx[ND][CPL];
+    float hx0[NR][CPL], hn0[NR][CPL], hx1[NR][CPL], hn1[NR][CPL], cvx[NR][CPL];
     auto rowmm = [&](float (*mx)[CPL], float (*mn)[CPL], float (*cv)[CPL]) {
 #pragma unroll
-        for (int m = 0; m < ND; m++) {
+        for (int m = 0; m < NR; m++) {
             float v[CPL + 2];
 #pragma unroll
             for (int k = 0; k < CPL; k++) v[k + 1] = dog[m][k];
@@ -128,7 +130,7 @@
         }
     };
     auto body = [&](int y) {
-        float hx2[ND][CPL], hn2[ND][CPL], cnx[ND][CPL];
+        float hx2[NR][CPL], hn2[NR][CPL], cnx[NR][CPL];
         rowmm(hx2, hn2, cnx);
         const bool row_ok = y < ye && y > 0 && y < H - 1;
         int ncand = 0;
@@ -139,7 +141,7 @@
                 const float v = cvx[j + 1][k];
                 float mx = hx0[j][k], mn = hn0[j][k];
 #pragma unroll
-                for (int m = j; m < j + 3; m++) {
+                for (int m = j; m < j + 3 && m < NR; m++) {
                     mx = fmax_(mx, fmax_(fmax_(hx0[m][k], hx1[m][k]), hx2[m][k]));
                     mn = fmin_(mn, fmin_(fmin_(hn0[m][k], hn1[m][k]), hn2[m][k]));
                 }
@@ -162,10 +164,12 @@
                 auto get = [&](int m, int r, int c) {
                     return ring[j + m][(y + r - 1) & 3][cl + c - 1 + CPL];
                 };
-                if (key_test(get, fp.t0, fp.t, fp.edge, fp.subpixel).result != 0.f) {
-                    const int xx = x0 - 1 + cl;
-                    uint32_t* mrow = mask + mask_off + j * mask_lstride +
-                                     ((long long)b * H + y) * nwords;
+                const int xx = x0 - 1 + cl;
+                uint32_t* mrow = mask + mask_off + j * mask_lstride + ((long long)b * H + y) * nwords;
+                if (LAZY && j == NJ - 1) {
+                    if (key_test<true>(get, fp.t0, fp.t, fp.edge, fp.subpixel).result != 0.f)
+                        atomicOr(&mrow[xx >> 5], 1u << (xx & 31));
+                } else if (key_test(get, fp.t0, fp.t, fp.edge, fp.subpixel).result != 0.f) {
                     atomicOr(&mrow[xx >> 5], 1u << (xx & 31));
                     atomicAdd(&row_count[(long long)b * fp.rows_per_image + rc_base + j * H + y],
                               1u);
@@ -173,7 +177,7 @@
             }
         }
 #pragma unroll
-        for (int m = 0; m < ND; m++)
+        for (int m = 0; m < NR; m++)
 #pragma unroll
             for (int k = 0; k < CPL; k++) {
                 hx0[m][k] = hx1[m][k]; hn0[m][k] = hn1[m][k];
@@ -302,6 +306,111 @@
     }
 }
 
+constexpr int kTopRows = 8;
+struct ExtremaTopGrid {
+    int unit0[kMaxOctaves + 1];
+};
+
+template <int FW>
+__global__ __launch_bounds__(256) void k_extrema_top(float* __restrict__ pyr,
+                                                     uint32_t* __restrict__ mask,
+                                                     uint32_t* __restrict__ row_count,
+                                                     const FeatureParams fp, const ExtremaTopGrid tg,
+                                                     const TopLevelFilter tf) {
+    using G = TopGeom<FW>;
+    __shared__ TopLds s_all[4];
+    __shared__ uint16_t s_list[4][kTopRows * 64];
+    const int lane = threadIdx.x & 63;
+    const int wave = __builtin_amdgcn_readfirstlane(threadIdx.x >> 6);
+    TopLds& s = s_all[wave];
+    uint16_t* list = s_list[wave];
+    const int jt = fp.d - 1, top = fp.d + 2;
+    const int nwaves = gridDim.x * 4;
+    const int gm = lane / 9, gq = lane - 9 * gm, gr = gq / 3, gc = gq - 3 * gr;
+    for (int u = blockIdx.x * 4 + wave; u < tg.unit0[fp.n_octaves]; u += nwaves) {
+        int o = 0;
+        while (o + 1 < fp.n_octaves && u >= tg.unit0[o + 1]) o++;
+        o = __builtin_amdgcn_readfirstlane(o);
+        const OctaveDesc& od = fp.oct[o];
+        const int W = od.wa, H = od.h, nwords = od.nwords;
+        const long long npx = (long long)W * H, lstride = od.level_stride;
+        const long long rows = (long long)fp.batch * H;
+        const long long r0 = (long long)(u - tg.unit0[o]) * kTopRows;
+        const int b0 = (int)(r0 / H), y0 = (int)(r0 - (long long)b0 * H);
+        uint32_t* mtop = mask + od.mask_off + jt * od.mask_level_stride;
+        float* g0 = pyr + od.gauss_off;
+        struct Px { int b, y, x, k; };
+        auto locate_px = [&](int code) {
+            Px p;
+            p.k = code >> 12;
+            p.x = code & 4095;
+            p.b = b0;
+            p.y = y0 + p.k;
+            while (p.y >= H) { p.y -= H; p.b++; }
+            return p;
+        };
+        for (int w0 = 0; w0 < nwords; w0 += 64) {
+            uint32_t word[kTopRows];
+#pragma unroll
+            for (int k = 0; k < kTopRows; k++)
+                word[k] = (r0 + k < rows && w0 + lane < nwords) ? mtop[(r0 + k) * nwords + w0 + lane] : 0u;
+            for (;;) {
+                int cnt = 0;
+#pragma unroll
+                for (int k = 0; k < kTopRows; k++) {
+                    const bool has = word[k] != 0u;
+                    const unsigned long long bal = __ballot(has);
+                    if (has) {
+                        const int bit = __ffs(word[k]) - 1;
+                        word[k] &= word[k] - 1;
+                        const int pos = cnt + __builtin_amdgcn_mbcnt_hi((uint32_t)(bal >> 32),
+                                                  __builtin_amdgcn_mbcnt_lo((uint32_t)bal, 0u));
+                        list[pos] = (uint16_t)((k << 12) | (lane * 32 + bit));
+                    }
+                    cnt += __popcll(bal);
+                }
+                if (cnt == 0) break;
+                asm volatile("" ::: "memory");
+                float vc[G::NLD], vn[G::NLD], gvc, gvn;
+                auto fetch = [&](int i, float (&v)[G::NLD], float& gv) {
+                    const Px p = locate_px(__builtin_amdgcn_readfirstlane((int)list[i]));
+                    const int x = w0 * 32 + p.x;
+                    const float* g = g0 + (long long)p.b * npx;
+                    top_window_load<FW>(g + (top - 1) * lstride, W, H, x, p.y, lane, v);
+                    const int yy = top_clamp(p.y + gr - 1, 0, H - 1), xx = top_clamp(x + gc - 1, 0, W - 1);
+                    gv = g[(top - 3 + min(gm, 2)) * lstride + (uint32_t)(yy * W + xx)];
+                };
+                fetch(0, vc, gvc);
+                for (int i = 0; i < cnt; i++) {
+                    fetch(min(i + 1, cnt - 1), vn, gvn);
+                    const Px p = locate_px(__builtin_amdgcn_readfirstlane((int)list[i]));
+                    const int x = w0 * 32 + p.x, y = p.y;
+                    const bool interior = x >= 1 && x <= W - 2 && y >= 1 && y <= H - 2;
+                    if (lane < 27) s.g[lane] = gvc;
+                    top_level_eval<FW>(vc, tf.taps, s, lane);
+                    float* g = g0 + (long long)p.b * npx;
+                    if (lane < 9 && interior)
+                        g[top * lstride + (long long)(y + gr - 1) * W + x + gc - 1] = s.top[lane];
+                    if (lane == 0) {
+                        auto get = [&](int m, int r, int c) {
+                            const int q = 3 * r + c;
+                            return (m == 2 ? s.top[q] : s.g[9 * (m + 1) + q]) - s.g[9 * m + q];
+                        };
+                        if (interior && key_test(get, fp.t0, fp.t, fp.edge, fp.subpixel).result != 0.f)
+                            atomicAdd(&row_count[(long long)p.b * fp.rows_per_image + fp.row_off[o] + jt * H + y], 1u);
+                        else
+                            atomicAnd(&mtop[(r0 + p.k) * nwords + w0 + (p.x >> 5)], ~(1u << (p.x & 31)));
+                    }
+                    asm volatile("" ::: "memory");
+#pragma unroll
+                    for (int q = 0; q < G::NLD; q++) vc[q] = vn[q];
+                    gvc = gvn;
+                }
+            }
+        }
+    }
+}
+
 __device__ __forceinline__ uint32_t wave_incl_scan(uint32_t v) {
     const int lane = threadIdx.x & 63;
 #pragma unroll
@@ -469,7 +578,8 @@
 }
 
 hipError_t launch_extrema(const float* pyr, uint32_t* mask, uint32_t* row_count,
-                          const FeatureParams& fp, hipStream_t stream, bool tiles) {
+                          const FeatureParams& fp, hipStream_t stream, bool tiles, bool lazy) {
+    if (tiles && lazy) return hipErrorInvalidValue;
     bool tile_ok = tiles && ((uintptr_t)pyr % 16) == 0;
     for (int o = 0; o < fp.n_octaves; o++)
         tile_ok = tile_ok && fp.oct[o].wa % 4 == 0 && fp.oct[o].wa >= 4 && fp.oct[o].gauss_off % 4 == 0 &&
@@ -519,17 +629,56 @@
     }
     eg.wave0[fp.n_octaves] = nw;
     const unsigned nb = (unsigned)((nw + 3) / 4);
-    switch ((fp.d + 2) * 2 + (pairs ? 1 : 0)) {
-#define SGK_EXTW(ND)                                                                             \
-    case 2 * ND: hipLaunchKernelGGL((k_extrema_wave2<ND, 1>), dim3(nb), dim3(256), 0, stream, pyr, \
-                                    mask, row_count, fp, eg); break;                             \
-    case 2 * ND + 1: hipLaunchKernelGGL((k_extrema_wave2<ND, 2>), dim3(nb), dim3(256), 0, stream,  \
-                                        pyr, mask, row_count, fp, eg); break;
-        SGK_EXTW(3) SGK_EXTW(4) SGK_EXTW(5) SGK_EXTW(6) SGK_EXTW(7) SGK_EXTW(8)
-        default: return hipErrorInvalidValue;
+#define SGK_EXTW(ND, LAZY)                                                                       \
+    case 2 * ND: hipLaunchKernelGGL((k_extrema_wave2<ND, 1, LAZY>), dim3(nb), dim3(256), 0, stream, \
+                                    pyr, mask, row_count, fp, eg); break;                        \
+    case 2 * ND + 1: hipLaunchKernelGGL((k_extrema_wave2<ND, 2, LAZY>), dim3(nb), dim3(256), 0,    \
+                                        stream, pyr, mask, row_count, fp, eg); break;
+    if (lazy) {
+        switch ((fp.d + 2) * 2 + (pairs ? 1 : 0)) {
+            SGK_EXTW(3, true) SGK_EXTW(4, true) SGK_EXTW(5, true) SGK_EXTW(6, true)
+            SGK_EXTW(7, true) SGK_EXTW(8, true)
+            default: return hipErrorInvalidValue;
+        }
+    } else {
+        switch ((fp.d + 2) * 2 + (pairs ? 1 : 0)) {
+            SGK_EXTW(3, false) SGK_EXTW(4, false) SGK_EXTW(5, false) SGK_EXTW(6, false)
+            SGK_EXTW(7, false) SGK_EXTW(8, false)
+            default: return hipErrorInvalidValue;
+        }
+    }
 #undef SGK_EXTW
-    }
     return hipGetLastError();
+}
+
+hipError_t launch_extrema_top(float* pyr, uint32_t* mask, uint32_t* row_count,
+                              const FeatureParams& fp, const TopLevelFilter& tf,
+                              hipStream_t stream) {
+    if (tf.fw < 1 || tf.fw > kTopMaxFW || !(tf.fw & 1) || fp.d < 1) return hipErrorInvalidValue;
+    ExtremaTopGrid tg{};
+    long long nu = 0;
+    for (int o = 0; o < fp.n_octaves; o++) {
+        tg.unit0[o] = (int)nu;
+        nu += ((long long)fp.batch * fp.oct[o].h + kTopRows - 1) / kTopRows;
+    }
+    if (nu <= 0 || nu >= (1ll << 31)) return hipErrorInvalidValue;
+    tg.unit0[fp.n_octaves] = (int)nu;
+    int dev = 0, cus = 0, per_cu = 0;
+    hipError_t e = hipGetDevice(&dev);
+    if (e == hipSuccess) e = hipDeviceGetAttribute(&cus, hipDeviceAttributeMultiprocessorCount, dev);
+    if (e != hipSuccess) return e;
+    const bool known = top_level_dispatch(tf.fw, [&](auto FWC) {
+        constexpr int FW = decltype(FWC)::value;
+        static int resident = 0;
+        if (!resident &&
+            hipOccupancyMaxActiveBlocksPerMultiprocessor(&resident, k_extrema_top<FW>, 256, 0) != hipSuccess)
+            resident = 0;
+        per_cu = std::max(1, resident);
+        const unsigned nb = (unsigned)std::min<long long>((nu + 3) / 4, (long long)std::max(1, cus) * per_cu);
+        hipLaunchKernelGGL((k_extrema_top<FW>), dim3(nb), dim3(256), 0, stream, pyr, mask, row_count,
+                           fp, tg, tf);
+    });
+    return known ? hipGetLastError() : hipErrorInvalidValue;
 }
 
 static size_t scan_blocks(size_t n) { return (n + 1023) / 1024; }
diff --git a/modify-sift-gpu_amd/csrc/sift_kernels.h b/modify-sift-gpu_amd/csrc/sift_kernels.h
--- a/modify-sift-gpu_amd/csrc/sift_kernels.h
+++ b/modify-sift-gpu_amd/csrc/sift_kernels.h
@@ -95,7 +95,15 @@
                                 int channels, bool bgr, float* dst, hipStream_t stream);
 
 hipError_t launch_extrema(const float* pyr, uint32_t* mask, uint32_t* row_count,
-                          const FeatureParams& fp, hipStream_t stream, bool tiles = false);
+                          const FeatureParams& fp, hipStream_t stream, bool tiles = false,
+                          bool lazy = false);
+struct TopLevelFilter {
+    int fw;
+    Taps taps;
+};
+hipError_t launch_extrema_top(float* pyr, uint32_t* mask, uint32_t* row_count,
+                              const FeatureParams& fp, const TopLevelFilter& tf,
+                              hipStream_t stream);
 
 size_t scan_tmp_words(size_t n);
 hipError_t launch_zero(uint32_t* a, size_t na, uint32_t* b, size_t nb, uint32_t* c, size_t nc,
@@ -176,6 +184,9 @@
                                         const uint32_t* n_cand_dev, int n_cand_cap,
                                         const FeatureParams* fp, int4* ints, float4* floats,
                                         hipStream_t stream);
+typedef hipError_t (*DebugTopLevelFn)(const float* pyr, const FeatureParams* fp,
+                                      const TopLevelFilter* tf, int image, int octave, int x, int y,
+                                      float* out9, hipStream_t stream);
 
 constexpr int kDistTable = 262145;
 struct Top2 { int max, idx, second; };
diff --git a/modify-sift-gpu_amd/csrc/sift_keys.h b/modify-sift-gpu_amd/csrc/sift_keys.h
--- a/modify-sift-gpu_amd/csrc/sift_keys.h
+++ b/modify-sift-gpu_amd/csrc/sift_keys.h
@@ -5,7 +5,9 @@
 
 struct KeyOut { float result, dx, dy, ds; };
 
-template <class Get>
+constexpr float kKeyUndecided = 2.0f;
+
+template <bool UNTIL_NEXT = false, class Get>
 __device__ __forceinline__ KeyOut key_test(Get get, float t0, float t, float edge, int subpixel) {
     KeyOut o{0.f, 0.f, 0.f, 0.f};
     const float v = get(1, 1, 1);
@@ -17,6 +19,10 @@
     const int seq_r[8] = {0, 2, 0, 1, 2, 0, 1, 2};
 #pragma unroll
     for (int s = 0; s < 8; s++) {
+        if (UNTIL_NEXT && s == 5) {
+            o.result = kKeyUndecided;
+            return o;
+        }
         if (s == 2) {
             const float vx2 = v * 2.0f;
             const float fxx = l + r - vx2;
diff --git a/modify-sift-gpu_amd/csrc/sift_top_level.h b/modify-sift-gpu_amd/csrc/sift_top_level.h
--- /dev/null
+++ b/modify-sift-gpu_amd/csrc/sift_top_level.h
@@ -0,0 +1,90 @@
+#pragma once
+#include <type_traits>
+
+namespace sgk {
+namespace {
+
+constexpr int kTopMaxFW = 33;
+constexpr int kTopWin = kTopMaxFW + 2;
+
+struct TopLds {
+    float win[kTopWin * kTopWin];
+    float hs[3 * kTopWin];
+    float top[9];
+    float g[27];
+};
+
+template <int FW>
+struct TopGeom {
+    static constexpr int N = FW + 2, HALF = FW >> 1;
+    static constexpr int SH = N <= 32 ? 5 : 6;
+    static constexpr int RSTEP = 64 >> SH;
+    static constexpr int NLD = (N + RSTEP - 1) / RSTEP;
+};
+
+__device__ __forceinline__ int top_clamp(int v, int lo, int hi) { return v < lo ? lo : (v > hi ? hi : v); }
+
+template <int FW>
+__device__ __forceinline__ void top_window_load(const float* __restrict__ src, int w, int h, int x,
+                                                int y, int lane, float (&v)[TopGeom<FW>::NLD]) {
+    using G = TopGeom<FW>;
+    const int c = lane & ((1 << G::SH) - 1), rsub = lane >> G::SH;
+    const int xx = top_clamp(x - 1 - G::HALF + c, 0, w - 1);
+#pragma unroll
+    for (int i = 0; i < G::NLD; i++) {
+        const int yy = top_clamp(y - 1 - G::HALF + i * G::RSTEP + rsub, 0, h - 1);
+        v[i] = src[(uint32_t)(yy * w + xx)];
+    }
+}
+
+template <int FW>
+__device__ __forceinline__ void top_level_eval(const float (&v)[TopGeom<FW>::NLD], const Taps& taps,
+                                               TopLds& s, int lane) {
+    using G = TopGeom<FW>;
+    constexpr int N = G::N;
+    const int c = lane & ((1 << G::SH) - 1), rsub = lane >> G::SH;
+#pragma unroll
+    for (int i = 0; i < G::NLD; i++) {
+        const int r = i * G::RSTEP + rsub;
+        if (c < N && r < N) s.win[r * N + c] = v[i];
+    }
+    asm volatile("" ::: "memory");
+    if (lane < N) {
+        const float* p = &s.win[lane * N];
+        float a0 = 0.f, a1 = 0.f, a2 = 0.f;
+#pragma unroll
+        for (int t = 0; t < N; t++) {
+            const float e = p[t];
+            if (t < FW) a0 = fma_(e, taps.k[t], a0);
+            if (t >= 1 && t - 1 < FW) a1 = fma_(e, taps.k[t - 1], a1);
+            if (t >= 2) a2 = fma_(e, taps.k[t - 2], a2);
+        }
+        s.hs[3 * lane] = a0;
+        s.hs[3 * lane + 1] = a1;
+        s.hs[3 * lane + 2] = a2;
+    }
+    asm volatile("" ::: "memory");
+    if (lane < 9) {
+        const float* p = &s.hs[lane];
+        float a = 0.f;
+#pragma unroll
+        for (int t = 0; t < FW; t++) a = fma_(p[3 * t], taps.k[t], a);
+        s.top[lane] = a;
+    }
+    asm volatile("" ::: "memory");
+}
+
+template <class F>
+inline bool top_level_dispatch(int fw, F&& f) {
+    switch (fw) {
+#define SGK_TOPFW(FW) case FW: f(std::integral_constant<int, FW>{}); return true;
+        SGK_TOPFW(5) SGK_TOPFW(7) SGK_TOPFW(9) SGK_TOPFW(11) SGK_TOPFW(13) SGK_TOPFW(15) SGK_TOPFW(17)
+        SGK_TOPFW(19) SGK_TOPFW(21) SGK_TOPFW(23) SGK_TOPFW(25) SGK_TOPFW(27) SGK_TOPFW(29)
+        SGK_TOPFW(31) SGK_TOPFW(33)
+#undef SGK_TOPFW
+        default: return false;
+    }
+}
+
+}
+}
diff --git a/modify-sift-gpu_amd/python/sgpu.py b/modify-sift-gpu_amd/python/sgpu.py
--- a/modify-sift-gpu_amd/python/sgpu.py
+++ b/modify-sift-gpu_amd/python/sgpu.py
@@ -36,6 +36,7 @@
     "sgpu_default_verify_params", "sgpu_verify_batch", "sgpu_verify_images",
     "sgpu_select_top_scale_batch", "sgpu_select_top_scale_images",
     "sgpu_prematch_batch", "sgpu_prematch_images",
+    "sgpu_debug_set_top_level", "sgpu_debug_top_level_at",
 ]
 
 PLAN_KINDS = ("level", "tile", "two", "tile_two", "tile_duo", "tile_duo_one", "duo", "trio")
@@ -89,6 +90,8 @@
         L.sgpu_debug_set_match_prune.argtypes = [vp, c.c_int]
         L.sgpu_debug_set_duo_strips.argtypes = [vp, c.c_int]
         L.sgpu_debug_set_feature_queue.argtypes = [vp, c.c_int]
+        L.sgpu_debug_set_top_level.argtypes = [vp, c.c_int]
+        L.sgpu_debug_top_level_at.argtypes = [vp, c.c_int, c.c_int, c.c_int, c.c_int, vp]
         L.sgpu_debug_geometry.argtypes = [vp, P(c.c_int), vp, c.c_int]
         L.sgpu_debug_gaussian.argtypes = [vp, c.c_int, c.c_int, c.c_int, vp]
         L.sgpu_debug_candidates.argtypes = [vp, vp, vp, c.c_int, P(c.c_int)]
@@ -939,6 +942,17 @@
     def set_duo_strips(self, mode: int = 0):
         self._check(lib().sgpu_debug_set_duo_strips(self._ctx, mode), "sgpu_debug_set_duo_strips")
 
+    TOP_LEVEL_RULE, TOP_LEVEL_DENSE, TOP_LEVEL_LAZY = 0, 1, 2
+
+    def set_top_level(self, mode: int = 0):
+        self._check(lib().sgpu_debug_set_top_level(self._ctx, mode), "sgpu_debug_set_top_level")
+
+    def top_level_at(self, image, octave, x, y):
+        out = np.zeros(9, np.float32)
+        self._check(lib().sgpu_debug_top_level_at(self._ctx, image, octave, x, y, out.ctypes.data),
+                    "sgpu_debug_top_level_at")
+        return out.reshape(3, 3)
+
     FEATURES_QUEUE, FEATURES_STATIC_ORIENTATION, FEATURES_STATIC_DESCRIPTOR, FEATURES_STATIC = 0, 1, 2, 3
 
     def set_feature_queue(self, mode: int = 0):
```

Result: faster. 20390 (median of 6 runs) (+7.4%).
